# cwitkowitz/amt-tools

Measured on AMD Instinct MI355X. Metric: audio frames/sec (OnsetsFrames+Mel-229 inference), higher is better.
Workload: dtype bf16

## Files before the change

amt_tools_amd/_lib.py:

```python
import ctypes as C
import os
import re

_HERE = os.path.dirname(os.path.abspath(__file__))
LIB_PATH = os.environ.get('AMTX_LIB_PATH') or os.path.join(_HERE, 'csrc', 'libamtx.so')
HEADER_PATH = os.path.join(os.path.dirname(_HERE), 'include', 'amtx.h')
EXTRA_HEADERS = ('amtx_tracks.h',)

_lib = None


class AmtxError(RuntimeError):
    pass


ERR_UNSUPPORTED = -3


class _Pointer(C.c_void_p):
    @classmethod
    def from_param(cls, obj):
        if hasattr(obj, 'data_ptr'):
            obj = obj.data_ptr()
        elif hasattr(obj, 'ctypes'):
            obj = obj.ctypes.data
        elif isinstance(obj, (str, bytes)):
            raise TypeError('a pointer argument, not text')
        return C.c_void_p.from_param(obj)


_CTYPES = {'i': C.c_int, 'l': C.c_int64, 'z': C.c_size_t, 'f': C.c_float, 'd': C.c_double, 's': C.c_char_p, 'p': _Pointer}
_SCALARS = {'int': 'i', 'int64_t': 'l', 'size_t': 'z', 'float': 'f', 'double': 'd'}
_POINTEES = {'void', 'float', 'double', 'int', 'int32_t', 'int64_t', 'uint16_t', 'uint8_t'}
_PARAM = re.compile(r'(const )?(\w+) ?(\*{0,2}) ?(\w*)')


def parse_header(text):
    text = re.sub(r'/\*.*?\*/|//[^\n]*', ' ', text, flags=re.S)
    text = re.sub(r'^[ \t]*(#.*|extern "C" \{|\})[ \t]*$', '', text, flags=re.M)
    handles, table = set(), {}

    def letter(decl, param, is_return=False):
        m = _PARAM.fullmatch(param)
        if m:
            const, base, stars, name = m.groups()
            if not stars and not const and base in _SCALARS:
                return _SCALARS[base], name
            if stars == '*' and const and base == 'char':
                return 's', name
            if stars and not is_return and (base in _POINTEES or base in handles):
                return 'p', name
        raise AmtxError(f'cannot map "{param}" in the declaration "{decl}"')

    for decl in (' '.join(d.split()) for d in text.split(';')):
        m = re.fullmatch(r'typedef struct (\w+) \1', decl)
        if m:
            handles.add(m.group(1))
            continue
        m = re.fullmatch(r'(.*?) ?\b(amtx_\w+) ?\((.*)\)', decl)
        if not m:
            if decl:
                raise AmtxError(f'cannot read the declaration "{decl}"')
            continue
        ret, name, params = m.groups()
        if name in table:
            raise AmtxError(f'{name} is declared twice')
        params = [] if params.strip() == 'void' else [p.strip() for p in params.split(',')]
        letters, names = letter(decl, ret, is_return=True)[0], []
        for param in params:
            code, pname = letter(decl, param)
            letters += code
            names.append(pname)
        if 'stream' in names and (names.index('stream') != len(names) - 1 or params[-1].replace(' ', '') != 'void*stream'):
            raise AmtxError(f'`stream` must be the last parameter and a `void*` in the declaration "{decl}"')
        table[name] = (letters, 'stream' in names)
    return table


_signatures = None


def signatures():
    global _signatures
    if _signatures is None:
        with open(HEADER_PATH) as f:
            _signatures = parse_header(f.read())
    return _signatures


def declared_symbols():
    return sorted(signatures())


_extra_signatures = None


def extra_signatures():
    global _extra_signatures
    if _extra_signatures is None:
        tables, seen = {}, set(signatures())
        for header in EXTRA_HEADERS:
            with open(os.path.join(os.path.dirname(HEADER_PATH), header)) as f:
                tables[header] = parse_header(f.read())
            twice = seen & set(tables[header])
            if twice:
                raise AmtxError(f'{sorted(twice)[0]} is declared in {header} and in another header')
            seen |= set(tables[header])
        _extra_signatures = tables
    return _extra_signatures


_funcs = {}


def lib():
    global _lib
    if _lib is None:
        if not os.path.exists(LIB_PATH):
            raise AmtxError(f'{LIB_PATH} is missing: build the HIP extension first '
                            f'(python -m amt_tools_amd.build, or __graft_entry__.build()). '
                            f'There is no CPU fallback for the product path.')
        try:
            handle = C.CDLL(LIB_PATH)
        except OSError as e:
            raise AmtxError(f'cannot load {LIB_PATH}: {e}') from e
        bound = dict(signatures())
        for table in extra_signatures().values():
            bound.update(table)
        for name, (letters, stream) in bound.items():
            try:
                fn = getattr(handle, name)
            except AttributeError as e:
                raise AmtxError(f'{LIB_PATH} does not export {name}') from e
            fn.restype = _CTYPES[letters[0]]
            fn.argtypes = [_CTYPES[c] for c in letters[1:]]
            _funcs[name] = (fn, len(letters) - 1, letters[0] in 'il', stream)
        _lib = handle
    return _lib


def call(name, *args, device=None):
    lib()
    try:
        fn, nargs, checked, stream = _funcs[name]
    except KeyError:
        raise AmtxError(f'include/amtx.h and {", ".join(EXTRA_HEADERS)} declare no function {name}') from None
    fill_stream = stream and device is not None
    if len(args) + fill_stream != nargs:
        raise TypeError(f'{name} takes {nargs - fill_stream} arguments{" besides the stream" if fill_stream else ""} ({len(args)} given)')
    if device is None:
        rc = fn(*args)
    else:
        import torch
        with torch.cuda.device(device):
            rc = fn(*args, current_stream(device)) if stream else fn(*args)
    return check(rc, name) if checked else rc


def check(rc, what=''):
    if rc is None or rc < 0:
        msg = lib().amtx_last_error()
        raise AmtxError(f'{what} failed ({rc}): {msg.decode() if msg else "?"}')
    return rc


def ptr(t):
    if t is None:
        return None
    if hasattr(t, 'data_ptr'):
        return C.c_void_p(t.data_ptr())
    return C.c_void_p(t.ctypes.data)


def current_stream(device=None):
    import torch
    return C.c_void_p(torch.cuda.current_stream(device).cuda_stream)


GUARD_BYTES = 0
_GUARD_PATTERN = 0xA5
_GUARDED = {}


def alloc_workspace(nbytes, device):
    import torch
    nbytes = int(nbytes)
    g = int(GUARD_BYTES)
    if g <= 0:
        return torch.empty(nbytes, dtype=torch.uint8, device=device)
    assert g % 256 == 0
    full = torch.empty(nbytes + 2 * g, dtype=torch.uint8, device=device)
    full[:g] = _GUARD_PATTERN
    full[g + nbytes:] = _GUARD_PATTERN
    ws = full[g:g + nbytes]
    import weakref
    for k in [k for k, (r, _) in _GUARDED.items() if r() is None]:
        del _GUARDED[k]
    _GUARDED[ws.data_ptr()] = (weakref.ref(full), g)
    return ws


def guards_intact(ws):
    rec = _GUARDED.get(ws.data_ptr())
    base = getattr(ws, '_base', None)
    if rec is None or base is None or rec[0]() is not base:
        return True
    g = rec[1]
    return bool((base[:g] == _GUARD_PATTERN).all().item()) and bool((base[g + ws.numel():] == _GUARD_PATTERN).all().item())
```

amt_tools_amd/csrc/amtx_kernels.h:

```cpp
#pragma once
#include "amtx_common.h"

enum { AMTX_T_BF16 = 0, AMTX_T_F32 = 1, AMTX_T_SPLIT = 2 };

static inline size_t amtx_tsize(int t) { return t == AMTX_T_BF16 ? 2 : 4; }

struct GemmArgs {
    const void* A; int64_t lda; int a_type;
    const bf16_t* W; int n_pad, k_pad, planes;
    const float* bias;
    void* C; int64_t ldc; int c_type;
    int64_t M; int N, K;
    int groups; int64_t a_gs, w_gs, bias_gs, c_gs;
    const int2* pair_map = nullptr; float* pair_out = nullptr; int64_t pair_gs = 0, pair_pitch = 0;
    int pair_rows[16] = {0, 0, 0, 0, 0, 0, 0, 0, 0, 0, 0, 0, 0, 0, 0, 0};
    float* pair_max = nullptr; int pair_nh = 0;
    float* roll_out = nullptr; int roll_T = 0; float roll_thr = 0.5f; int roll_group = 0;
    bf16_t* copy16 = nullptr; int64_t copy16_ld = 0; int copy16_col0 = 0, copy16_gs = 0, copy16_pad = 0;
    int64_t a_plane = 0;
    int64_t a_valid_lo = 0, a_valid_hi = 0;
    int64_t a_split = 0, c_split = 0;
};
constexpr int AMTX_GEMM_MULTI_MAX = 10;
struct GemmMulti { GemmArgs p[AMTX_GEMM_MULTI_MAX]; int n; };

struct ConvArgs {
    const void* in; int in_type;
    const bf16_t* wfrag; int planes;
    const float* shift;
    void* out; int out_type;
    int B, T, F, c_out;
    int groups; int64_t in_gs, w_gs, shift_gs, out_gs;
    const float* feats = nullptr; int64_t f_stride_b = 0, f_stride_c = 0, f_stride_t = 0, f_stride_f = 0;
    int c_in = 0;
    const bf16_t* w1frag = nullptr; const float* shift1 = nullptr;
    int64_t w1_gs = 0;
    const float* f_clip_max = nullptr; const float* f_ref = nullptr;
    const void* feats16 = nullptr;
    int64_t out_ts = 0;
    int64_t in_split = 0, out_split = 0;
};
struct ConvTiling { int ft, ntf, ntt; int64_t ntiles; };
static inline ConvTiling amtx_conv_tiling(int B, int T, int F, int ft_max, int tt) {
    const int fe = (F + 1) & ~1;
    const int ntf = (fe + ft_max - 1) / ft_max, ntt = (T + tt - 1) / tt;
    return {2 * (((fe >> 1) + ntf - 1) / ntf), ntf, ntt, (int64_t)ntf * ntt * B};
}
static inline int amtx_conv_recip(int cols, int n) {
    const int inv = 65536 / cols + 1;
    for (int x = 0; x < n; ++x)
        if (((x * inv) >> 16) != x / cols) return 0;
    return inv;
}
struct ConvRefusal { int code = AMTX_OK; char text[192] = {0}; };
#define AMTX_ROUTE_REFUSE(r, code_, ...)                                  \
    do {                                                                   \
        (r).err.code = (code_);                                            \
        snprintf((r).err.text, sizeof((r).err.text), __VA_ARGS__);         \
        return (r);                                                        \
    } while (0)
#define AMTX_ROUTE_REQUIRE(r, cond, ...) do { if (!(cond)) AMTX_ROUTE_REFUSE(r, AMTX_ERR_ARG, __VA_ARGS__); } while (0)
#define AMTX_RETURN_REFUSAL(r)                                             \
    do {                                                                   \
        if ((r).err.code != AMTX_OK) {                                     \
            amtx_set_error("%s", (r).err.text);                            \
            return (r).err.code;                                           \
        }                                                                  \
    } while (0)

int amtx_launch_convx3(const ConvArgs& c, hipStream_t stream);
int amtx_launch_convx12(const ConvArgs& c, hipStream_t stream);

static inline __host__ __device__ bool amtx_conv1g_tapk(int c_in, int planes) { return (planes == 1 || planes == 2) && c_in >= 2 && c_in <= 8; }

struct Conv1Args {
    const float* in; int64_t stride_b, stride_c, stride_t, stride_f;
    const float* w;
    const float* shift;
    void* out; int out_type;
    int B, T, F, c_in, c_out;
    int groups; int64_t w_gs, shift_gs, out_gs;
    int relu = 1;
};

struct LstmArgs {
    const void* xproj; int x_type;
    const bf16_t* whh; int planes;
    void* out; int out_type;
    int B, T;
    int groups; int64_t x_gs, w_gs, out_gs;
    int hidden = 128;
    float* save = nullptr;
};

namespace amtx_bf16 {
#include "amtx_kernels_fmt.h"
}
#ifdef AMTX_WITH_F16
namespace amtx_f16 {
#include "amtx_kernels_fmt.h"
}
#endif
using namespace AMTX_FMT_NS;

size_t amtx_bce_loss_partials(int B, int T, int keys);
int amtx_launch_bce_loss(const float* logits, int64_t ld, const float* labels, const float* weight, int B, int T, int keys, float* loss,
                         float* grad, float* partial, hipStream_t stream);
int amtx_launch_loss_reduce(const float* partial, int64_t n, float inv_bt, float* loss, hipStream_t stream);
int amtx_launch_pianoroll(const float* logits, int64_t ld, int col0, int B, int T, int keys, float threshold, float* out,
                          hipStream_t stream);

int amtx_launch_cvt_pad_bf16(const float* src, int64_t ld_src, int n_src, bf16_t* dst, int ld_dst, int64_t rows, hipStream_t stream,
                             bool f16 = false );
int amtx_launch_cvt_split(const float* src, int64_t ld_src, int n_src, bf16_t* dst, int ld_dst, int64_t split, int64_t rows, hipStream_t stream);
int amtx_launch_zero_cols(void* base, int64_t pitch_bytes, int width_bytes, int64_t rows, hipStream_t stream);

constexpr int DEC_HALF = 150;
constexpr int DEC_TAPS = 2 * DEC_HALF + 1;
constexpr int DEC_KW = 352;
constexpr int DEC_NKS = DEC_KW / 32;
int amtx_launch_cqt_decimate(const float* in, int64_t n_in, int64_t in_stride, int in_pad, float* out, int64_t n_out, int64_t out_stride, int pad,
                             const void* tfrag, int zero_pads, float* maxbuf, int n_harm, int batch, hipStream_t stream);
```

amt_tools_amd/csrc/amtx_kernels_fmt.h:

```cpp

bool amtx_gemm_has_roll_epilogue(const GemmArgs& g);
int amtx_launch_gemm(const GemmArgs& g, hipStream_t stream);
int amtx_launch_gemm_multi(const GemmArgs* gs, int n, hipStream_t stream);
void amtx_gemm_pack_dims(int N, int K, int* n_pad, int* k_pad);
void amtx_gemm_pack_host(const float* W, int64_t ldw, int N, int K, int planes, bf16_t* out);

int amtx_launch_conv3x3(const ConvArgs& c, hipStream_t stream);
size_t amtx_conv1_wfrag_elems(int c_in, int planes);
void amtx_conv1_pack_host(const float* w, const float* scale, int c_in, int planes, bf16_t* out);
size_t amtx_conv3x3_wfrag_elems(int c_out, int planes);
void amtx_conv3x3_pack_host(const float* w, const float* scale, int c_out, int planes, bf16_t* out);
int amtx_launch_conv1(const Conv1Args& c, hipStream_t stream);

bool amtx_conv_stack_fused_ok(int B, int T, int F, int groups);
int amtx_launch_conv_stack(const ConvArgs& c2, const bf16_t* w3frag, int64_t w3_gs, const float* shift3, void* out, int64_t out_gs,
                           int64_t out_plane, hipStream_t stream);

int amtx_conv3x3_gen_ntc(int c_in, int c_out);
size_t amtx_conv3x3_gen_wfrag_elems(int c_in, int c_out, int planes);
void amtx_conv3x3_gen_pack_host(const float* w , const float* scale, int c_in, int c_out, int planes, bf16_t* out);
int amtx_launch_conv3x3_gen(const ConvArgs& c, int c_in, hipStream_t stream);
size_t amtx_conv1g_wfrag_elems(int c_in, int c_mid, int planes);
void amtx_conv1g_pack_host(const float* w , const float* scale, int c_in, int c_mid, int planes, bf16_t* out);
bool amtx_conv3x3_gen_can_fuse1(int c_in, int c_mid, int c_out, int planes);

int amtx_launch_bilstm(const LstmArgs& l, hipStream_t stream);
size_t amtx_bilstm_wfrag_elems(int hidden, int planes);
void amtx_bilstm_pack_host(const float* whh_fwd, const float* whh_bwd, int hidden, int planes, bf16_t* out);
int amtx_launch_bilstm_pack_dev(const float* whh_fwd, const float* whh_bwd, int hidden, int planes, bf16_t* frag_fwd, bf16_t* frag_bwd, hipStream_t stream);
int amtx_launch_bilstm_bwd(const float* dout, const float* save, const bf16_t* whh_t, int hidden, int planes, float* dxproj, int B, int T, int groups,
                           hipStream_t stream);

int amtx_pack_bn_fold_dev(const float* conv_bias, const float* gamma, const float* beta, const float* mean, const float* var, int c_out, float* scale,
                          float* shift, hipStream_t s);
int amtx_pack_conv3x3_dev(const float* w, const float* scale, int c_out, int planes, bf16_t* out, hipStream_t s);
int amtx_pack_conv1_dev(const float* w, const float* scale, int planes, bf16_t* out, hipStream_t s);
int amtx_pack_conv_gen_dev(const float* w, const float* scale, int c_in, int c_out, int ntc, int planes, bf16_t* out, hipStream_t s);
int amtx_pack_conv1g_dev(const float* w, const float* scale, int c_in, int c_mid, int planes, bf16_t* out, hipStream_t s);
int amtx_pack_scale_rows_dev(const float* w, const float* scale, int rows, int cols, float* out, hipStream_t s);
int amtx_pack_linear_dev(const float* W, int64_t ldw, int N, int K, int planes, int n_pad, int k_pad, int row0, int rows_owned, int perm_c, int perm_f,
                         bf16_t* out, hipStream_t s);
void amtx_pack_linear_host(const float* W, int64_t ldw, int N, int K, int planes, int n_pad, int k_pad, int row0, int rows_owned, int perm_c, int perm_f,
                           bf16_t* out);
int amtx_pack_head_fold_dev(const float* w_out, const float* w_fc1, const float* b_fc1, const float* b_out, int n_out, int dim_am, int kfc, int kfc_pad,
                            int nf3, int fq, float* wfold, float* bfold, hipStream_t s);
int amtx_pack_vec_add_dev(const float* a, const float* b, int n, float* out, hipStream_t s);
```

amt_tools_amd/csrc/amtx_pack_layouts.h:

```cpp
#pragma once
#include "amtx_common.h"

#include <cmath>

constexpr int AMTX_FRAG = 64 * 8;
constexpr int AMTX_CONV_CIN = 32;
constexpr int AMTX_LSTM_BWD_WAVES = 8;

static constexpr __host__ __device__ int g_wfrags_per_tile(int ci16) { return 9 * (ci16 / 2) + 5 * (ci16 % 2); }

static inline __host__ __device__ void amtx_split_store(bf16_t* out, size_t i, size_t plane_stride, int planes, float v) {
#if defined(__HIP_DEVICE_COMPILE__)
    asm volatile("" : "+v"(v));
#endif
    const bf16_t hi = f32_to_bf16_rn(v);
    out[i] = hi;
    if (planes == 2) out[i + plane_stride] = f32_to_bf16_rn(v - bf16_to_f32(hi));
}

namespace {
struct AmtxFragPut {
    bf16_t* out; int planes; int frag_elems = AMTX_FRAG;
    __host__ __device__ void operator()(size_t frag, int e, float v) const { amtx_split_store(out, frag * planes * frag_elems + e, frag_elems, planes, v); }
};
struct AmtxPlanePut {
    bf16_t* out; int planes; size_t plane_elems;
    __host__ __device__ void operator()(size_t i, float v) const { amtx_split_store(out, i, plane_elems, planes, v); }
};
}

static inline __host__ __device__ void amtx_bn_fold(const float* cb, const float* g, const float* be, const float* mu, const float* var, int c, float* scale,
                                                    float* shift) {
#pragma clang fp contract(off)
    const double s = (double)g[c] / sqrt((double)var[c] + 1e-5);
    scale[c] = (float)s;
    shift[c] = (float)((double)be[c] + ((double)cb[c] - (double)mu[c]) * s);
}

static inline __host__ __device__ void amtx_layout_scale_rows(int item, const float* w, const float* scale, int cols, float* out) {
    out[item] = w[item] * scale[item / cols];
}

static inline __host__ __device__ int amtx_layout_conv3x3_items(int c_out) { return 9 * (c_out / 16) * AMTX_FRAG; }
template <class Put>
static inline __host__ __device__ void amtx_layout_conv3x3(int item, const float* w, const float* scale, int c_out, const Put& put) {
    const int NT = c_out / 16;
    int r = item;
    const int j = r & 7; r >>= 3;
    const int l = r & 63; r >>= 6;
    const int nt = r % NT, tap = r / NT;
    const int row = l & 15;
    const int co = (row >> 2) * (4 * NT) + 4 * nt + (row & 3);
    const int ci = (l >> 4) * 8 + j;
    put(tap * NT + nt, l * 8 + j, w[((size_t)co * AMTX_CONV_CIN + ci) * 9 + tap] * (scale ? scale[co] : 1.0f));
}

constexpr int AMTX_LAYOUT_CONV1_ITEMS = 4 * 2 * AMTX_FRAG;
template <class Put>
static inline __host__ __device__ void amtx_layout_conv1(int item, const float* w, const float* scale, const Put& put) {
    int r = item;
    const int e = r & 7; r >>= 3;
    const int l = r & 63; r >>= 6;
    const int nt = r & 1, q = r >> 1;
    const int row = l & 15, g = l >> 4;
    const int co = (row >> 2) * 8 + 4 * nt + (row & 3);
    const int kw = e - q;
    put(q * 2 + nt, l * 8 + e, (g < 3 && kw >= 0 && kw <= 2) ? w[(size_t)co * 9 + g * 3 + kw] * (scale ? scale[co] : 1.0f) : 0.0f);
}

static inline void amtx_layout_conv1_multi(const float* w, const float* scale, int c_in, int planes, bf16_t* out) {
    const int kvalid = 9 * c_in, ksteps = (kvalid + 15) / 16;
    const AmtxFragPut put{out, planes, 64 * 4};
    for (int ks = 0; ks < ksteps; ++ks)
        for (int nt = 0; nt < 2; ++nt)
            for (int l = 0; l < 64; ++l) {
                const int row = l & 15;
                const int co = (row >> 2) * 8 + 4 * nt + (row & 3);
                for (int j = 0; j < 4; ++j) {
                    const int k = 16 * ks + 4 * (l >> 4) + j;
                    put(ks * 2 + nt, l * 4 + j, k < kvalid ? w[(size_t)co * kvalid + k] * (scale ? scale[co] : 1.0f) : 0.0f);
                }
            }
}

static inline __host__ __device__ int amtx_layout_conv_gen_items(int c_out) { return (c_out / 16) * AMTX_FRAG; }
template <class Put>
static inline __host__ __device__ void amtx_layout_conv_gen(int item, const float* w, const float* scale, int c_in, int ntc, const Put& put) {
    const int ci16 = c_in / 16, n32 = ci16 / 2, n16 = ci16 % 2;
    const int nmain = 9 * ntc * n32, nfrag = ntc * g_wfrags_per_tile(ci16);
    int r = item;
    const int j = r & 7; r >>= 3;
    const int l = r & 63; r >>= 6;
    const int nt = r % ntc, ch = r / ntc;
    const int row = l & 15, gq = l >> 4;
    const int co = ch * 16 * ntc + (row >> 2) * (4 * ntc) + 4 * nt + (row & 3);
    const float sc = scale ? scale[co] : 1.0f;
    auto wv = [&](int ci, int tap) { return w[((size_t)co * c_in + ci) * 9 + tap] * sc; };
    auto frag = [&](int f, float v) { put((size_t)ch * nfrag + f, l * 8 + j, v); };
    for (int tap = 0; tap < 9; ++tap)
        for (int ks = 0; ks < n32; ++ks) frag((tap * ntc + nt) * n32 + ks, wv(32 * ks + 8 * gq + j, tap));
    if (!n16) return;
    const int ct = 32 * n32 + 8 * (gq & 1) + j;
    for (int kw = 0; kw < 3; ++kw) frag(nmain + kw * ntc + nt, wv(ct, (gq < 2 ? 0 : 3) + kw));
    frag(nmain + 3 * ntc + nt, wv(ct, gq < 2 ? 6 : 7));
    frag(nmain + 4 * ntc + nt, gq < 2 ? wv(ct, 8) : 0.0f);
}

static inline __host__ __device__ int amtx_conv1g_ksteps(int c_in, bool tapk) { return tapk ? 3 : (9 * c_in + 31) / 32; }
static inline __host__ __device__ int amtx_layout_conv1g_items(int c_in, int c_mid, bool tapk) { return (c_mid / 16) * amtx_conv1g_ksteps(c_in, tapk) * AMTX_FRAG; }
template <class Put>
static inline __host__ __device__ void amtx_layout_conv1g(int item, const float* w, const float* scale, int c_in, bool tapk, const Put& put) {
    const int kvalid = 9 * c_in, nks = amtx_conv1g_ksteps(c_in, tapk);
    int r = item;
    const int j = r & 7; r >>= 3;
    const int l = r & 63; r >>= 6;
    const int ks = r % nks, nt = r / nks;
    const int co = 16 * nt + (l & 15);
    const int tap = 4 * ks + (l >> 4), k = 32 * ks + 8 * (l >> 4) + j;
    const bool valid = tapk ? tap < 9 && j < c_in : k < kvalid;
    const size_t src = tapk ? ((size_t)co * c_in + j) * 9 + tap : (size_t)co * kvalid + k;
    put(nt * nks + ks, l * 8 + j, valid ? w[src] * (scale ? scale[co] : 1.0f) : 0.0f);
}

static inline __host__ __device__ int amtx_fc1_col(int k, int nf3, int fq) { return (k % nf3) * fq + k / nf3; }

static inline __host__ __device__ int64_t amtx_layout_linear_items(int rows_owned, int k_pad) { return (int64_t)rows_owned * (k_pad / 8); }
template <class Put>
static inline __host__ __device__ void amtx_layout_linear(int64_t item, const float* W, int64_t ldw, int N, int K, int k_pad, int row0, int perm_c, int perm_f,
                                                          const Put& put) {
    const int n = (int)(item / (k_pad / 8)), k0 = 8 * (int)(item - (int64_t)n * (k_pad / 8));
    const float* src = W + (int64_t)n * ldw + (perm_c > 0 ? amtx_fc1_col(k0, perm_c, perm_f) : k0);
    const int step = perm_c > 0 ? perm_f : 1;
    for (int j = 0; j < 8; ++j) put((size_t)(row0 + n) * k_pad + k0 + j, n < N && k0 + j < K ? src[(int64_t)j * step] : 0.0f);
}

static inline __host__ __device__ int amtx_layout_bilstm_items(int hidden) { return hidden * hidden; }
template <class Put>
static inline __host__ __device__ void amtx_layout_bilstm(int item, const float* whh_fwd, const float* whh_bwd, int hidden, const Put& put) {
    const int nu = hidden / 16, ksn = hidden / 32;
    int r = item;
    const int l = r & 63; r >>= 6;
    const int ks = r % ksn; r /= ksn;
    const int q = r & 3; r >>= 2;
    const int u = r % nu, dir = r / nu;
    const float* src = (dir == 0 ? whh_fwd : whh_bwd) + (size_t)(q * hidden + 16 * u + (l & 15)) * hidden + 32 * ks + 8 * (l >> 4);
    for (int j = 0; j < 8; ++j) put(item >> 6, l * 8 + j, src[j]);
}

template <class Put>
static inline __host__ __device__ void amtx_layout_bilstm_transposed(int item, const float* whh_fwd, const float* whh_bwd, int hidden, const Put& put) {
    const int ut_n = hidden / (16 * AMTX_LSTM_BWD_WAVES), ksn = 4 * hidden / 32;
    int r = item;
    const int l = r & 63; r >>= 6;
    const int ks = r % ksn; r /= ksn;
    const int ut = r % ut_n; r /= ut_n;
    const int wv = r % AMTX_LSTM_BWD_WAVES, dir = r / AMTX_LSTM_BWD_WAVES;
    const float* src = (dir == 0 ? whh_fwd : whh_bwd) + (size_t)(32 * ks + 8 * (l >> 4)) * hidden + 16 * ut_n * wv + 16 * ut + (l & 15);
    for (int j = 0; j < 8; ++j) put(item >> 6, l * 8 + j, src[(size_t)j * hidden]);
}
```

amt_tools_amd/csrc/gemm.hip:

```cpp

#include "amtx_kernels.h"

#include <algorithm>
#include <cstdlib>

namespace {

constexpr int BM = 128, BN = 128, BK = 32;
constexpr int TILE_BYTES = BM * BK * 2;

__device__ __forceinline__ int lds_off(int row, int chunk) {
    return (row * 4 + (chunk ^ ((0x78 >> (((row >> 2) & 3) * 2)) & 3))) * 16;
}

template <int A_TYPE, int NS>
struct AStage {
    uint4 hi, lo;
    __device__ __forceinline__ void load(const char* base, int64_t row_off_elems, bool valid, int64_t vlo = 0, int64_t vhi = 0, int64_t split = 0) {
        if (A_TYPE == AMTX_T_SPLIT) {
            hi = valid ? *reinterpret_cast<const uint4*>(base + row_off_elems * 2) : make_uint4(0, 0, 0, 0);
            lo = valid ? *reinterpret_cast<const uint4*>(base + (split + row_off_elems) * 2) : make_uint4(0, 0, 0, 0);
        } else if (A_TYPE == AMTX_T_BF16) {
            hi = valid ? *reinterpret_cast<const uint4*>(base + row_off_elems * 2) : make_uint4(0, 0, 0, 0);
            lo = make_uint4(0, 0, 0, 0);
        } else {
            float4 x0 = make_float4(0, 0, 0, 0), x1 = make_float4(0, 0, 0, 0);
            if (valid && vhi > 0 && (row_off_elems < vlo || row_off_elems + 8 > vhi)) {
                float e[8];
#pragma unroll
                for (int i = 0; i < 8; ++i) {
                    const int64_t idx = row_off_elems + i;
                    e[i] = (idx >= vlo && idx < vhi) ? reinterpret_cast<const float*>(base)[idx] : 0.f;
                }
                x0 = make_float4(e[0], e[1], e[2], e[3]);
                x1 = make_float4(e[4], e[5], e[6], e[7]);
            } else if (valid) {
                struct __attribute__((packed, aligned(4))) f32x4_a4 { float x, y, z, w; };
                const f32x4_a4* p = reinterpret_cast<const f32x4_a4*>(base + row_off_elems * 4);
                const f32x4_a4 p0 = p[0], p1 = p[1];
                x0 = make_float4(p0.x, p0.y, p0.z, p0.w);
                x1 = make_float4(p1.x, p1.y, p1.z, p1.w);
            }
            hi = __builtin_bit_cast(uint4, x0);
            lo = __builtin_bit_cast(uint4, x1);
        }
    }
    __device__ __forceinline__ void finish() {
        if (A_TYPE == AMTX_T_F32) {
            const float4 x0 = __builtin_bit_cast(float4, hi), x1 = __builtin_bit_cast(float4, lo);
            const float f[8] = {x0.x, x0.y, x0.z, x0.w, x1.x, x1.y, x1.z, x1.w};
            uint32_t h[4], l[4];
#pragma unroll
            for (int i = 0; i < 4; ++i) {
                l[i] = 0;
                if (NS == 2) split_bf16x2(f[2 * i], f[2 * i + 1], h[i], l[i]);
                else h[i] = pack_bf16x2(f[2 * i], f[2 * i + 1]);
            }
            hi = make_uint4(h[0], h[1], h[2], h[3]);
            lo = make_uint4(l[0], l[1], l[2], l[3]);
        }
    }
};

template <int A_TYPE, int C_TYPE, int NS>
__device__ __forceinline__ void gemm_tile(const GemmArgs& g, int grp, int bx, int by, char* smem) {
    constexpr int BUF_BYTES = 2 * NS * TILE_BYTES;
    const int tid = threadIdx.x, lane = tid & 63, wave = tid >> 6;
    const int wm = wave >> 1, wn = wave & 1;
    const int64_t m0 = (int64_t)bx * BM;
    const int n0 = by * BN;

    const char* Abase = reinterpret_cast<const char*>(g.A) + (int64_t)grp * g.a_gs * (A_TYPE == AMTX_T_F32 ? 4 : 2);
    const bf16_t* Wbase = g.W + (int64_t)grp * g.w_gs;
    const int64_t plane_elems = (int64_t)g.n_pad * g.k_pad;

    const int srow0 = tid >> 2, srow1 = srow0 + 64, schunk = tid & 3;
    const bool arow_ok0 = (m0 + srow0) < g.M, arow_ok1 = (m0 + srow1) < g.M;
    const int64_t a_off0 = (m0 + srow0) * g.lda + schunk * 8, a_off1 = (m0 + srow1) * g.lda + schunk * 8;
    const int64_t w_off0 = (int64_t)(n0 + srow0) * g.k_pad + schunk * 8, w_off1 = (int64_t)(n0 + srow1) * g.k_pad + schunk * 8;
    const int soff0 = lds_off(srow0, schunk), soff1 = lds_off(srow1, schunk);

    AStage<A_TYPE, NS> sa0, sa1;
    uint4 sw0h, sw1h, sw0l = make_uint4(0, 0, 0, 0), sw1l = make_uint4(0, 0, 0, 0);
#define LOAD_TILE(k0)                                                                              \
    do {                                                                                           \
        const bool kok = ((k0) + schunk * 8) < g.K;                                                \
        sa0.load(Abase, a_off0 + (k0), arow_ok0 && kok, g.a_valid_lo, g.a_valid_hi, g.a_split);    \
        sa1.load(Abase, a_off1 + (k0), arow_ok1 && kok, g.a_valid_lo, g.a_valid_hi, g.a_split);    \
        sw0h = *reinterpret_cast<const uint4*>(Wbase + w_off0 + (k0));                             \
        sw1h = *reinterpret_cast<const uint4*>(Wbase + w_off1 + (k0));                             \
        if (NS == 2) {                                                                             \
            sw0l = *reinterpret_cast<const uint4*>(Wbase + plane_elems + w_off0 + (k0));           \
            sw1l = *reinterpret_cast<const uint4*>(Wbase + plane_elems + w_off1 + (k0));           \
        }                                                                                          \
    } while (0)
#define STORE_TILE(buf)                                                                            \
    do {                                                                                           \
        char* sb = smem + (buf) * BUF_BYTES;                                                       \
        sa0.finish();                                                                              \
        sa1.finish();                                                                              \
        *reinterpret_cast<uint4*>(sb + soff0) = sa0.hi;                                            \
        *reinterpret_cast<uint4*>(sb + soff1) = sa1.hi;                                            \
        if (NS == 2) {                                                                             \
            *reinterpret_cast<uint4*>(sb + TILE_BYTES + soff0) = sa0.lo;                           \
            *reinterpret_cast<uint4*>(sb + TILE_BYTES + soff1) = sa1.lo;                           \
        }                                                                                          \
        *reinterpret_cast<uint4*>(sb + NS * TILE_BYTES + soff0) = sw0h;                            \
        *reinterpret_cast<uint4*>(sb + NS * TILE_BYTES + soff1) = sw1h;                            \
        if (NS == 2) {                                                                             \
            *reinterpret_cast<uint4*>(sb + 3 * TILE_BYTES + soff0) = sw0l;                         \
            *reinterpret_cast<uint4*>(sb + 3 * TILE_BYTES + soff1) = sw1l;                         \
        }                                                                                          \
    } while (0)

    f32x4_t acc[4][4];
#pragma unroll
    for (int i = 0; i < 4; ++i)
#pragma unroll
        for (int j = 0; j < 4; ++j) acc[i][j] = (f32x4_t){0.f, 0.f, 0.f, 0.f};

    const int nk = g.k_pad / BK;
    LOAD_TILE(0);
    STORE_TILE(0);
    __syncthreads();

    const int frow = lane & 15, fchunk = lane >> 4;
    for (int kt = 0; kt < nk; ++kt) {
        const int cur = kt & 1;
        if (kt + 1 < nk) LOAD_TILE((kt + 1) * BK);
        const char* b = smem + cur * BUF_BYTES;
        uint4 af[4][NS], wf[4][NS];
#pragma unroll
        for (int t = 0; t < 4; ++t) {
            const int ar = wm * 64 + t * 16 + frow;
            const int wr = wn * 64 + t * 16 + frow;
#pragma unroll
            for (int p = 0; p < NS; ++p) {
                af[t][p] = *reinterpret_cast<const uint4*>(b + p * TILE_BYTES + lds_off(ar, fchunk));
                wf[t][p] = *reinterpret_cast<const uint4*>(b + (NS + p) * TILE_BYTES + lds_off(wr, fchunk));
            }
        }
#pragma unroll
        for (int nt = 0; nt < 4; ++nt)
#pragma unroll
            for (int mt = 0; mt < 4; ++mt) {
                acc[nt][mt] = mfma16(wf[nt][0], af[mt][0], acc[nt][mt]);
                if (NS == 2) {
                    acc[nt][mt] = mfma16(wf[nt][0], af[mt][1], acc[nt][mt]);
                    acc[nt][mt] = mfma16(wf[nt][1], af[mt][0], acc[nt][mt]);
                }
            }
        if (kt + 1 < nk) STORE_TILE(cur ^ 1);
        __syncthreads();
    }
// ... 107 lines not shown
    const bf16_t* a_src[4];
    const bf16_t* w_src[4];
#define GLDS_SET_TILE(TILE_ID)                                                                                \
    do {                                                                                                      \
        const unsigned lg = xcd_remap((unsigned)(TILE_ID), (unsigned)ntiles);                                 \
        const int tn0 = (lg % nbn) * TB;                                                                      \
        const int64_t tm0 = (int64_t)(lg / nbn) * TB;                                                         \
        _Pragma("unroll") for (int n = 0; n < 4; ++n) {                                                       \
            const int row = (wave * 4 + n) * 8 + (lane >> 3);                                                 \
            const int c = (lane & 7) ^ ((row >> 1) & 7);                                                      \
            const int cw = (lane & 7) ^ wswz(row);                                                            \
            int64_t mr = tm0 + row;                                                                           \
            if (mr >= g.M) mr = g.M - 1;           \
            a_src[n] = Abase + mr * a_pitch + c * 8;                                                          \
            w_src[n] = Wbase + (int64_t)(tn0 + row) * g.k_pad + cw * 8;                                       \
        }                                                                                                     \
    } while (0)
    const unsigned lds_base = __builtin_amdgcn_readfirstlane((unsigned)(uintptr_t)(lds_void_t*)smem) + wave * 4096;
#define GLDS_ISSUE(k0, buf)                                                                                   \
    do {                                                                                                      \
        const unsigned sb = lds_base + (buf) * 2 * TILE;                                                      \
        const int64_t a_off = (int64_t)((k0) / GBK) * a_kstep;                                                \
        glds16x4(a_src[0] + a_off, a_src[1] + a_off, a_src[2] + a_off, a_src[3] + a_off, sb);                 \
        glds16x4(w_src[0] + (k0), w_src[1] + (k0), w_src[2] + (k0), w_src[3] + (k0), sb + TILE);              \
    } while (0)
#define GLDS_COMPUTE(buf)                                                                                     \
    do {                                                                                                      \
        const char* b = smem + (buf) * 2 * TILE;                                                              \
        _Pragma("unroll") for (int kk = 0; kk < 2; ++kk) {                                                    \
            uint4 af[MT], wf[4];                                                                              \
            _Pragma("unroll") for (int t = 0; t < MT; ++t) {                                                  \
                const int ar = wm * (TB / 2) + t * 16 + frow;                                                 \
                af[t] = *reinterpret_cast<const uint4*>(b + ar * 128 + (((kk * 4 + fchunk) ^ ((ar >> 1) & 7)) << 4)); \
            }                                                                                                 \
            _Pragma("unroll") for (int t = 0; t < 4; ++t) {                                                   \
                const int wr = wn * 64 + 16 * (frow >> 2) + 4 * t + (frow & 3);         \
                wf[t] = *reinterpret_cast<const uint4*>(b + TILE + wr * 128 + (((kk * 4 + fchunk) ^ wswz(wr)) << 4)); \
            }                                                                                                 \
            _Pragma("unroll") for (int nt = 0; nt < 4; ++nt)                                                  \
                _Pragma("unroll") for (int mt = 0; mt < MT; ++mt) acc[nt][mt] = mfma16(wf[nt], af[mt], acc[nt][mt]); \
        }                                                                                                     \
    } while (0)
#define GLDS_SYNC()                                                                                           \
    do {                                                                                                      \
        asm volatile("s_waitcnt vmcnt(0)" ::: "memory");                                                      \
        __syncthreads();                                                                                      \
    } while (0)

    const int nk = g.k_pad / GBK;
    const int frow = lane & 15, fchunk = lane >> 4;

    int tile = blockIdx.x;
    GLDS_SET_TILE(tile);
    GLDS_ISSUE(0, 0);
    GLDS_SYNC();
    int cur = 0;
    for (;;) {
        const unsigned lg = xcd_remap((unsigned)tile, (unsigned)ntiles);
        const int n0 = (lg % nbn) * TB;
        const int64_t m0 = (int64_t)(lg / nbn) * TB;
        const int next = tile + (int)gridDim.x;
        const bool has_next = next < ntiles;

        f32x4_t acc[4][MT];
#pragma unroll
        for (int i = 0; i < 4; ++i)
#pragma unroll
            for (int j = 0; j < MT; ++j) acc[i][j] = (f32x4_t){0.f, 0.f, 0.f, 0.f};

        for (int kt = 0; kt + 1 < nk; ++kt) {
            GLDS_ISSUE((kt + 1) * GBK, cur ^ 1);
            GLDS_COMPUTE(cur);
            GLDS_SYNC();
            cur ^= 1;
        }
        if (has_next) {
            GLDS_SET_TILE(next);
            GLDS_ISSUE(0, cur ^ 1);
        }
        GLDS_COMPUTE(cur);

        {
            const int nb = n0 + wn * 64 + 16 * (lane >> 4);
            float bv[4][4];
#pragma unroll
            for (int nt = 0; nt < 4; ++nt)
#pragma unroll
                for (int r = 0; r < 4; ++r) bv[nt][r] = (bias && nb + 4 * nt < g.N) ? bias[nb + 4 * nt + r] : 0.f;
            constexpr int ES = (C_TYPE == AMTX_T_BF16 ? 2 : 4);
            const bool wide = nb + 16 <= g.N && ((g.ldc * ES) % 16) == 0;
#pragma unroll
            for (int mt = 0; mt < MT; ++mt) {
                const int64_t m = m0 + wm * (TB / 2) + mt * 16 + (lane & 15);
                if (m >= g.M) continue;
                char* dst = Cbase + (m * g.ldc + nb) * ES;
                float o[4][4];
#pragma unroll
                for (int nt = 0; nt < 4; ++nt)
#pragma unroll
                    for (int r = 0; r < 4; ++r) o[nt][r] = acc[nt][mt][r] + bv[nt][r];
                if (C_TYPE == AMTX_T_F32) {
                    if (g.C) {
#pragma unroll
                        for (int nt = 0; nt < 4; ++nt)
                            if (wide || nb + 4 * nt < g.N) reinterpret_cast<float4*>(dst)[nt] = make_float4(o[nt][0], o[nt][1], o[nt][2], o[nt][3]);
                    }
                    if (g.copy16) {
                        bf16_t* cp = g.copy16 + m * g.copy16_ld + g.copy16_col0 + (int64_t)grp * g.copy16_gs + nb;
#pragma unroll
                        for (int nt = 0; nt < 4; ++nt) {
                            const int n4 = nb + 4 * nt;
                            if (n4 < g.N) reinterpret_cast<uint2*>(cp)[nt] = make_uint2(pack_bf16x2(o[nt][0], o[nt][1]), pack_bf16x2(o[nt][2], o[nt][3]));
                            else if (n4 < g.N + g.copy16_pad) reinterpret_cast<uint2*>(cp)[nt] = make_uint2(0u, 0u);
                        }
                    }
                    if (g.roll_out && grp == g.roll_group) {
                        const unsigned bclip = (unsigned)m / (unsigned)g.roll_T, tfrm = (unsigned)m - bclip * (unsigned)g.roll_T;
                        float* ro = g.roll_out + ((int64_t)bclip * g.N + nb) * g.roll_T + tfrm;
#pragma unroll
                        for (int nt = 0; nt < 4; ++nt)
#pragma unroll
                            for (int r = 0; r < 4; ++r)
                                if (nb + 4 * nt + r < g.N) {
                                    const float sg = 1.0f / (1.0f + expf(-o[nt][r]));
                                    ro[(int64_t)(4 * nt + r) * g.roll_T] = g.roll_thr < 0.f ? sg : (sg < g.roll_thr ? 0.f : 1.f);
                                }
                    }
                } else if (wide) {
#pragma unroll
                    for (int h = 0; h < 2; ++h)
                        reinterpret_cast<uint4*>(dst)[h] = make_uint4(pack_bf16x2(o[2 * h][0], o[2 * h][1]), pack_bf16x2(o[2 * h][2], o[2 * h][3]),
                                                                     pack_bf16x2(o[2 * h + 1][0], o[2 * h + 1][1]), pack_bf16x2(o[2 * h + 1][2], o[2 * h + 1][3]));
                } else {
#pragma unroll
                    for (int nt = 0; nt < 4; ++nt)
                        if (nb + 4 * nt < g.N) reinterpret_cast<uint2*>(dst)[nt] = make_uint2(pack_bf16x2(o[nt][0], o[nt][1]), pack_bf16x2(o[nt][2], o[nt][3]));
                }
            }
        }
        if (!has_next) break;
        GLDS_SYNC();
        cur ^= 1;
        tile = next;
    }
#undef GLDS_SET_TILE
#undef GLDS_ISSUE
#undef GLDS_COMPUTE
#undef GLDS_SYNC
}
constexpr int RBK = 32, RST = 4, RTB = 256;
constexpr int RING_MAX_NPAD = 4096;
constexpr int ROP = RTB * RBK * 2;
constexpr int RSTAGE = 2 * ROP;
__device__ uint4 g_gemm_trash[4];

__device__ __forceinline__ int rswz(int q) { return (0x78 >> (q * 2)) & 3; }

#ifdef AMTX_GEMM_TIMING
__device__ unsigned long long g_gemm_prof[2][16];
#define PP_TICK(SLOT)                                                      \
    do {                                                                   \
        const unsigned long long now_ = __builtin_readcyclecounter();      \
        prof_acc[SLOT] += now_ - prof_t;                                   \
        prof_t = now_;                                                     \
    } while (0)
#else
#define PP_TICK(SLOT) do {} while (0)
#endif

template <int C_TYPE>
__global__ __launch_bounds__(512) void gemm_pp_kernel(GemmArgs g, int ntiles) {
    extern __shared__ __attribute__((aligned(16))) char smem[];
    constexpr int MT = 8;
    constexpr int ES = (C_TYPE == AMTX_T_BF16 ? 2 : 4);
    constexpr int NSTORE = MT * (C_TYPE == AMTX_T_BF16 ? 2 : 4);
    const int tid = threadIdx.x, lane = tid & 63, wave = __builtin_amdgcn_readfirstlane(tid >> 6);
    const int wm = wave >> 2, wn = wave & 3;
    const int grp = blockIdx.z;
    const unsigned nbn = g.n_pad / RTB;
    const int nk = g.k_pad / RBK;

    const bf16_t* Abase = reinterpret_cast<const bf16_t*>(g.A) + (int64_t)grp * g.a_gs;
    const bf16_t* Wbase = g.W + (int64_t)grp * g.w_gs;
    char* Cbase = reinterpret_cast<char*>(g.C) + (int64_t)grp * g.c_gs * ES;
    float* bias_l = reinterpret_cast<float*>(smem + RST * RSTAGE);
    for (int i = tid; i < g.n_pad; i += 512) bias_l[i] = (g.bias && i < g.N) ? g.bias[(int64_t)grp * g.bias_gs + i] : 0.f;

    const bf16_t* a_src[2];
    const bf16_t* w_src[2];
#define PP_SET_TILE(TILE_ID)                                                                                  \
    do {                                                                                                      \
        const unsigned lg = xcd_remap((unsigned)(TILE_ID), (unsigned)ntiles);                                 \
        const int tn0 = (lg % nbn) * RTB;                                                                     \
        const int64_t tm0 = (int64_t)(lg / nbn) * RTB;                                                        \
        _Pragma("unroll") for (int n = 0; n < 2; ++n) {                                                       \
            const int row = wave * 32 + n * 16 + (lane >> 2);                                                 \
            int64_t mr = tm0 + row;                                                                           \
            if (mr >= g.M) mr = g.M - 1;                                                                      \
            a_src[n] = Abase + mr * g.lda + ((lane & 3) ^ rswz((row >> 2) & 3)) * 8;                          \
            w_src[n] = Wbase + (int64_t)(tn0 + row) * g.k_pad + ((lane & 3) ^ rswz((row >> 4) & 3)) * 8;      \
        }                                                                                                     \
    } while (0)
    const unsigned lds_base = __builtin_amdgcn_readfirstlane((unsigned)(uintptr_t)(lds_void_t*)smem) + wave * 2048;

    const int my_tiles = (ntiles - (int)blockIdx.x + (int)gridDim.x - 1) / (int)gridDim.x;
    const int S = my_tiles * nk;
    int is = 0, ikt = 0, itile = blockIdx.x;
    bool pending_w = false;
#define PP_ISSUE_A()                                                                                          \
    do {                                                                                                      \
        if (is < S) {                                                                                         \
            const unsigned sb = lds_base + (is & (RST - 1)) * RSTAGE;                                         \
            _Pragma("unroll") for (int n = 0; n < 2; ++n) glds16(a_src[n] + ikt * RBK, sb + n * 1024);        \
            pending_w = true;                                                                                 \
        }                                                                                                     \
    } while (0)
#define PP_ISSUE_W()                                                                                          \
    do {                                                                                                      \
        if (pending_w) {                                                                                      \
            const unsigned sb = lds_base + (is & (RST - 1)) * RSTAGE;                                         \
            _Pragma("unroll") for (int n = 0; n < 2; ++n) glds16(w_src[n] + ikt * RBK, sb + ROP + n * 1024);  \
            pending_w = false;                                                                                \
            ++is;                                                                                             \
            if (++ikt == nk) {                                                                                \
                ikt = 0;                                                                                      \
                itile += (int)gridDim.x;                                                                      \
                if (is < S) PP_SET_TILE(itile);                                                               \
            }                                                                                                 \
        }                                                                                                     \
    } while (0)
#define PP_BARRIER()                                                                                          \
    do {                                                                                                      \
        __builtin_amdgcn_sched_barrier(0);                                                                    \
        asm volatile("s_barrier" ::: "memory");                                                               \
        __builtin_amdgcn_sched_barrier(0);                                                                    \
    } while (0)

    PP_SET_TILE(itile);
    PP_ISSUE_A(); PP_ISSUE_W();
    PP_ISSUE_A(); PP_ISSUE_W();
    PP_ISSUE_A();
    if (S >= 3) wait_vm<6>(); else if (S == 2) wait_vm<4>(); else wait_vm<0>();
    asm volatile("s_waitcnt lgkmcnt(0)\n\ts_barrier" ::: "memory");
    __builtin_amdgcn_sched_barrier(0);
    if (wm == 1) PP_BARRIER();

    const int frow = lane & 15, fchunk = lane >> 4;
    const int a_off = (wm * 128 + frow) * 64 + ((fchunk ^ rswz((frow >> 2) & 3)) << 4);
    const int w_off = ROP + (wn * 64 + 16 * (frow >> 2) + (frow & 3)) * 64 + ((fchunk ^ rswz(frow >> 2)) << 4);

    f32x4_t acc[4][MT];
#pragma unroll
    for (int i = 0; i < 4; ++i)
#pragma unroll
        for (int j = 0; j < MT; ++j) acc[i][j] = (f32x4_t){0.f, 0.f, 0.f, 0.f};

#ifdef AMTX_GEMM_TIMING
    unsigned long long prof_acc[14] = {0,0,0,0,0,0,0,0,0,0,0,0,0,0};
    unsigned long long prof_t = __builtin_readcyclecounter();
#endif
    int ckt = 0, ctile = blockIdx.x;
    bool stores_recent = false;
    for (int cs = 0; cs < S; ++cs) {
        const char* b = smem + (cs & (RST - 1)) * RSTAGE;
        uint4 af[4], wf[4];
#pragma unroll
        for (int t = 0; t < 4; ++t) wf[t] = *reinterpret_cast<const uint4*>(b + w_off + t * 256);
#pragma unroll
        for (int t = 0; t < 4; ++t) af[t] = *reinterpret_cast<const uint4*>(b + a_off + t * 1024);
        __builtin_amdgcn_sched_barrier(0);
        PP_ISSUE_W();
        PP_TICK(0);
        PP_BARRIER();
        PP_TICK(1);
        asm volatile("s_waitcnt lgkmcnt(0)" ::: "memory");
        PP_TICK(2);
        __builtin_amdgcn_s_setprio(1);
#pragma unroll
        for (int mt = 0; mt < 4; ++mt)
#pragma unroll
            for (int nt = 0; nt < 4; ++nt) acc[nt][mt] = mfma16(wf[nt], af[mt], acc[nt][mt]);
        __builtin_amdgcn_s_setprio(0);
        PP_TICK(3);
        PP_BARRIER();
        PP_TICK(4);
        {
            const int newer = min(S - 2 - cs, 1);
            if (newer >= 0) {
                if (!stores_recent) { if (newer == 1) wait_vm<4>(); else wait_vm<0>(); }
                else { if (newer == 1) wait_vm<4 + NSTORE>(); else wait_vm<NSTORE>(); }
            }
        }
        __builtin_amdgcn_sched_barrier(0);
        PP_TICK(5);
#pragma unroll
        for (int t = 0; t < 4; ++t) af[t] = *reinterpret_cast<const uint4*>(b + a_off + (4 + t) * 1024);
        __builtin_amdgcn_sched_barrier(0);
        PP_ISSUE_A();
        stores_recent = false;
        PP_TICK(6);
        PP_BARRIER();
        PP_TICK(7);
        asm volatile("s_waitcnt lgkmcnt(0)" ::: "memory");
        PP_TICK(8);
        __builtin_amdgcn_s_setprio(1);
#pragma unroll
        for (int mt = 0; mt < 4; ++mt)
#pragma unroll
            for (int nt = 0; nt < 4; ++nt) acc[nt][4 + mt] = mfma16(wf[nt], af[mt], acc[nt][4 + mt]);
        __builtin_amdgcn_s_setprio(0);
        PP_TICK(9);

        if (++ckt == nk) {
            const unsigned lg = xcd_remap((unsigned)ctile, (unsigned)ntiles);
            const int n0 = (lg % nbn) * RTB;
            const int64_t m0 = (int64_t)(lg / nbn) * RTB;
            const int nb = n0 + wn * 64 + 16 * (lane >> 4);
            f32x4_t bv[4];
#pragma unroll
            for (int nt = 0; nt < 4; ++nt) bv[nt] = *reinterpret_cast<const f32x4_t*>(bias_l + nb + 4 * nt);
#pragma unroll
            for (int mt = 0; mt < MT; ++mt) {
                const int64_t m = m0 + wm * 128 + mt * 16 + (lane & 15);
#ifdef AMTX_PP_NOSTORE
                char* dst = reinterpret_cast<char*>(g_gemm_trash);
#else
                char* dst = m < g.M ? Cbase + (m * g.ldc + nb) * ES : reinterpret_cast<char*>(g_gemm_trash);
#endif
                float o[4][4];
#pragma unroll
                for (int nt = 0; nt < 4; ++nt)
#pragma unroll
                    for (int r = 0; r < 4; ++r) o[nt][r] = acc[nt][mt][r] + bv[nt][r];
                if (C_TYPE == AMTX_T_F32) {
#pragma unroll
                    for (int nt = 0; nt < 4; ++nt) reinterpret_cast<float4*>(dst)[nt] = make_float4(o[nt][0], o[nt][1], o[nt][2], o[nt][3]);
                } else {
#pragma unroll
                    for (int h = 0; h < 2; ++h)
                        reinterpret_cast<uint4*>(dst)[h] = make_uint4(pack_bf16x2(o[2 * h][0], o[2 * h][1]), pack_bf16x2(o[2 * h][2], o[2 * h][3]),
                                                                     pack_bf16x2(o[2 * h + 1][0], o[2 * h + 1][1]), pack_bf16x2(o[2 * h + 1][2], o[2 * h + 1][3]));
                }
#pragma unroll
                for (int nt = 0; nt < 4; ++nt) acc[nt][mt] = (f32x4_t){0.f, 0.f, 0.f, 0.f};
            }
            ckt = 0;
            ctile += (int)gridDim.x;
            stores_recent = true;
            PP_TICK(13);
        }
        PP_TICK(10);
        PP_BARRIER();
        PP_TICK(11);
    }
#ifdef AMTX_GEMM_TIMING
    if (lane == 0 && (wave & 3) == 0) {
        for (int i = 0; i < 12; ++i) atomicAdd(&g_gemm_prof[wm][i], prof_acc[i]);
        atomicAdd(&g_gemm_prof[wm][13], prof_acc[13]);
        atomicAdd(&g_gemm_prof[wm][12], (unsigned long long)S);
    }
#endif
    if (wm == 0) PP_BARRIER();
#undef PP_SET_TILE
#undef PP_ISSUE_A
#undef PP_ISSUE_W
#undef PP_BARRIER
}

constexpr int SPL = 256 * RBK * 2;
constexpr int SSTAGE = 4 * SPL;

template <int C_TYPE>
__global__ __launch_bounds__(512) void gemm_split_kernel(GemmArgs g, int ntiles) {
    extern __shared__ __attribute__((aligned(16))) char smem[];
    constexpr int MT = 8;
    const int tid = threadIdx.x, lane = tid & 63, wave = __builtin_amdgcn_readfirstlane(tid >> 6);
    const int wm = wave >> 2, wn = wave & 3;
    const int grp = blockIdx.z;
    const unsigned nbn = g.n_pad / RTB;
    const int nk = g.k_pad / RBK;

    const bf16_t* Abase = reinterpret_cast<const bf16_t*>(g.A) + (int64_t)grp * g.a_gs;
    const bf16_t* Wbase = g.W + (int64_t)grp * g.w_gs;
    const int64_t w_plane = (int64_t)g.n_pad * g.k_pad;
    const float* bias = g.bias ? g.bias + (int64_t)grp * g.bias_gs : nullptr;

    const bf16_t* a_src[2];
    const bf16_t* w_src[2];
#define SP_SET_TILE(TILE_ID)                                                                                  \
    do {                                                                                                      \
        const unsigned lg = xcd_remap((unsigned)(TILE_ID), (unsigned)ntiles);                                 \
        const int tn0 = (lg % nbn) * RTB;                                                                     \
        const int64_t tm0 = (int64_t)(lg / nbn) * RTB;                                                        \
        _Pragma("unroll") for (int n = 0; n < 2; ++n) {                                                       \
            const int row = wave * 32 + n * 16 + (lane >> 2);                                                 \
            int64_t mr = tm0 + row;                                                                           \
            if (mr >= g.M) mr = g.M - 1;                                                                      \
            a_src[n] = Abase + mr * g.lda + ((lane & 3) ^ rswz((row >> 2) & 3)) * 8;                          \
            w_src[n] = Wbase + (int64_t)(tn0 + row) * g.k_pad + ((lane & 3) ^ rswz((row >> 4) & 3)) * 8;      \
        }                                                                                                     \
    } while (0)
    const unsigned lds_base = __builtin_amdgcn_readfirstlane((unsigned)(uintptr_t)(lds_void_t*)smem) + wave * 2048;
#define SP_ISSUE(k0, buf)                                                                                     \
    do {                                                                                                      \
        const unsigned sb = lds_base + (buf) * SSTAGE;                                                        \
        glds16x2(a_src[0] + (k0), a_src[1] + (k0), sb);                                                       \
        glds16x2(a_src[0] + g.a_split + (k0), a_src[1] + g.a_split + (k0), sb + SPL);                         \
        glds16x2(w_src[0] + (k0), w_src[1] + (k0), sb + 2 * SPL);                                             \
        glds16x2(w_src[0] + w_plane + (k0), w_src[1] + w_plane + (k0), sb + 3 * SPL);                         \
    } while (0)
    const int frow = lane & 15, fchunk = lane >> 4;
    const int a_off = (wm * 128 + frow) * 64 + ((fchunk ^ rswz((frow >> 2) & 3)) << 4);
    const int w_off = 2 * SPL + (wn * 64 + 16 * (frow >> 2) + (frow & 3)) * 64 + ((fchunk ^ rswz(frow >> 2)) << 4);
#define SP_COMPUTE(buf)                                                                                       \
    do {                                                                                                      \
        const char* b = smem + (buf) * SSTAGE;                                                                \
        uint4 wh[4], wl[4];                                                                                   \
        _Pragma("unroll") for (int t = 0; t < 4; ++t) {                                                       \
            wh[t] = *reinterpret_cast<const uint4*>(b + w_off + t * 256);                                     \
            wl[t] = *reinterpret_cast<const uint4*>(b + w_off + SPL + t * 256);                               \
        }                                                                                                     \
        _Pragma("unroll") for (int h = 0; h < 2; ++h) {                                                       \
            uint4 ah[4], al[4];                                                                               \
            _Pragma("unroll") for (int t = 0; t < 4; ++t) {                                                   \
                ah[t] = *reinterpret_cast<const uint4*>(b + a_off + (4 * h + t) * 1024);                      \
                al[t] = *reinterpret_cast<const uint4*>(b + a_off + SPL + (4 * h + t) * 1024);                \
            }                                                                                                 \
            _Pragma("unroll") for (int mt = 0; mt < 4; ++mt)                                                  \
                _Pragma("unroll") for (int nt = 0; nt < 4; ++nt) acc[nt][4 * h + mt] = mfma16(wh[nt], ah[mt], acc[nt][4 * h + mt]); \
            _Pragma("unroll") for (int mt = 0; mt < 4; ++mt)                                                  \
                _Pragma("unroll") for (int nt = 0; nt < 4; ++nt) acc[nt][4 * h + mt] = mfma16(wh[nt], al[mt], acc[nt][4 * h + mt]); \
            _Pragma("unroll") for (int mt = 0; mt < 4; ++mt)                                                  \
                _Pragma("unroll") for (int nt = 0; nt < 4; ++nt) acc[nt][4 * h + mt] = mfma16(wl[nt], ah[mt], acc[nt][4 * h + mt]); \
        }                                                                                                     \
    } while (0)
#define SP_SYNC()                                                                                             \
    do {                                                                                                      \
        asm volatile("s_waitcnt vmcnt(0)" ::: "memory");                                                      \
        __syncthreads();                                                                                      \
    } while (0)

    int tile = blockIdx.x;
    SP_SET_TILE(tile);
    SP_ISSUE(0, 0);
    SP_SYNC();
    int cur = 0;
    for (;;) {
        const unsigned lg = xcd_remap((unsigned)tile, (unsigned)ntiles);
        const int n0 = (lg % nbn) * RTB;
        const int64_t m0 = (int64_t)(lg / nbn) * RTB;
        const int next = tile + (int)gridDim.x;
        const bool has_next = next < ntiles;

        f32x4_t acc[4][MT];
#pragma unroll
        for (int i = 0; i < 4; ++i)
#pragma unroll
            for (int j = 0; j < MT; ++j) acc[i][j] = (f32x4_t){0.f, 0.f, 0.f, 0.f};

        for (int kt = 0; kt + 1 < nk; ++kt) {
            SP_ISSUE((kt + 1) * RBK, cur ^ 1);
            SP_COMPUTE(cur);
            SP_SYNC();
            cur ^= 1;
        }
        if (has_next) {
            SP_SET_TILE(next);
            SP_ISSUE(0, cur ^ 1);
        }
        SP_COMPUTE(cur);

        {
            const int nb = n0 + wn * 64 + 16 * (lane >> 4);
            float bv[4][4];
#pragma unroll
            for (int nt = 0; nt < 4; ++nt)
#pragma unroll
                for (int r = 0; r < 4; ++r) bv[nt][r] = (bias && nb + 4 * nt < g.N) ? bias[nb + 4 * nt + r] : 0.f;
#pragma unroll
            for (int mt = 0; mt < MT; ++mt) {
                const int64_t m = m0 + wm * 128 + mt * 16 + (lane & 15);
                if (m >= g.M || nb + 16 > g.N) continue;
                float o[16];
#pragma unroll
                for (int nt = 0; nt < 4; ++nt)
#pragma unroll
                    for (int r = 0; r < 4; ++r) o[4 * nt + r] = acc[nt][mt][r] + bv[nt][r];
                if (C_TYPE == AMTX_T_F32) {
                    float4* dst = reinterpret_cast<float4*>(reinterpret_cast<float*>(g.C) + (int64_t)grp * g.c_gs + m * g.ldc + nb);
#pragma unroll
                    for (int nt = 0; nt < 4; ++nt) dst[nt] = make_float4(o[4 * nt], o[4 * nt + 1], o[4 * nt + 2], o[4 * nt + 3]);
                } else {
                    bf16_t* dh = reinterpret_cast<bf16_t*>(g.C) + (int64_t)grp * g.c_gs + m * g.ldc + nb;
                    uint32_t hh[8], ll[8];
// ... 343 lines not shown
                                if (nb + 4 * nt + r < g.N) {
                                    const float sg = 1.0f / (1.0f + expf(-o[nt][r]));
                                    ro[(int64_t)(4 * nt + r) * g.roll_T] = g.roll_thr < 0.f ? sg : (sg < g.roll_thr ? 0.f : 1.f);
                                }
                    }
                }
            }
            zero_acc();
            ckt = 0;
            ++cj;
        }
    }
    asm volatile("s_waitcnt vmcnt(0)" ::: "memory");
}

int launch_skinny(const GemmArgs& g, hipStream_t stream, bool split) {
    const int64_t ntiles = (g.M + 255) / 256;
    AMTX_REQUIRE(ntiles < (1ll << 31), "gemm: too many output tiles");
    int64_t gx = std::max<int64_t>(1, 256 / std::max(1, g.groups));
    if (gx > ntiles) gx = ntiles;
    if (split) {
        AMTX_GRANT_LDS(gemm_skinny_split_kernel, SK_LDS);
        hipLaunchKernelGGL(gemm_skinny_split_kernel, dim3((unsigned)gx, 1, (unsigned)g.groups), dim3(512), SK_LDS, stream, g, (int)ntiles);
    } else {
        AMTX_GRANT_LDS(gemm_skinny_kernel, SK_LDS);
        hipLaunchKernelGGL(gemm_skinny_kernel, dim3((unsigned)gx, 1, (unsigned)g.groups), dim3(512), SK_LDS, stream, g, (int)ntiles);
    }
    AMTX_CHECK_LAUNCH();
    return AMTX_OK;
}

template <int C_TYPE, int TB>
int launch_glds(const GemmArgs& g, hipStream_t stream) {
    const int64_t ntiles = ((g.M + TB - 1) / TB) * (g.n_pad / TB);
    AMTX_REQUIRE(ntiles < (1ll << 31), "gemm: too many output tiles");
    const size_t lds = 4 * (size_t)TB * GBK * 2;
    auto kern = gemm_glds_kernel<C_TYPE, TB>;
    AMTX_GRANT_LDS(kern, lds);
    hipLaunchKernelGGL(kern, dim3(persistent_gx(TB == 128 ? 512 : 256, g.groups, ntiles), 1, (unsigned)g.groups), dim3(TB * 2), lds, stream, g, (int)ntiles);
    AMTX_CHECK_LAUNCH();
    return AMTX_OK;
}

template <int A_TYPE, int C_TYPE, int NS>
int launch(const GemmArgs& g, hipStream_t stream) {
    dim3 grid((unsigned)((g.M + BM - 1) / BM), (unsigned)(g.n_pad / BN), (unsigned)g.groups);
    const size_t lds = 2 * 2 * NS * TILE_BYTES;
    hipLaunchKernelGGL((gemm_kernel<A_TYPE, C_TYPE, NS>), grid, dim3(256), lds, stream, g);
    AMTX_CHECK_LAUNCH();
    return AMTX_OK;
}

}

#if defined(AMTX_GEMM_TIMING) && !defined(AMTX_F16)
extern "C" void amtxdbg_gemm_prof(unsigned long long* out, int reset) {
    unsigned long long h[2][16];
    (void)hipMemcpyFromSymbol(h, HIP_SYMBOL(g_gemm_prof), sizeof(h));
    memcpy(out, h, sizeof(h));
    if (reset) { memset(h, 0, sizeof(h)); (void)hipMemcpyToSymbol(HIP_SYMBOL(g_gemm_prof), h, sizeof(h)); }
}
#endif

namespace AMTX_FMT_NS {

void amtx_gemm_pack_dims(int N, int K, int* n_pad, int* k_pad) {
    *n_pad = ((N + BN - 1) / BN) * BN;
    *k_pad = ((K + GBK - 1) / GBK) * GBK;
}

void amtx_gemm_pack_host(const float* W, int64_t ldw, int N, int K, int planes, bf16_t* out) {
    int n_pad, k_pad;
    amtx_gemm_pack_dims(N, K, &n_pad, &k_pad);
    amtx_pack_linear_host(W, ldw, N, K, planes, n_pad, k_pad, 0, n_pad, 0, 0, out);
}


struct GemmSwitches { bool no_skinny, force_pp, no_pp, no_split_dma; };
static const GemmSwitches& gemm_switches() {
    auto on = [](const char* name) { return getenv(name) != nullptr; };
    static const GemmSwitches sw = {on("AMTX_GEMM_NO_SKINNY"), on("AMTX_GEMM_PP"), on("AMTX_GEMM_NO_PP"), on("AMTX_GEMM_NO_SPLIT_DMA")};
    return sw;
}

static int gemm_validate(const GemmArgs& g) {
    AMTX_REQUIRE(g.A && g.W, "gemm: null pointer");
    AMTX_REQUIRE(!g.pair_map || (g.a_type == AMTX_T_F32 && g.c_type == AMTX_T_F32 && g.pair_out && g.N % 2 == 0), "gemm: the magnitude epilogue needs fp32 A / C, an output and an even N");
    AMTX_REQUIRE(g.M > 0 && g.N > 0 && g.K > 0 && g.groups > 0, "gemm: bad sizes");
    AMTX_REQUIRE(g.K % 8 == 0 && g.N % 4 == 0, "gemm: K must be a multiple of 8 and N of 4 (K=%d N=%d)", g.K, g.N);
    AMTX_REQUIRE(g.n_pad % BN == 0 && g.k_pad % BK == 0 && g.n_pad >= g.N && g.k_pad >= g.K, "gemm: bad packed dims");
    AMTX_REQUIRE(g.a_type == AMTX_T_F32 ? (g.a_valid_hi > 0 ? ((uintptr_t)g.A % 4) == 0 : (g.lda % 4 == 0 && ((uintptr_t)g.A % 16) == 0))
                                        : ((g.lda * 2) % 16 == 0 && ((uintptr_t)g.A % 16) == 0),
                 "gemm: A rows must be 16-byte aligned (4-byte aligned for a bounded fp32 A)");
    AMTX_REQUIRE(g.a_valid_hi == 0 || (g.a_type == AMTX_T_F32 && g.a_valid_lo >= 0 && g.a_valid_hi > g.a_valid_lo), "gemm: bad valid range of A");
    AMTX_REQUIRE(g.ldc % 4 == 0 && ((uintptr_t)g.C % 16) == 0, "gemm: C rows must be 16-byte aligned");
    AMTX_REQUIRE(g.planes == 1 || g.planes == 2, "gemm: planes must be 1 or 2");
    return AMTX_OK;
}

int amtx_launch_gemm_multi(const GemmArgs* gs, int n, hipStream_t stream) {
    AMTX_REQUIRE(gs && n >= 1 && n <= AMTX_GEMM_MULTI_MAX, "gemm_multi: 1 .. %d problems", AMTX_GEMM_MULTI_MAX);
    GemmMulti mm;
    unsigned gx = 0, gy = 0;
    for (int i = 0; i < n; ++i) {
        const GemmArgs& g = gs[i];
        AMTX_REQUIRE(g.C || g.pair_map, "gemm: null pointer");
        if (const int rc = gemm_validate(g); rc != AMTX_OK) return rc;
        AMTX_REQUIRE(g.a_type == AMTX_T_F32 && g.c_type == AMTX_T_F32 && g.planes == 2 && g.groups == gs[0].groups,
                     "gemm_multi: fp32 A / C, two weight planes and one group count for all problems");
        mm.p[i] = g;
        gx = std::max(gx, (unsigned)((g.M + BM - 1) / BM));
        gy = std::max(gy, (unsigned)(g.n_pad / BN));
    }
    mm.n = n;
    const size_t lds = 2 * 2 * 2 * TILE_BYTES;
    hipLaunchKernelGGL((gemm_multi_kernel<AMTX_T_F32, AMTX_T_F32, 2>), dim3(gx, gy, (unsigned)(n * gs[0].groups)), dim3(256), lds, stream, mm);
    AMTX_CHECK_LAUNCH();
    return AMTX_OK;
}

enum GemmRoute { ROUTE_SKINNY, ROUTE_SKINNY_SPLIT, ROUTE_GLDS256, ROUTE_GLDS128, ROUTE_PP, ROUTE_SPLIT, ROUTE_GENERIC, ROUTE_ERROR };
struct GemmRouted { GemmRoute route; const char* error; };

static GemmRouted gemm_route(const GemmArgs& g, const GemmSwitches& sw) {
#define ROUTE_REQUIRE(cond, msg) if (!(cond)) return {ROUTE_ERROR, msg}
    const bool tiles256 = g.n_pad % 256 == 0 && g.N % 256 == 0 && g.M >= 256;
    if (g.a_type == AMTX_T_BF16 && g.planes == 1 && g.K % GBK == 0 && g.k_pad == g.K && (g.lda % 8) == 0) {
        if (!sw.no_skinny && g.n_pad == 128 && g.c_type == AMTX_T_F32 && g.M >= 1024 && g.K >= 2 * GBK && g.M < (1ll << 31) * 256) return {ROUTE_SKINNY, nullptr};
        if (!tiles256) return {ROUTE_GLDS128, nullptr};
        if (!g.a_plane && !sw.no_pp && (sw.force_pp || g.K <= 1024) && g.n_pad <= RING_MAX_NPAD && g.K >= 4 * RBK && (g.ldc * amtx_tsize(g.c_type)) % 16 == 0)
            return {ROUTE_PP, nullptr};
        return {ROUTE_GLDS256, nullptr};
    }
    ROUTE_REQUIRE(!g.a_plane, "gemm: planar A exists on the bf16 direct-to-LDS path only");
    if (g.a_type == AMTX_T_SPLIT) {
        ROUTE_REQUIRE(g.planes == 2 && g.a_split > 0 && (g.a_split % 8) == 0, "gemm: two-plane A needs two-plane weights and a plane stride that keeps 16-byte alignment");
        ROUTE_REQUIRE(g.c_type != AMTX_T_SPLIT || (g.c_split > 0 && (g.c_split % 8) == 0), "gemm: two-plane C needs a plane stride");
        ROUTE_REQUIRE(!g.pair_map && !g.roll_out && !g.copy16 && g.C, "gemm: two-plane A has the plain epilogues only");
        const bool c_aligned = g.c_type == AMTX_T_SPLIT ? ((g.ldc * 2) % 16 == 0 && (g.c_split % 8) == 0) : ((g.ldc * 4) % 16 == 0);
        if (!sw.no_split_dma && tiles256 && g.K == g.k_pad && (g.lda % 8) == 0 && g.c_type != AMTX_T_BF16 && c_aligned) return {ROUTE_SPLIT, nullptr};
        ROUTE_REQUIRE(g.c_type != AMTX_T_BF16, "gemm: two-plane A writes fp32 or two-plane C");
        if (!sw.no_skinny && !sw.no_split_dma && g.n_pad == 128 && g.c_type == AMTX_T_F32 && g.M >= 1024 && g.K == g.k_pad && g.K >= 2 * RBK && (g.lda % 8) == 0 &&
            g.M < (1ll << 31) * 256)
            return {ROUTE_SKINNY_SPLIT, nullptr};
        return {ROUTE_GENERIC, nullptr};
    }
    ROUTE_REQUIRE(g.c_type != AMTX_T_SPLIT, "gemm: two-plane C needs two-plane A");
    return {ROUTE_GENERIC, nullptr};
#undef ROUTE_REQUIRE
}

static bool route_has_roll_epilogue(GemmRoute r, const GemmArgs& g) { return (r == ROUTE_SKINNY || r == ROUTE_GLDS128) && g.c_type == AMTX_T_F32; }
bool amtx_gemm_has_roll_epilogue(const GemmArgs& g) { return route_has_roll_epilogue(gemm_route(g, gemm_switches()).route, g); }

int amtx_launch_gemm(const GemmArgs& g, hipStream_t stream) {
    if (const int rc = gemm_validate(g); rc != AMTX_OK) return rc;
    const GemmRouted r = gemm_route(g, gemm_switches());
    const bool roll_epilogue = route_has_roll_epilogue(r.route, g);
    AMTX_REQUIRE(g.a_type == AMTX_T_BF16 || g.a_type == AMTX_T_F32 || g.a_type == AMTX_T_SPLIT, "gemm: bad A type");
    AMTX_REQUIRE(!g.copy16 || (roll_epilogue && g.copy16_pad % 4 == 0 && g.N + g.copy16_pad <= g.n_pad &&
                               (g.copy16_ld % 4) == 0 && ((g.copy16_col0 | g.copy16_gs) % 4) == 0 && ((uintptr_t)g.copy16 % 8) == 0),
                 "gemm: bad bf16-copy epilogue arguments");
    AMTX_REQUIRE(g.C || g.pair_map || g.roll_out || g.copy16, "gemm: no output");
    AMTX_REQUIRE(!g.roll_out || roll_epilogue, "gemm: the piano-roll epilogue exists on the bf16 direct-to-LDS path with fp32 C only");
    AMTX_REQUIRE(!g.roll_out || (g.roll_T > 0 && g.M % g.roll_T == 0 && g.M < (1ll << 31)), "gemm: piano-roll epilogue: M must be clips x frames");
    const bool c16 = g.c_type == AMTX_T_BF16;
    switch (r.route) {
        case ROUTE_ERROR: amtx_set_error("%s", r.error); return AMTX_ERR_ARG;
        case ROUTE_SKINNY: case ROUTE_SKINNY_SPLIT: return launch_skinny(g, stream, r.route == ROUTE_SKINNY_SPLIT);
        case ROUTE_GLDS256: return c16 ? launch_glds<AMTX_T_BF16, 256>(g, stream) : launch_glds<AMTX_T_F32, 256>(g, stream);
        case ROUTE_GLDS128: return c16 ? launch_glds<AMTX_T_BF16, 128>(g, stream) : launch_glds<AMTX_T_F32, 128>(g, stream);
        case ROUTE_PP: return c16 ? launch_pp<AMTX_T_BF16>(g, stream) : launch_pp<AMTX_T_F32>(g, stream);
        case ROUTE_SPLIT: return g.c_type == AMTX_T_SPLIT ? launch_split<AMTX_T_SPLIT>(g, stream) : launch_split<AMTX_T_F32>(g, stream);
        case ROUTE_GENERIC: break;
    }
    if (g.a_type == AMTX_T_SPLIT) return g.c_type == AMTX_T_SPLIT ? launch<AMTX_T_SPLIT, AMTX_T_SPLIT, 2>(g, stream) : launch<AMTX_T_SPLIT, AMTX_T_F32, 2>(g, stream);
    const int key = (g.a_type << 2) | (g.c_type << 1) | (g.planes - 1);
    switch (key) {
        case 0: return launch<AMTX_T_BF16, AMTX_T_BF16, 1>(g, stream);
        case 1: return launch<AMTX_T_BF16, AMTX_T_BF16, 2>(g, stream);
        case 2: return launch<AMTX_T_BF16, AMTX_T_F32, 1>(g, stream);
        case 3: return launch<AMTX_T_BF16, AMTX_T_F32, 2>(g, stream);
        case 4: return launch<AMTX_T_F32, AMTX_T_BF16, 1>(g, stream);
        case 5: return launch<AMTX_T_F32, AMTX_T_BF16, 2>(g, stream);
        case 6: return launch<AMTX_T_F32, AMTX_T_F32, 1>(g, stream);
        case 7: return launch<AMTX_T_F32, AMTX_T_F32, 2>(g, stream);
    }
    amtx_set_error("gemm: unsupported type combination");
    return AMTX_ERR_UNSUPPORTED;
}

}
```

amt_tools_amd/csrc/lstm.hip:

```cpp

#include "amtx_kernels.h"
#include "amtx_pack_layouts.h"

#include <type_traits>

namespace {

constexpr int H = 128;
constexpr int UB = 1;
constexpr int LWAVES = H / (16 * UB);
constexpr int LTHREADS = 64 * LWAVES;
constexpr int HP = H + 8;
constexpr int HBUF_BYTES = 16 * HP * 2;

template <bool FAST>
__device__ __forceinline__ float sigmoid_f(float x) {
    if (FAST) return __builtin_amdgcn_rcpf(1.0f + __builtin_amdgcn_exp2f(-1.4426950408889634f * x));
    return 1.0f / (1.0f + expf(-x));
}
template <bool FAST>
__device__ __forceinline__ float tanh_f(float x) {
    if (FAST) return fmaf(2.0f, __builtin_amdgcn_rcpf(1.0f + __builtin_amdgcn_exp2f(-2.8853900817779268f * x)), -1.0f);
    return tanhf(x);
}
// ... 47 lines not shown
    __device__ __forceinline__ uint4 load(int gi, int k, int p) const {
        return __builtin_bit_cast(uint4, *reinterpret_cast<const gu4_t*>(wb + ((gi * SGK + k) * NS + p) * 1024 + wlane));
    }
    __device__ __forceinline__ void load_group(int gi, uint4 (&dst)[SGK][NS]) const {
        static_for<0, SGK>([&](auto kc) {
            static_for<0, NS>([&](auto pc) { dst[decltype(kc)::value][decltype(pc)::value] = load(gi, decltype(kc)::value, decltype(pc)::value); });
        });
    }
};

template <int X_TYPE> struct XRaw { typedef float4 type; };
template <> struct XRaw<AMTX_T_BF16> { typedef uint2 type; };

template <int X_TYPE>
__device__ __forceinline__ void load_x(const char* xbase, int64_t row_off, typename XRaw<X_TYPE>::type (&dst)[UB][4]) {
#pragma unroll
    for (int ub = 0; ub < UB; ++ub)
#pragma unroll
        for (int q = 0; q < 4; ++q) {
            const int64_t e = row_off + q * 128 + 16 * ub;
            dst[ub][q] = *reinterpret_cast<const typename XRaw<X_TYPE>::type*>(xbase + e * (X_TYPE == AMTX_T_F32 ? 4 : 2));
        }
}
__device__ __forceinline__ f32x4_t unpack_x(float4 v) { return (f32x4_t){v.x, v.y, v.z, v.w}; }
__device__ __forceinline__ f32x4_t unpack_x(uint2 v) {
    return (f32x4_t){unpack16_lo(v.x), unpack16_hi(v.x), unpack16_lo(v.y), unpack16_hi(v.y)};
}

__device__ __forceinline__ void lds_barrier() {
    asm volatile("s_waitcnt lgkmcnt(0)\n\ts_barrier" ::: "memory");
    __builtin_amdgcn_sched_barrier(0);
}

template <int NS, int X_TYPE, int OUT_TYPE, bool FAST>
__device__ __forceinline__ void lstm_step(char* smem, int cur, const uint4 (&wf)[UB][4][4][NS], const typename XRaw<X_TYPE>::type (&xcur)[UB][4],
                                          typename XRaw<X_TYPE>::type (&xnext)[UB][4], float (&c)[UB][4], const char* xbase, char* obase, int t, int tnext,
                                          int clip, int g, int wave, bool clip_ok) {
    const char* hb = smem + cur * NS * HBUF_BYTES;
    uint4 hf[4][NS];
#pragma unroll
    for (int ks = 0; ks < 4; ++ks)
#pragma unroll
        for (int p = 0; p < NS; ++p)
            hf[ks][p] = *reinterpret_cast<const uint4*>(hb + p * HBUF_BYTES + (clip * HP + 32 * ks + 8 * g) * 2);

    load_x<X_TYPE>(xbase, (int64_t)tnext * 1024, xnext);

    f32x4_t acc[UB][4];
#pragma unroll
    for (int ub = 0; ub < UB; ++ub)
#pragma unroll
        for (int q = 0; q < 4; ++q) acc[ub][q] = unpack_x(xcur[ub][q]);
#pragma unroll
    for (int ks = 0; ks < 4; ++ks)
#pragma unroll
        for (int ub = 0; ub < UB; ++ub)
#pragma unroll
            for (int q = 0; q < 4; ++q) {
                acc[ub][q] = mfma16(wf[ub][q][ks][0], hf[ks][0], acc[ub][q]);
                if (NS == 2) {
                    acc[ub][q] = mfma16(wf[ub][q][ks][0], hf[ks][1], acc[ub][q]);
                    acc[ub][q] = mfma16(wf[ub][q][ks][1], hf[ks][0], acc[ub][q]);
                }
            }

    char* hn = smem + (cur ^ 1) * NS * HBUF_BYTES;
#pragma unroll
    for (int ub = 0; ub < UB; ++ub) {
        float h[4];
#pragma unroll
        for (int r = 0; r < 4; ++r) {
            h[r] = lstm_cell<FAST>(lstm_gates<FAST>(acc[ub][0][r], acc[ub][1][r], acc[ub][2][r], acc[ub][3][r]), c[ub][r]);
        }
        uint2 hiw, low;
        split16<NS>(h, hiw, low);
        store16<NS>(hn, HBUF_BYTES, (clip * HP + 16 * UB * wave + 16 * ub + 4 * g) * 2, hiw, low);
        if (clip_ok) {
            const int64_t e = (int64_t)t * 256 + 16 * ub;
            if (OUT_TYPE == AMTX_T_BF16) *reinterpret_cast<uint2*>(obase + e * 2) = hiw;
            else *reinterpret_cast<float4*>(obase + e * 4) = make_float4(h[0], h[1], h[2], h[3]);
        }
    }
    lds_barrier();
}

template <int NS, int X_TYPE, int OUT_TYPE>
__global__ __launch_bounds__(LTHREADS) void bilstm_kernel(LstmArgs a) {
    extern __shared__ __attribute__((aligned(16))) char smem[];
    constexpr bool FAST = true;
    const int tid = threadIdx.x, lane = tid & 63, wave = tid >> 6;
    const int clip = lane & 15, g = lane >> 4;
    const int b0 = blockIdx.x * 16, dir = blockIdx.y, grp = blockIdx.z;
    const int b = b0 + clip;
    const bool clip_ok = b < a.B;
    const int T = a.T;

    uint4 wf[UB][4][4][NS];
    {
        const uint4* w = reinterpret_cast<const uint4*>(a.whh + (int64_t)grp * a.w_gs) + lane;
#pragma unroll
        for (int ub = 0; ub < UB; ++ub)
#pragma unroll
            for (int q = 0; q < 4; ++q)
#pragma unroll
                for (int ks = 0; ks < 4; ++ks)
#pragma unroll
                    for (int p = 0; p < NS; ++p)
                        wf[ub][q][ks][p] = w[((((((dir * LWAVES + wave) * UB + ub) * 4 + q) * 4 + ks) * NS) + p) * 64];
    }

    for (int i = tid; i < 2 * NS * HBUF_BYTES / 16; i += LTHREADS) reinterpret_cast<uint4*>(smem)[i] = make_uint4(0, 0, 0, 0);

    float c[UB][4];
#pragma unroll
    for (int ub = 0; ub < UB; ++ub)
#pragma unroll
        for (int r = 0; r < 4; ++r) c[ub][r] = 0.f;

    const char* xbase = reinterpret_cast<const char*>(a.xproj) +
                        ((int64_t)grp * a.x_gs + (int64_t)(clip_ok ? b : 0) * T * 1024 + dir * 512 + 16 * UB * wave + 4 * g) * (X_TYPE == AMTX_T_BF16 ? 2 : 4);
    char* obase = reinterpret_cast<char*>(a.out) +
                  ((int64_t)grp * a.out_gs + (int64_t)(clip_ok ? b : 0) * T * 256 + dir * 128 + 16 * UB * wave + 4 * g) * (OUT_TYPE == AMTX_T_BF16 ? 2 : 4);

    typename XRaw<X_TYPE>::type x0[UB][4], x1[UB][4], x2[UB][4], x3[UB][4];
    auto tidx = [&](int s) { return (int64_t)step_frame(s, T, dir); };
    load_x<X_TYPE>(xbase, tidx(0) * 1024, x0);
    load_x<X_TYPE>(xbase, tidx(1) * 1024, x1);
    load_x<X_TYPE>(xbase, tidx(2) * 1024, x2);
    __syncthreads();

    for (int s = 0; s < T; s += 4) {
        lstm_step<NS, X_TYPE, OUT_TYPE, FAST>(smem, 0, wf, x0, x3, c, xbase, obase, (int)tidx(s), (int)tidx(s + 3), clip, g, wave, clip_ok);
        lstm_step<NS, X_TYPE, OUT_TYPE, FAST>(smem, 1, wf, x1, x0, c, xbase, obase, (int)tidx(s + 1), (int)tidx(s + 4), clip, g, wave, clip_ok && s + 1 < T);
        lstm_step<NS, X_TYPE, OUT_TYPE, FAST>(smem, 0, wf, x2, x1, c, xbase, obase, (int)tidx(s + 2), (int)tidx(s + 5), clip, g, wave, clip_ok && s + 2 < T);
        lstm_step<NS, X_TYPE, OUT_TYPE, FAST>(smem, 1, wf, x3, x2, c, xbase, obase, (int)tidx(s + 3), (int)tidx(s + 6), clip, g, wave, clip_ok && s + 3 < T);
    }
}

template <int X_TYPE> struct XScalar { typedef float type; };
template <> struct XScalar<AMTX_T_BF16> { typedef unsigned int type; };
__device__ __forceinline__ float unpack_xs(float v, bool) { return v; }
__device__ __forceinline__ float unpack_xs(unsigned int v, bool odd) { return odd ? unpack16_hi(v) : unpack16_lo(v); }

template <int X_TYPE>
__device__ __forceinline__ void load_x4(const char* xbase, int64_t row_off, typename XScalar<X_TYPE>::type (&dst)[4]) {
#pragma unroll
    for (int q = 0; q < 4; ++q)
    {
        if (X_TYPE == AMTX_T_F32) dst[q] = *reinterpret_cast<const typename XScalar<X_TYPE>::type*>(xbase + (row_off + q * 128) * 4);
        else dst[q] = *reinterpret_cast<const unsigned int*>(xbase + (row_off + q * 128) * 2);
    }
}

template <int NS, int X_TYPE, int OUT_TYPE, bool FAST, int NC>
__device__ __forceinline__ void lstm4_step(char* smem, int cur, const uint4 (&wf)[4][4][NS], const typename XScalar<X_TYPE>::type (&xcur)[NC][4],
                                           typename XScalar<X_TYPE>::type (&xnext)[NC][4], float (&c)[NC], const char* const (&xbase)[NC],
                                           char* const (&obase)[NC], int t, int tnext, int lane, const int (&hwoff)[NC], const bool (&clip_ok)[NC],
                                           float* save) {
    constexpr int RSTEP = 4 / NC;
    const char* hb = smem + cur * NS * HBUF_BYTES;
    uint4 hf[4][NS];
#pragma unroll
    for (int ks = 0; ks < 4; ++ks)
#pragma unroll
        for (int p = 0; p < NS; ++p)
            hf[ks][p] = *reinterpret_cast<const uint4*>(hb + p * HBUF_BYTES + ((lane & 15) * HP + 32 * ks + 8 * (lane >> 4)) * 2);

#pragma unroll
    for (int j = 0; j < NC; ++j) load_x4<X_TYPE>(xbase[j], (int64_t)tnext * 1024, xnext[j]);

    f32x4_t acc[4];
#pragma unroll
    for (int q = 0; q < 4; ++q) {
        acc[q] = (f32x4_t){0.f, 0.f, 0.f, 0.f};
#pragma unroll
        for (int j = 0; j < NC; ++j) acc[q][RSTEP * j] = unpack_xs(xcur[j][q], lane & 1);
    }
#pragma unroll
    for (int ks = 0; ks < 4; ++ks) {
#pragma unroll
        for (int q = 0; q < 4; ++q) acc[q] = mfma16(hf[ks][0], wf[q][ks][0], acc[q]);
        if (NS == 2) {
#pragma unroll
            for (int q = 0; q < 4; ++q) acc[q] = mfma16(hf[ks][NS - 1], wf[q][ks][0], acc[q]);
#pragma unroll
            for (int q = 0; q < 4; ++q) acc[q] = mfma16(hf[ks][0], wf[q][ks][NS - 1], acc[q]);
        }
    }

    char* hn = smem + (cur ^ 1) * NS * HBUF_BYTES;
    Gates z[NC];
    float h[NC];
    uint32_t hiw[NC], low[NC];
#pragma unroll
    for (int j = 0; j < NC; ++j) z[j] = lstm_gates<FAST>(acc[0][RSTEP * j], acc[1][RSTEP * j], acc[2][RSTEP * j], acc[3][RSTEP * j]);
#pragma unroll
    for (int j = 0; j < NC; ++j) {
        h[j] = lstm_cell<FAST>(z[j], c[j]);
        low[j] = 0;
        if (NS == 2) split_bf16x2(h[j], 0.f, hiw[j], low[j]);
        else hiw[j] = pack_bf16x2(h[j], 0.f);
    }
#pragma unroll
    for (int j = 0; j < NC; ++j) {
        *reinterpret_cast<unsigned short*>(hn + hwoff[j]) = (unsigned short)hiw[j];
        if (NS == 2) *reinterpret_cast<unsigned short*>(hn + HBUF_BYTES + hwoff[j]) = (unsigned short)low[j];
    }
#pragma unroll
    for (int j = 0; j < NC; ++j) {
        if (NC == 1 && save && clip_ok[j]) {
            float* sv = save + (int64_t)t * (2 * 5 * H);
            sv[0] = z[j].i; sv[H] = z[j].f; sv[2 * H] = z[j].g; sv[3 * H] = z[j].o; sv[4 * H] = c[j];
        }
        if (clip_ok[j]) {
            if (OUT_TYPE == AMTX_T_BF16) *reinterpret_cast<unsigned short*>(obase[j] + (int64_t)t * 256 * 2) = (unsigned short)hiw[j];
            else *reinterpret_cast<float*>(obase[j] + (int64_t)t * 256 * 4) = h[j];
        }
    }
    lds_barrier();
}

template <int NS, int X_TYPE, int OUT_TYPE, int NC = 1>
__global__ __launch_bounds__(LTHREADS) void bilstm4_kernel(LstmArgs a) {
    extern __shared__ __attribute__((aligned(16))) char smem[];
    constexpr bool FAST = true;
    const int tid = threadIdx.x, lane = tid & 63, wave = tid >> 6;
    const int unit = 16 * wave + (lane & 15), cg = lane >> 4;
    const int dir = blockIdx.y, grp = blockIdx.z;
    const int T = a.T;

    uint4 wf[4][4][NS];
    {
        const uint4* w = reinterpret_cast<const uint4*>(a.whh + (int64_t)grp * a.w_gs) + lane;
#pragma unroll
        for (int q = 0; q < 4; ++q)
#pragma unroll
            for (int ks = 0; ks < 4; ++ks)
#pragma unroll
                for (int p = 0; p < NS; ++p) wf[q][ks][p] = w[(((((dir * LWAVES + wave) * 4 + q) * 4 + ks) * NS) + p) * 64];
    }
    for (int i = tid; i < 2 * NS * HBUF_BYTES / 16; i += LTHREADS) reinterpret_cast<uint4*>(smem)[i] = make_uint4(0, 0, 0, 0);

    float c[NC];
    bool clip_ok[NC];
    const char* xbase[NC];
    char* obase[NC];
    int hwoff[NC];
    float* save = nullptr;
#pragma unroll
    for (int j = 0; j < NC; ++j) {
        const int b = (blockIdx.x * 4 + cg) * NC + j;
        clip_ok[j] = b < a.B;
        c[j] = 0.f;
        xbase[j] = reinterpret_cast<const char*>(a.xproj) +
                   ((int64_t)grp * a.x_gs + (int64_t)(clip_ok[j] ? b : 0) * T * 1024 + dir * 512 + (X_TYPE == AMTX_T_BF16 ? (unit & ~1) : unit)) *
                       (X_TYPE == AMTX_T_BF16 ? 2 : 4);
        obase[j] = reinterpret_cast<char*>(a.out) +
                   ((int64_t)grp * a.out_gs + (int64_t)(clip_ok[j] ? b : 0) * T * 256 + dir * 128 + unit) * (OUT_TYPE == AMTX_T_BF16 ? 2 : 4);
        hwoff[j] = ((4 * cg + (4 / NC) * j) * HP + unit) * 2;
        if (NC == 1) save = a.save ? a.save + (((int64_t)grp * a.B + (clip_ok[j] ? b : 0)) * T * 2 + dir) * (5 * H) + unit : nullptr;
    }

    typename XScalar<X_TYPE>::type x0[NC][4], x1[NC][4], x2[NC][4], x3[NC][4];
    auto tidx = [&](int s) { return (int64_t)step_frame(s, T, dir); };
#pragma unroll
    for (int j = 0; j < NC; ++j) {
        load_x4<X_TYPE>(xbase[j], tidx(0) * 1024, x0[j]);
        load_x4<X_TYPE>(xbase[j], tidx(1) * 1024, x1[j]);
        load_x4<X_TYPE>(xbase[j], tidx(2) * 1024, x2[j]);
    }
    __syncthreads();

    for (int s = 0; s < T; s += 4) {
        bool ok1[NC], ok2[NC], ok3[NC];
#pragma unroll
        for (int j = 0; j < NC; ++j) { ok1[j] = clip_ok[j] && s + 1 < T; ok2[j] = clip_ok[j] && s + 2 < T; ok3[j] = clip_ok[j] && s + 3 < T; }
        lstm4_step<NS, X_TYPE, OUT_TYPE, FAST, NC>(smem, 0, wf, x0, x3, c, xbase, obase, (int)tidx(s), (int)tidx(s + 3), lane, hwoff, clip_ok, save);
        lstm4_step<NS, X_TYPE, OUT_TYPE, FAST, NC>(smem, 1, wf, x1, x0, c, xbase, obase, (int)tidx(s + 1), (int)tidx(s + 4), lane, hwoff, ok1, save);
        lstm4_step<NS, X_TYPE, OUT_TYPE, FAST, NC>(smem, 0, wf, x2, x1, c, xbase, obase, (int)tidx(s + 2), (int)tidx(s + 5), lane, hwoff, ok2, save);
        lstm4_step<NS, X_TYPE, OUT_TYPE, FAST, NC>(smem, 1, wf, x3, x2, c, xbase, obase, (int)tidx(s + 3), (int)tidx(s + 6), lane, hwoff, ok3, save);
    }
}

constexpr int GP = 4 * H + 8;
constexpr int GBUF_BYTES = 16 * GP * 2;

struct LstmBwdArgs {
    const float* dout;
    const float* save;
    const bf16_t* whh_t;
    int planes;
    float* dxproj;
    int B, T;
};

#ifdef AMTX_LSTM_TIMING
__device__ unsigned long long g_lstm_prof[4];
#define LT_TICK(SLOT) do { const unsigned long long n_ = __builtin_readcyclecounter(); lt_acc[SLOT] += n_ - lt_t; lt_t = n_; } while (0)
#else
#define LT_TICK(SLOT) do {} while (0)
#endif
template <int NS>
__global__ __launch_bounds__(LTHREADS) void bilstm4_bwd_kernel(LstmBwdArgs a) {
    extern __shared__ __attribute__((aligned(16))) char smem[];
    const int tid = threadIdx.x, lane = tid & 63, wave = tid >> 6;
    const int unit = 16 * wave + (lane & 15), cg = lane >> 4;
    const int dir = blockIdx.y;
    const int b = blockIdx.x * 4 + cg;
    const bool clip_ok = b < a.B;
    const int T = a.T;

    uint4 wt[16][NS];
    {
        const uint4* w = reinterpret_cast<const uint4*>(a.whh_t) + lane;
#pragma unroll
        for (int ks = 0; ks < 16; ++ks)
#pragma unroll
            for (int p = 0; p < NS; ++p) wt[ks][p] = w[((((dir * LWAVES + wave) * 16 + ks) * NS) + p) * 64];
    }
    for (int i = tid; i < 2 * NS * GBUF_BYTES / 16; i += LTHREADS) reinterpret_cast<uint4*>(smem)[i] = make_uint4(0, 0, 0, 0);
    __syncthreads();

    const int64_t bb = clip_ok ? b : 0;
    const float* sv0 = a.save + ((bb * T) * 2 + dir) * (5 * H) + unit;
    const float* do0 = a.dout + (bb * T) * 256 + dir * H + unit;
    float* dx0 = a.dxproj + (bb * T) * 1024 + dir * 512 + unit;
    const int gwoff = (4 * cg * GP + unit) * 2;

    float dh_rec = 0.f, dc_rec = 0.f;
    auto frame = [&](int s) { return step_frame(s, T, dir == 0); };
    float n_i, n_f, n_g, n_o, n_c, n_do;
    {
        const float* sv = sv0 + (int64_t)frame(0) * (2 * 5 * H);
        n_i = sv[0]; n_f = sv[H]; n_g = sv[2 * H]; n_o = sv[3 * H]; n_c = sv[4 * H];
        n_do = do0[(int64_t)frame(0) * 256];
    }
#ifdef AMTX_LSTM_TIMING
    unsigned long long lt_acc[4] = {0, 0, 0, 0}, lt_t = __builtin_readcyclecounter();
#endif
    for (int s = 0; s < T; ++s) {
        const int t = frame(s);
        const float ig = n_i, fg = n_f, gg = n_g, og = n_o, ct = n_c, dout_t = n_do;
        {
            const int tn = frame(s + 1);
            const float* sv = sv0 + (int64_t)tn * (2 * 5 * H);
            n_i = sv[0]; n_f = sv[H]; n_g = sv[2 * H]; n_o = sv[3 * H]; n_c = sv[4 * H];
            n_do = do0[(int64_t)tn * 256];
        }
        asm volatile("" : "+v"(n_c));
        const float cp = s + 1 < T ? n_c : 0.f;
        const float dh = dout_t + dh_rec;
        const float tc = tanh_f<true>(ct);
        const float d_o = dh * tc * og * (1.f - og);
        const float dc = dc_rec + dh * og * (1.f - tc * tc);
        const float d_i = dc * gg * ig * (1.f - ig);
        const float d_g = dc * ig * (1.f - gg * gg);
        const float d_f = dc * cp * fg * (1.f - fg);
        dc_rec = dc * fg;
        const float dgv[4] = {d_i, d_f, d_g, d_o};
        char* gt = smem + (s & 1) * NS * GBUF_BYTES;
#pragma unroll
        for (int q = 0; q < 4; ++q) {
            if (clip_ok) dx0[(int64_t)t * 1024 + q * H] = dgv[q];
            uint32_t hiw, low = 0;
            if (NS == 2) split_bf16x2(dgv[q], 0.f, hiw, low);
            else hiw = pack_bf16x2(dgv[q], 0.f);
            *reinterpret_cast<unsigned short*>(gt + gwoff + q * H * 2) = (unsigned short)hiw;
            if (NS == 2) *reinterpret_cast<unsigned short*>(gt + GBUF_BYTES + gwoff + q * H * 2) = (unsigned short)low;
        }
        LT_TICK(0);
        lds_barrier();
        LT_TICK(1);
        f32x4_t acc4[4];
#pragma unroll
        for (int i = 0; i < 4; ++i) acc4[i] = (f32x4_t){0.f, 0.f, 0.f, 0.f};
#pragma unroll
        for (int k4 = 0; k4 < 16; k4 += 4) {
            uint4 gf[4][NS];
#pragma unroll
            for (int i = 0; i < 4; ++i)
#pragma unroll
                for (int p = 0; p < NS; ++p)
                    gf[i][p] = *reinterpret_cast<const uint4*>(gt + p * GBUF_BYTES + ((lane & 15) * GP + 32 * (k4 + i) + 8 * (lane >> 4)) * 2);
#pragma unroll
            for (int i = 0; i < 4; ++i) acc4[i] = mfma16(gf[i][0], wt[k4 + i][0], acc4[i]);
            if (NS == 2) {
#pragma unroll
                for (int i = 0; i < 4; ++i) acc4[i] = mfma16(gf[i][NS - 1], wt[k4 + i][0], acc4[i]);
#pragma unroll
                for (int i = 0; i < 4; ++i) acc4[i] = mfma16(gf[i][0], wt[k4 + i][NS - 1], acc4[i]);
            }
        }
        dh_rec = (acc4[0][0] + acc4[1][0]) + (acc4[2][0] + acc4[3][0]);
#ifdef AMTX_LSTM_TIMING
        asm volatile("" ::"v"(dh_rec));
        LT_TICK(2);
        lt_acc[3] += 1;
#endif
    }
#ifdef AMTX_LSTM_TIMING
    if (tid == 0 && blockIdx.x == 0 && blockIdx.y == 0)
        for (int i = 0; i < 4; ++i) atomicAdd(&g_lstm_prof[i], lt_acc[i]);
#endif
}
#if defined(AMTX_LSTM_TIMING) && !defined(AMTX_F16)
extern "C" int amtxdbg_lstm_prof(unsigned long long* out4, int reset) {
    if (hipMemcpyFromSymbol(out4, HIP_SYMBOL(g_lstm_prof), 4 * sizeof(unsigned long long)) != hipSuccess) return -1;
    if (reset) {
        unsigned long long z[4] = {0, 0, 0, 0};
        if (hipMemcpyToSymbol(HIP_SYMBOL(g_lstm_prof), z, sizeof(z)) != hipSuccess) return -1;
    }
    return 0;
}
#endif

template <int HC>
__global__ void bilstm_pack_dev_kernel(const float* __restrict__ whh_fwd, const float* __restrict__ whh_bwd, int hidden, AmtxFragPut fwd, AmtxFragPut bwd) {
    if (HC) hidden = HC;
    for (int item = blockIdx.x * blockDim.x + threadIdx.x, n = amtx_layout_bilstm_items(hidden); item < n; item += gridDim.x * blockDim.x) {
        amtx_layout_bilstm(item, whh_fwd, whh_bwd, hidden, fwd);
        amtx_layout_bilstm_transposed(item, whh_fwd, whh_bwd, hidden, bwd);
    }
}

template <int HH, int NS, int X_TYPE, int OUT_TYPE>
__global__ __launch_bounds__(512) void bilstm_stream_kernel(LstmArgs a) {
    constexpr int NU = HH / 16, UPW = NU / 8, KSN = HH / 32;
    constexpr int SGK = NS == 2 ? 2 : 4;
    constexpr int NSUB = KSN / SGK;
    constexpr int NG = UPW * 4 * NSUB;
    constexpr int HPG = HH + 8;
    constexpr int HBG = 16 * HPG * 2;
    constexpr bool FAST = true;
    constexpr int RS = 4;
// ... 228 lines not shown

    for (int s = 0; s < T; ++s) {
        ws.rewind();
        const int t = frame(s);
        float cur[UT][6];
#pragma unroll
        for (int ut = 0; ut < UT; ++ut)
#pragma unroll
            for (int q = 0; q < 6; ++q) cur[ut][q] = nv[ut][q];
        load_next(frame(s + 1));
        char* gt = smem + (s & 1) * NS * GBH;
#pragma unroll
        for (int ut = 0; ut < UT; ++ut) {
            asm volatile("" : "+v"(nv[ut][4]));
            const float cp = s + 1 < T ? nv[ut][4] : 0.f;
            const float ig = cur[ut][0], fg = cur[ut][1], gg = cur[ut][2], og = cur[ut][3], ct = cur[ut][4];
            const float dh = cur[ut][5] + dh_rec[ut];
            const float tc = tanh_f<true>(ct);
            const float d_o = dh * tc * og * (1.f - og);
            const float dc = dc_rec[ut] + dh * og * (1.f - tc * tc);
            const float d_i = dc * gg * ig * (1.f - ig);
            const float d_g = dc * ig * (1.f - gg * gg);
            const float d_f = dc * cp * fg * (1.f - fg);
            dc_rec[ut] = dc * fg;
            const float dgv[4] = {d_i, d_f, d_g, d_o};
#pragma unroll
            for (int q = 0; q < 4; ++q) {
                if (clip_ok) dx0[(int64_t)t * (8 * HH) + q * HH + 16 * ut] = dgv[q];
                uint32_t hiw, low = 0;
                if (NS == 2) split_bf16x2(dgv[q], 0.f, hiw, low);
                else hiw = pack_bf16x2(dgv[q], 0.f);
                *reinterpret_cast<unsigned short*>(gt + gwoff + (q * HH + 16 * ut) * 2) = (unsigned short)hiw;
                if (NS == 2) *reinterpret_cast<unsigned short*>(gt + GBH + gwoff + (q * HH + 16 * ut) * 2) = (unsigned short)low;
            }
        }
        lds_barrier();
        f32x4_t acc[UT];
#pragma unroll
        for (int ut = 0; ut < UT; ++ut) acc[ut] = (f32x4_t){0.f, 0.f, 0.f, 0.f};
        static_for<0, NG>([&](auto ic) {
            constexpr int gi = decltype(ic)::value;
            constexpr int ut = gi / (KSN / SGK), sub = gi % (KSN / SGK);
            constexpr bool pinned = PINB && (gi & 3) == 0;
            constexpr int si = PINB ? (gi >> 2) * 3 + (gi & 3) - 1 : gi;
            if constexpr (!pinned) {
                constexpr int sn = (si + RS - 1) % NSGB;
                constexpr int gn = PINB ? (sn / 3) * 4 + 1 + sn % 3 : sn;
                ws.load_group(gn, w[sn % RS]);
            }
            static_for<0, SGK>([&](auto kc) {
                constexpr int k = decltype(kc)::value;
                constexpr int ks = sub * SGK + k;
                uint4 gf[NS];
#pragma unroll
                for (int p = 0; p < NS; ++p)
                    gf[p] = *reinterpret_cast<const uint4*>(gt + p * GBH + groff + 32 * ks * 2);
                uint4 w0, w1;
                if constexpr (pinned) { w0 = wpin[gi >> 2][k][0]; w1 = wpin[gi >> 2][k][NS - 1]; }
                else { w0 = w[si % RS][k][0]; w1 = w[si % RS][k][NS - 1]; }
                acc[ut] = mfma16(gf[0], w0, acc[ut]);
                if constexpr (NS == 2) {
                    acc[ut] = mfma16(gf[NS - 1], w0, acc[ut]);
                    acc[ut] = mfma16(gf[0], w1, acc[ut]);
                }
            });
            __builtin_amdgcn_sched_barrier(0);
        });
#pragma unroll
        for (int ut = 0; ut < UT; ++ut) dh_rec[ut] = acc[ut][0];
    }
}


struct LstmSwitches { bool no8; };
const LstmSwitches& lstm_switches() {
    static const LstmSwitches sw = {getenv("AMTX_LSTM_NO8") != nullptr};
    return sw;
}

enum LstmFamily { LSTM_CLIPS4, LSTM_CLIPS8, LSTM_CLIPS16, LSTM_STREAM, LSTM_ERROR };
enum LstmInst { LSTM_BF16, LSTM_BF16_F32IO, LSTM_X3, LSTM_NO_INST };
struct LstmRouted { LstmFamily family; LstmInst inst; dim3 grid; size_t lds; int code; const char* error; };

LstmRouted lstm_route(const LstmArgs& a, const LstmSwitches& sw) {
    const bool io16 = a.x_type == AMTX_T_BF16 && a.out_type == AMTX_T_BF16, io32 = a.x_type == AMTX_T_F32 && a.out_type == AMTX_T_F32;
    const LstmInst inst = a.planes == 1 && io16 ? LSTM_BF16 : (a.planes == 1 && io32 ? LSTM_BF16_F32IO : (a.planes == 2 && io32 ? LSTM_X3 : LSTM_NO_INST));
    auto error = [](int code, const char* msg) { return LstmRouted{LSTM_ERROR, LSTM_NO_INST, dim3(), 0, code, msg}; };
    auto on = [&](LstmFamily family, int clips, size_t lds) {
        return LstmRouted{family, inst, dim3((unsigned)((a.B + clips - 1) / clips), 2, (unsigned)a.groups), lds, AMTX_OK, nullptr};
    };
    if (a.hidden != H) {
        if (a.save && a.planes != 2) return error(AMTX_ERR_ARG, "bilstm: the training forward (save) is built for the two-plane precision");
        if (a.hidden != 256 && a.hidden != 384 && a.hidden != 512) return error(AMTX_ERR_UNSUPPORTED, "bilstm: unsupported hidden size (128, 256, 384 and 512 are built)");
        if (inst != LSTM_BF16 && inst != LSTM_X3) return error(AMTX_ERR_UNSUPPORTED, "bilstm: unsupported precision/type combination");
        return on(LSTM_STREAM, 16, 2 * (size_t)a.planes * 16 * (a.hidden + 8) * 2 + (a.planes == 1 && a.hidden <= 384 ? (size_t)8 * 4 * 4096 : 0));
    }
    if (inst == LSTM_NO_INST) return error(AMTX_ERR_UNSUPPORTED, "bilstm: unsupported precision/type combination");
    const size_t lds = 2 * (size_t)a.planes * HBUF_BYTES;
    const int64_t blocks4 = (int64_t)((a.B + 3) / 4) * 2 * a.groups;
    if (a.save) return on(LSTM_CLIPS4, 4, lds);
    if (blocks4 > 1024) return on(LSTM_CLIPS16, 16, lds);
    if (!sw.no8 && a.planes == 1 && blocks4 > 256) return on(LSTM_CLIPS8, 8, lds);
    return on(LSTM_CLIPS4, 4, lds);
}

template <typename F>
int with_hidden(int hidden, F&& f) {
    switch (hidden) {
        case 256: return f(std::integral_constant<int, 256>{});
        case 384: return f(std::integral_constant<int, 384>{});
        case 512: return f(std::integral_constant<int, 512>{});
    }
    amtx_set_error("bilstm: unsupported hidden size %d (128, 256, 384 and 512 are built)", hidden);
    return AMTX_ERR_UNSUPPORTED;
}

template <typename K, typename A>
int launch_kernel(K kern, dim3 grid, size_t lds, hipStream_t stream, const A& a) {
    AMTX_GRANT_LDS(kern, lds);
    hipLaunchKernelGGL(kern, grid, dim3(LTHREADS), lds, stream, a);
    AMTX_CHECK_LAUNCH();
    return AMTX_OK;
}

template <int NS, int XT>
int launch_routed(const LstmRouted& r, const LstmArgs& a, hipStream_t stream) {
    switch (r.family) {
        case LSTM_CLIPS4: return launch_kernel(bilstm4_kernel<NS, XT, XT>, r.grid, r.lds, stream, a);
        case LSTM_CLIPS8: return launch_kernel(bilstm4_kernel<NS, XT, XT, 2>, r.grid, r.lds, stream, a);
        case LSTM_CLIPS16: return launch_kernel(bilstm_kernel<NS, XT, XT>, r.grid, r.lds, stream, a);
        case LSTM_STREAM:
            if constexpr (NS == 2 || XT == AMTX_T_BF16)
                return with_hidden(a.hidden, [&](auto hh) { return launch_kernel(bilstm_stream_kernel<decltype(hh)::value, NS, XT, XT>, r.grid, r.lds, stream, a); });
            break;
        case LSTM_ERROR: break;
    }
    amtx_set_error("bilstm: route without a kernel");
    return AMTX_ERR_UNSUPPORTED;
}

}

namespace AMTX_FMT_NS {

size_t amtx_bilstm_wfrag_elems(int hidden, int planes) { return (size_t)2 * 4 * hidden * hidden * planes; }

static_assert(16 * UB * LWAVES == H && LWAVES == AMTX_LSTM_BWD_WAVES, "W_hh fragment layouts");

void amtx_bilstm_pack_host(const float* whh_fwd, const float* whh_bwd, int hidden, int planes, bf16_t* out) {
    const AmtxFragPut put{out, planes};
    for (int item = 0, n = amtx_layout_bilstm_items(hidden); item < n; ++item) amtx_layout_bilstm(item, whh_fwd, whh_bwd, hidden, put);
}

int amtx_launch_bilstm(const LstmArgs& a, hipStream_t stream) {
    AMTX_REQUIRE(a.xproj && a.whh && a.out, "bilstm: null pointer");
    AMTX_REQUIRE(a.B > 0 && a.T > 0 && a.groups > 0, "bilstm: bad sizes");
    AMTX_REQUIRE(a.planes == 1 || a.planes == 2, "bilstm: planes must be 1 or 2");
    const LstmRouted r = lstm_route(a, lstm_switches());
    switch (r.inst) {
        case LSTM_BF16: return launch_routed<1, AMTX_T_BF16>(r, a, stream);
        case LSTM_BF16_F32IO: return launch_routed<1, AMTX_T_F32>(r, a, stream);
        case LSTM_X3: return launch_routed<2, AMTX_T_F32>(r, a, stream);
        case LSTM_NO_INST: break;
    }
    amtx_set_error("%s (hidden %d)", r.error, a.hidden);
    return r.code;
}

int amtx_launch_bilstm_pack_dev(const float* whh_fwd, const float* whh_bwd, int hidden, int planes, bf16_t* frag_fwd, bf16_t* frag_bwd, hipStream_t stream) {
    AMTX_REQUIRE(whh_fwd && whh_bwd && frag_fwd && frag_bwd && (planes == 1 || planes == 2), "bilstm pack: bad argument");
    AMTX_REQUIRE(hidden == H || hidden == 256 || hidden == 384 || hidden == 512, "bilstm pack: hidden size %d is not built (128, 256, 384, 512)", hidden);
    const AmtxFragPut fwd{frag_fwd, planes}, bwd{frag_bwd, planes};
    if (hidden == H) hipLaunchKernelGGL(bilstm_pack_dev_kernel<H>, dim3(64), dim3(256), 0, stream, whh_fwd, whh_bwd, H, fwd, bwd);
    else hipLaunchKernelGGL(bilstm_pack_dev_kernel<0>, dim3(256), dim3(256), 0, stream, whh_fwd, whh_bwd, hidden, fwd, bwd);
    AMTX_CHECK_LAUNCH();
    return AMTX_OK;
}

int amtx_launch_bilstm_bwd(const float* dout, const float* save, const bf16_t* whh_t, int hidden, int planes, float* dxproj, int B, int T, int groups,
                           hipStream_t stream) {
    AMTX_REQUIRE(groups >= 1, "bilstm backward: bad group count");
    AMTX_REQUIRE(dout && save && whh_t && dxproj, "bilstm backward: null pointer");
    AMTX_REQUIRE(B > 0 && T > 0 && (planes == 1 || planes == 2), "bilstm backward: bad sizes");
    const int64_t w_gs = (int64_t)amtx_bilstm_wfrag_elems(hidden, planes), bt = (int64_t)B * T;
    const dim3 grid((unsigned)((B + 3) / 4), 2);
    if (hidden == H) {
        for (int g = 0; g < groups; ++g) {
            const LstmBwdArgs a{dout + g * bt * 2 * H, save + g * bt * 2 * 5 * H, whh_t + g * w_gs, planes, dxproj + g * bt * 8 * H, B, T};
            const size_t lds = 2 * (size_t)planes * GBUF_BYTES;
            const int rc = planes == 2 ? launch_kernel(bilstm4_bwd_kernel<2>, grid, lds, stream, a) : launch_kernel(bilstm4_bwd_kernel<1>, grid, lds, stream, a);
            if (rc != AMTX_OK) return rc;
        }
        return AMTX_OK;
    }
    AMTX_REQUIRE(planes == 2 && (hidden == 256 || hidden == 384 || hidden == 512),
                 "bilstm backward: hidden 256 / 384 / 512 are built for the two-plane precision only (got hidden %d, planes %d)", hidden, planes);
    const LstmBwdHArgs a{dout, save, whh_t, dxproj, B, T, w_gs};
    return with_hidden(hidden, [&](auto hh) {
        return launch_kernel(bilstm_stream_bwd_kernel<decltype(hh)::value, 2>, dim3(grid.x, 2, (unsigned)groups), 2 * (size_t)planes * 5 * (4 * hidden + 8) * 2, stream, a);
    });
}

}
```

amt_tools_amd/csrc/ofmodel.hip:

```cpp

#include "amtx_kernels.h"
#include "amtx_model_common.h"
#include "amtx_pack_layouts.h"

#include <cmath>
#include <cstdlib>
#include <thread>

namespace {

struct LinearPack { DevBuf w, b; int N = 0, K = 0, n_pad = 0, k_pad = 0, groups = 0; };

#define AMTX_FMT_KERNELS(X, ns)                                                                                                    \
    X(ns, pack_linear_host) X(ns, bilstm_pack_host) X(ns, conv1_pack_host) X(ns, conv1g_pack_host) X(ns, conv3x3_pack_host)     \
    X(ns, conv3x3_gen_pack_host) X(ns, pack_conv1_dev) X(ns, pack_conv1g_dev) X(ns, pack_conv3x3_dev) X(ns, pack_conv_gen_dev)    \
    X(ns, pack_linear_dev) X(ns, launch_bilstm_pack_dev) X(ns, launch_conv1) X(ns, launch_conv3x3) X(ns, launch_conv3x3_gen)    \
    X(ns, launch_conv_stack) X(ns, launch_gemm) X(ns, launch_bilstm)
#define AMTX_KERNEL_FIELD(ns, name) decltype(&ns::amtx_##name) name;
#define AMTX_KERNEL_ENTRY(ns, name) &ns::amtx_##name,
struct KernelSet { AMTX_FMT_KERNELS(AMTX_KERNEL_FIELD, amtx_bf16) };
const KernelSet kKernelsBf16 = {AMTX_FMT_KERNELS(AMTX_KERNEL_ENTRY, amtx_bf16)};
#ifdef AMTX_WITH_F16
const KernelSet kKernelsF16 = {AMTX_FMT_KERNELS(AMTX_KERNEL_ENTRY, amtx_f16)};
#endif

enum ConvFamily { K_CONV1,
                  K_CONV,
                  K_CONVG };
struct ConvLayer { const char* name; int c_in, c_out; ConvFamily fam; size_t frag_per; };

struct ConvSwitches { bool no_convg_mc2, no_conv_fuse, x3_no_split, no_convx12m, rowmajor_a3, no_roll_epilogue; };
ConvSwitches switches_from_env() {
    auto on = [](const char* name) { return getenv(name) != nullptr; };
    return {on("AMTX_NO_CONVG_MC2"), on("AMTX_NO_CONV_FUSE"), on("AMTX_X3_NO_SPLIT"), on("AMTX_NO_CONVX12M"), on("AMTX_OF_ROWMAJOR_A3"), on("AMTX_OF_NO_ROLL_EPILOGUE")};
}

struct ConvPlan {
    ConvLayer layer[3];
    bool conv1_fused;
    bool stack;
    bool two_plane_acts;
    bool convx12; size_t c2x_per;
    bool rowmajor_a3, no_roll_epilogue;
    bool device_resync;
    int fuses_db_scale, takes_feats16;
};

ConvPlan make_conv_plan(int in_channels, int model_complexity, int precision, const ConvSwitches& sw) {
    const int ic = in_channels, nf1 = 16 * model_complexity, nf3 = 2 * nf1, pl = precision == AMTX_PREC_X3 ? 2 : 1;
    ConvPlan p{};
    const ConvFamily f3 = nf1 != 32 ? K_CONVG : K_CONV;
    const bool g_fuse1 = amtx_conv3x3_gen_can_fuse1(ic, nf1, nf1, pl);
    const ConvFamily f2 = f3 == K_CONVG || (ic > 1 && !sw.no_convg_mc2 && g_fuse1) ? K_CONVG : K_CONV;
    p.conv1_fused = f2 == K_CONVG ? g_fuse1 : 9 * ic <= 64;
    auto frag3x3 = [pl](ConvFamily f, int c_in, int c_out) { return f == K_CONVG ? amtx_conv3x3_gen_wfrag_elems(c_in, c_out, pl) : amtx_conv3x3_wfrag_elems(c_out, pl); };
    p.layer[0] = {"layer1", ic, nf1, p.conv1_fused ? f2 : K_CONV1,
                  !p.conv1_fused ? 0 : f2 == K_CONVG ? amtx_conv1g_wfrag_elems(ic, nf1, pl) : amtx_conv1_wfrag_elems(ic, pl)};
    p.layer[1] = {"layer2", nf1, nf1, f2, frag3x3(f2, nf1, nf1)};
    p.layer[2] = {"layer3", nf1, nf3, f3, frag3x3(f3, nf1, nf3)};
    p.stack = f2 == K_CONV && p.conv1_fused && ic == 1 && pl == 1 && !sw.no_conv_fuse;
    p.two_plane_acts = pl == 2 && f3 == K_CONV && p.conv1_fused && !sw.x3_no_split && (f2 == K_CONV ? ic == 1 : ic > 1 && (9 * ic + 31) / 32 <= 2);
    p.convx12 = p.two_plane_acts && f2 == K_CONVG && ic >= 2 && ic <= 8 && amtx_conv1g_tapk(ic, 2) && !sw.no_convx12m;
    p.c2x_per = frag3x3(K_CONV, nf1, nf1);
    p.rowmajor_a3 = sw.rowmajor_a3; p.no_roll_epilogue = sw.no_roll_epilogue;
    p.device_resync = f2 == K_CONVG || ic == 1;
    p.fuses_db_scale = p.conv1_fused && f2 == K_CONV && ic == 1;
    p.takes_feats16 = !(p.conv1_fused && f2 == K_CONVG && precision != AMTX_PREC_F16) ? 0 : p.convx12 ? 2 : pl == 1 && nf1 == 32 && amtx_conv1g_tapk(ic, pl);
    return p;
}

}

struct amtx_of_model {
    int dim_in, in_channels, mc, n_out, has_offsets, precision;
    int planes, act_type;
    bool f16 = false;
    const KernelSet* k = &kKernelsBf16;
    int nf1, nf2, nf3, dim_am, dim_lm, fq, kfc;
    int kfc_pad;
    int hid, xw;
    size_t hh_elems;
    ConvPlan plan;
    int n_heads;
    int n_rec;
    std::vector<std::string> head_names;
    TensorStore store{"of_model", "was not provided"};
    DevBuf pack_scratch;
    bool finalized = false;
    bool packed_once = false;
    DevBuf conv_w[3], conv_s[3];
    DevBuf conv1_w;
    DevBuf conv2_wx;
    LinearPack fc1;
    LinearPack rec_ih;
    DevBuf rec_hh;
    LinearPack rec_out;
    LinearPack pitch_out;
    LinearPack adj_ih;
    DevBuf adj_hh;
    LinearPack adj_out;
    int dim_aj;
    mutable bool prof = false;
    mutable std::vector<std::vector<hipEvent_t>> prof_events;
};

enum { ST_CONV1 = 0, ST_CONV2, ST_CONV3, ST_FC1, ST_REC_XPROJ, ST_REC_LSTM, ST_REC_HEAD, ST_PITCH_HEAD, ST_ADJ_XPROJ, ST_ADJ_LSTM,
       ST_ADJ_HEAD, ST_PIANOROLL, ST_COUNT };
static const char* kStageNames[ST_COUNT] = {"conv1", "conv2_pool", "conv3_pool", "fc1_gemm", "rec_xproj_gemm", "rec_bilstm", "rec_head_gemm",
                                            "pitch_head_gemm", "adj_xproj_gemm", "adj_bilstm", "adj_head_gemm", "pianoroll"};

namespace {

struct Workspace {
    char *a1, *a2, *a3, *e, *xp, *l1, *joint, *joint16, *xp2, *l2, *mp;
    size_t total;
};

enum ConvPath { PATH_STACK,
                PATH_CONVX12,
                PATH_CONV12, PATH_CONVG12,
                PATH_CONV1 };
struct ConvCall { ConvPath path; bool a2_in_hbm; int64_t a3_plane; };

ConvCall resolve_conv(const amtx_of_model* m, int B, int T, bool feats16) {
    const ConvPlan& p = m->plan;
    if (p.stack && amtx_conv_stack_fused_ok(B, T, m->dim_in, m->n_heads))
        return {PATH_STACK, false, p.rowmajor_a3 ? 0 : (int64_t)B * T * 64};
    return {feats16 && p.convx12 ? PATH_CONVX12 : !p.conv1_fused ? PATH_CONV1 : p.layer[1].fam == K_CONVG ? PATH_CONVG12 : PATH_CONV12, true, 0};
}

Workspace carve(const amtx_of_model* m, int B, int T, char* base) {
    Workspace w;
    const size_t es = amtx_tsize(m->act_type);
    const size_t BT = (size_t)B * T;
    const int F = m->dim_in, F2 = F / 2;
    WorkspaceCarver ws{base};
    w.a1 = ws.take(m->plan.conv1_fused ? 256 : BT * F * m->nf1 * es * m->n_heads);
    w.a2 = ws.take(resolve_conv(m, B, T, false).a2_in_hbm ? BT * F2 * m->nf2 * es * m->n_heads : 256);
    w.a3 = ws.take(BT * m->kfc_pad * es * m->n_heads);
    w.e = ws.take(BT * m->dim_am * es * m->n_heads);
    w.xp = ws.take(BT * m->xw * es * m->n_rec);
    w.l1 = ws.take(BT * m->dim_lm * es * m->n_rec);
    w.joint = ws.take(BT * m->dim_aj * sizeof(float));
    w.joint16 = ws.take(BT * (size_t)((m->dim_aj + 63) / 64 * 64) * 2 * (m->plan.two_plane_acts ? 2 : 1));
    w.xp2 = ws.take(BT * m->xw * es);
    w.l2 = ws.take(BT * m->dim_lm * es);
    w.mp = ws.take(BT * m->n_out * sizeof(float));
    w.total = ws.off;
    return w;
}

}

extern "C" int amtx_has_f16(void) {
#ifdef AMTX_WITH_F16
    return 1;
#else
    return 0;
#endif
}

extern "C" int amtx_of_model_create(amtx_of_model** out, int dim_in, int in_channels, int model_complexity, int n_out,
                                    int has_offsets, int precision) {
    AMTX_REQUIRE(out, "amtx_of_model_create: null model pointer");
    *out = nullptr;
    AMTX_REQUIRE(precision == AMTX_PREC_BF16 || precision == AMTX_PREC_X3 || precision == AMTX_PREC_F16, "amtx_of_model_create: bad precision");
    AMTX_REQUIRE(dim_in >= 4 && in_channels >= 1 && n_out > 0 && n_out % 4 == 0, "amtx_of_model_create: bad dims");
    if (precision == AMTX_PREC_F16 && !amtx_has_f16()) {
        amtx_set_error("amtx_of_model_create: precision f16 needs a library built with the half-operand kernel twins (AMTX_BUILD_F16=1 python -m amt_tools_amd.build)");
        return AMTX_ERR_UNSUPPORTED;
    }
    if (model_complexity < 2 || model_complexity > 5) {
        amtx_set_error("amtx_of_model_create: model_complexity 2 (32/32/64-channel convolutions, LSTM hidden 128), 3 (48/48/96, hidden 256) and "
                       "4 (64/64/128, hidden 384), 5 (80/80/160, hidden 512) are implemented, with or without the OnsetsFrames2 offset head (got model_complexity=%d)", model_complexity);
        return AMTX_ERR_UNSUPPORTED;
    }
    amtx_of_model* m = new amtx_of_model();
    m->dim_in = dim_in; m->in_channels = in_channels; m->mc = model_complexity; m->n_out = n_out;
    m->has_offsets = has_offsets; m->precision = precision;
    m->planes = precision == AMTX_PREC_X3 ? 2 : 1;
    m->act_type = precision == AMTX_PREC_X3 ? AMTX_T_F32 : AMTX_T_BF16;
    m->f16 = precision == AMTX_PREC_F16;
#ifdef AMTX_WITH_F16
    if (m->f16) m->k = &kKernelsF16;
#endif
    m->nf1 = 16 * model_complexity; m->nf2 = m->nf1; m->nf3 = 32 * model_complexity;
    m->dim_am = 256 * model_complexity; m->dim_lm = 256 * (model_complexity - 1);
    m->fq = dim_in / 4;
    m->kfc = m->nf3 * m->fq;
    m->kfc_pad = (m->kfc + 63) / 64 * 64;
    m->hid = m->dim_lm / 2; m->xw = 8 * m->hid;
    m->hh_elems = amtx_bilstm_wfrag_elems(m->hid, m->planes);
    m->plan = make_conv_plan(in_channels, model_complexity, precision, switches_from_env());
    m->head_names = {"onset_head"};
    if (has_offsets) m->head_names.push_back("offset_head");
    m->n_rec = (int)m->head_names.size();
    m->head_names.push_back("pitch_head");
    m->n_heads = (int)m->head_names.size();
    m->dim_aj = (m->n_rec + 1) * n_out;
    *out = m;
    return AMTX_OK;
}

extern "C" int amtx_of_model_destroy(amtx_of_model* m) {
    if (!m) return AMTX_OK;
    DevBuf* bufs[] = {&m->conv1_w, &m->conv_w[0], &m->conv_w[1], &m->conv_w[2], &m->conv_s[0], &m->conv_s[1], &m->conv_s[2], &m->conv2_wx, &m->fc1.w, &m->fc1.b,
                      &m->rec_ih.w, &m->rec_ih.b, &m->rec_hh, &m->rec_out.w, &m->rec_out.b, &m->pitch_out.w, &m->pitch_out.b,
                      &m->adj_ih.w, &m->adj_ih.b, &m->adj_hh, &m->adj_out.w, &m->adj_out.b, &m->pack_scratch};
    for (DevBuf* b : bufs) b->release();
    delete m;
    return AMTX_OK;
}

extern "C" int amtx_of_model_set_tensor(amtx_of_model* m, const char* name, const float* host_data, int64_t numel) {
    AMTX_REQUIRE(m && name && host_data && numel > 0, "amtx_of_model_set_tensor: bad argument");
    m->store.set(name, host_data, numel);
    m->finalized = false;
// ... 128 lines not shown
        lp.N = N; lp.K = K; lp.groups = groups;
        amtx_gemm_pack_dims(N, K, &lp.n_pad, &lp.k_pad);
    };
    size_linear(m->fc1, m->dim_am, m->kfc_pad, m->n_rec);
    size_linear(m->rec_ih, m->xw, m->dim_am, m->n_rec);
    size_linear(m->rec_out, m->n_out, m->dim_lm, m->n_rec);
    size_linear(m->pitch_out, m->n_out, m->kfc_pad, 1);
    size_linear(m->adj_ih, m->xw, m->dim_aj, 1);
    size_linear(m->adj_out, m->n_out, m->dim_lm, 1);
    auto linear = [&](LinearPack& lp, int grp, const float* W, int N, int K, int row0, int rows, int perm_c, int perm_f) {
        const size_t per = (size_t)lp.n_pad * lp.k_pad * pl;
        return x.linear(W, K, N, K, lp, row0, rows, perm_c, perm_f, x.template dst<bf16_t>(lp.w, per * lp.groups) + per * grp);
    };
    auto bias = [&](LinearPack& lp, int grp) { return x.template dst<float>(lp.b, (size_t)lp.N * lp.groups) + (size_t)lp.N * grp; };
    auto need_fc1 = [&](int h, const float*& w, const float*& b) {
        NEED(m->head_names[h] + ".0.fc1.0.weight", (size_t)m->dim_am * m->kfc, w);
        NEED(m->head_names[h] + ".0.fc1.0.bias", (size_t)m->dim_am, b);
        return (int)AMTX_OK;
    };
    auto need_bank = [&](const std::string& bank, int K, const float*& w, const float*& b) {
        NEED(bank + ".output_layer.weight", (size_t)m->n_out * K, w);
        NEED(bank + ".output_layer.bias", (size_t)m->n_out, b);
        return (int)AMTX_OK;
    };
    AMTX_REQUIRE(m->nf3 <= 256, "of_model: internal: scale scratch");
    float* scale;
    STEP(x.scratch(256 + (size_t)m->n_out * m->kfc_pad + m->n_out, &scale));
    float* wfold = scale + 256;
    float* bfold = wfold + (size_t)m->n_out * m->kfc_pad;

    for (int h = 0; h < nh; ++h) {
        const std::string am = m->head_names[h] + ".0";
        const float *w, *cb, *g, *be, *mu, *var;
        for (int l = 0; l < 3; ++l) {
            const ConvLayer& y = p.layer[l];
            const std::string conv = am + "." + y.name + ".0", bn = am + "." + y.name + ".1";
            NEED(conv + ".weight", (size_t)y.c_out * y.c_in * 9, w);
            NEED(conv + ".bias", (size_t)y.c_out, cb); NEED(bn + ".weight", (size_t)y.c_out, g); NEED(bn + ".bias", (size_t)y.c_out, be);
            NEED(bn + ".running_mean", (size_t)y.c_out, mu); NEED(bn + ".running_var", (size_t)y.c_out, var);
            STEP(x.bn_fold(cb, g, be, mu, var, y.c_out, scale, x.template dst<float>(m->conv_s[l], (size_t)nh * y.c_out) + (size_t)h * y.c_out));
            bf16_t* frag = x.template dst<bf16_t>(m->conv_w[l], y.frag_per * nh) + y.frag_per * h;
            if (l == 0) {
                const size_t per = (size_t)y.c_out * ic * 9;
                STEP(x.scale_rows(w, scale, y.c_out, ic * 9, x.template dst<float>(m->conv1_w, per * nh) + per * h));
                if (y.fam == K_CONVG) STEP(x.conv1g(w, scale, ic, y.c_out, frag));
                else if (y.fam == K_CONV) STEP(x.conv1(w, scale, ic, frag));
            } else if (y.fam == K_CONVG) STEP(x.conv_gen(w, scale, y.c_in, y.c_out, frag));
            else STEP(x.conv3x3(w, scale, y.c_out, frag));
            if (l == 1 && p.convx12) STEP(x.conv3x3(w, scale, y.c_out, x.template dst<bf16_t>(m->conv2_wx, p.c2x_per * nh) + p.c2x_per * h));
        }
        if (h < m->n_rec) {
            const float* fb;
            STEP(need_fc1(h, w, fb));
            STEP(linear(m->fc1, h, w, m->dim_am, m->kfc, 0, m->fc1.n_pad, m->nf3, m->fq));
            STEP(x.copy(bias(m->fc1, h), fb, m->dim_am));
        }
    }
    auto pack_rec = [&](const std::string& lstm, const std::string& bank, int dim_in, LinearPack& ih, DevBuf& hh, LinearPack& outp, int grp) {
        const float *wif, *wib, *whf, *whb, *bif, *bib, *bhf, *bhb, *wo, *bo;
        const std::string q = lstm + ".mlm.";
        NEED(q + "weight_ih_l0", (size_t)G * dim_in, wif); NEED(q + "weight_ih_l0_reverse", (size_t)G * dim_in, wib);
        NEED(q + "weight_hh_l0", (size_t)G * m->hid, whf); NEED(q + "weight_hh_l0_reverse", (size_t)G * m->hid, whb);
        NEED(q + "bias_ih_l0", (size_t)G, bif); NEED(q + "bias_ih_l0_reverse", (size_t)G, bib);
        NEED(q + "bias_hh_l0", (size_t)G, bhf); NEED(q + "bias_hh_l0_reverse", (size_t)G, bhb);
        STEP(linear(ih, grp, wif, G, dim_in, 0, G, 0, 0));
        STEP(linear(ih, grp, wib, G, dim_in, G, ih.n_pad - G, 0, 0));
        STEP(x.vec_add(bif, bhf, G, bias(ih, grp)));
        STEP(x.vec_add(bib, bhb, G, bias(ih, grp) + G));
        STEP(x.bilstm(whf, whb, x.template dst<bf16_t>(hh, m->hh_elems * ih.groups) + m->hh_elems * grp));
        STEP(need_bank(bank, m->dim_lm, wo, bo));
        STEP(linear(outp, grp, wo, m->n_out, m->dim_lm, 0, outp.n_pad, 0, 0));
        STEP(x.copy(bias(outp, grp), bo, m->n_out));
        return (int)AMTX_OK;
    };
    for (int r = 0; r < m->n_rec; ++r) STEP(pack_rec(m->head_names[r] + ".1", m->head_names[r] + ".2", m->dim_am, m->rec_ih, m->rec_hh, m->rec_out, r));
    {
        const float *wo, *bo, *w1, *b1;
        STEP(need_bank("pitch_head.1", m->dim_am, wo, bo));
        STEP(need_fc1(nh - 1, w1, b1));
        STEP(x.head_fold(wo, w1, b1, bo, wfold, bfold));
        STEP(linear(m->pitch_out, 0, wfold, m->n_out, m->kfc_pad, 0, m->pitch_out.n_pad, 0, 0));
        STEP(x.copy(bias(m->pitch_out, 0), bfold, m->n_out));
    }
    return pack_rec("adjoin.0", "adjoin.1", m->dim_aj, m->adj_ih, m->adj_hh, m->adj_out, 0);
}

}

extern "C" int amtx_of_model_finalize(amtx_of_model* m) {
    AMTX_REQUIRE(m, "amtx_of_model_finalize: null model");
    STEP(amtx_quiesce_before_resync(m->packed_once));
    if (m->plan.layer[2].fam == K_CONVG && (!amtx_conv3x3_gen_ntc(m->nf1, m->nf2) || !amtx_conv3x3_gen_ntc(m->nf2, m->nf3))) {
        amtx_set_error("of_model: no convolution kernel for %d -> %d -> %d channels", m->nf1, m->nf2, m->nf3);
        return AMTX_ERR_UNSUPPORTED;
    }
    HostPack x{m};
    STEP(pack_model(m, x));
    DevBuf* order[] = {&m->conv1_w, &m->conv_s[0], &m->conv_w[0], &m->conv_w[1], &m->conv2_wx, &m->conv_s[1], &m->conv_w[2], &m->conv_s[2],
                       &m->fc1.w, &m->fc1.b, &m->rec_ih.w, &m->rec_ih.b, &m->rec_hh, &m->rec_out.w, &m->rec_out.b, &m->pitch_out.w, &m->pitch_out.b,
                       &m->adj_ih.w, &m->adj_ih.b, &m->adj_hh, &m->adj_out.w, &m->adj_out.b};
    for (DevBuf* b : order) {
        const std::vector<char>& v = x.image[b];
        if (!v.empty()) STEP(b->upload(v.data(), v.size()));
    }
    m->store.host.clear();
    m->finalized = true;
    m->packed_once = true;
    return AMTX_OK;
}

extern "C" int amtx_of_model_set_tensor_device(amtx_of_model* m, const char* name, const float* device_data, int64_t numel) {
    AMTX_REQUIRE(m && name && device_data && numel > 0, "amtx_of_model_set_tensor_device: bad argument");
    m->store.set_device(name, device_data, numel);
    return AMTX_OK;
}

extern "C" int amtx_of_model_finalize_device(amtx_of_model* m, void* stream_) {
    AMTX_REQUIRE(m, "amtx_of_model_finalize_device: null model");
    struct Clear {
        amtx_of_model* m;
        ~Clear() { m->store.device.clear(); }
    } clear{m};
    AMTX_REQUIRE(m->finalized, "amtx_of_model_finalize_device: the first sync goes through amtx_of_model_finalize (it allocates the packed buffers)");
    if (!m->plan.device_resync) {
        amtx_set_error("amtx_of_model_finalize_device: no device packer for conv.hip's multi-channel first conv; use amtx_of_model_finalize");
        return AMTX_ERR_UNSUPPORTED;
    }
    DevicePack x{m, (hipStream_t)stream_, true};
    STEP(pack_model(m, x));
    STEP(amtx_quiesce_before_resync(m->packed_once));
    x.dry = false;
    const int rc = pack_model(m, x);
    if (rc != AMTX_OK) m->finalized = false;
    return rc;
}

extern "C" size_t amtx_of_workspace_bytes(const amtx_of_model* m, int batch, int num_frames) {
    if (!m || batch <= 0 || num_frames <= 0) return 0;
    return carve(m, batch, num_frames, nullptr).total;
}

static GemmArgs gemm_args(const void* A, int64_t lda, int a_type, const LinearPack& lp, int planes, void* C, int64_t ldc, int c_type,
                          int64_t M, int groups, int64_t a_gs, int64_t c_gs) {
    GemmArgs g;
    g.A = A; g.lda = lda; g.a_type = a_type;
    g.W = (const bf16_t*)lp.w.p; g.n_pad = lp.n_pad; g.k_pad = lp.k_pad; g.planes = planes;
    g.bias = (const float*)lp.b.p;
    g.C = C; g.ldc = ldc; g.c_type = c_type;
    g.M = M; g.N = lp.N; g.K = lp.K;
    g.groups = groups; g.a_gs = a_gs; g.w_gs = (int64_t)lp.n_pad * lp.k_pad * planes; g.bias_gs = lp.N; g.c_gs = c_gs;
    return g;
}

struct FeatsIn { const float* feats; const void* feats16; int64_t stride_b, stride_c, stride_t, stride_f; const float *clip_max, *ref; };

template <class Mark>
static int run_convs(const amtx_of_model* m, const ConvCall& call, const FeatsIn& in, const Workspace& w, int B, int T, hipStream_t s, Mark&& mark) {
    const ConvPlan& p = m->plan;
    const KernelSet* k = m->k;
    const int64_t BT = (int64_t)B * T;
    const int F = m->dim_in, F2 = F / 2, at = m->act_type, pl = m->planes, nh = m->n_heads;
    int rc;
    if (call.path == PATH_CONV1) {
        Conv1Args c1;
        c1.in = in.feats; c1.stride_b = in.stride_b; c1.stride_c = in.stride_c; c1.stride_t = in.stride_t; c1.stride_f = in.stride_f;
        c1.w = (const float*)m->conv1_w.p; c1.shift = (const float*)m->conv_s[0].p; c1.out = w.a1; c1.out_type = at;
        c1.B = B; c1.T = T; c1.F = F; c1.c_in = m->in_channels; c1.c_out = m->nf1;
        c1.groups = nh; c1.w_gs = (int64_t)m->nf1 * m->in_channels * 9; c1.shift_gs = m->nf1; c1.out_gs = BT * F * m->nf1;
        if ((rc = k->launch_conv1(c1, s)) != AMTX_OK) return rc;
    }
    mark();
    ConvArgs c2;
    c2.in = w.a1; c2.in_type = at; c2.wfrag = (const bf16_t*)m->conv_w[1].p; c2.planes = pl; c2.shift = (const float*)m->conv_s[1].p;
    c2.out = w.a2; c2.out_type = at; c2.B = B; c2.T = T; c2.F = F; c2.c_out = m->nf2;
    c2.groups = nh; c2.in_gs = BT * F * m->nf1; c2.shift_gs = m->nf2; c2.w_gs = (int64_t)p.layer[1].frag_per; c2.out_gs = BT * F2 * m->nf2;
    const int64_t a2_split = BT * F2 * m->nf2 * nh, a3_split = BT * m->kfc_pad * nh;
    if (p.two_plane_acts) { c2.out_type = AMTX_T_SPLIT; c2.out_split = a2_split; }
    if (p.conv1_fused) {
        c2.in = nullptr;
        c2.feats = in.feats; c2.f_stride_b = in.stride_b; c2.f_stride_c = in.stride_c; c2.f_stride_t = in.stride_t; c2.f_stride_f = in.stride_f;
        c2.c_in = m->in_channels; c2.w1frag = (const bf16_t*)m->conv_w[0].p; c2.shift1 = (const float*)m->conv_s[0].p; c2.w1_gs = (int64_t)p.layer[0].frag_per;
        c2.f_clip_max = in.clip_max; c2.f_ref = in.ref;
        if (in.feats16) { c2.feats = nullptr; c2.feats16 = in.feats16; }
    }
    if (call.path == PATH_CONVX12) { c2.in_split = BT * F * 8; c2.wfrag = (const bf16_t*)m->conv2_wx.p; c2.w_gs = (int64_t)p.c2x_per; }
    if (call.path == PATH_STACK)
        rc = k->launch_conv_stack(c2, (const bf16_t*)m->conv_w[2].p, (int64_t)p.layer[2].frag_per, (const float*)m->conv_s[2].p, w.a3, BT * m->kfc_pad, call.a3_plane, s);
    else if (call.path == PATH_CONVX12) rc = amtx_launch_convx12(c2, s);
    else rc = p.layer[1].fam == K_CONVG ? k->launch_conv3x3_gen(c2, m->nf1, s) : k->launch_conv3x3(c2, s);
    if (rc != AMTX_OK) return rc;
    mark();
    ConvArgs c3 = c2;
    c3.feats = nullptr; c3.feats16 = nullptr; c3.w1frag = nullptr; c3.shift1 = nullptr; c3.c_in = 0;
    c3.in = w.a2; c3.wfrag = (const bf16_t*)m->conv_w[2].p; c3.shift = (const float*)m->conv_s[2].p; c3.out = w.a3;
    c3.F = F2; c3.c_out = m->nf3; c3.in_gs = BT * F2 * m->nf2; c3.w_gs = (int64_t)p.layer[2].frag_per; c3.shift_gs = m->nf3; c3.out_gs = BT * m->kfc_pad;
    if (p.two_plane_acts) { c3.in_type = AMTX_T_SPLIT; c3.in_split = a2_split; c3.out_type = AMTX_T_SPLIT; c3.out_split = a3_split; }
    if (m->kfc_pad != m->kfc) {
        AMTX_REQUIRE(p.layer[2].fam == K_CONVG, "amtx_of_forward: internal: padded fc1 rows need the general conv kernel");
        c3.out_ts = m->kfc_pad;
        const size_t es = amtx_tsize(at);
        if ((rc = amtx_launch_zero_cols(w.a3 + (size_t)m->kfc * es, (int64_t)m->kfc_pad * es, (int)((m->kfc_pad - m->kfc) * es), BT * nh, s)) != AMTX_OK) return rc;
    }
    if (call.path != PATH_STACK && (rc = p.layer[2].fam == K_CONVG ? k->launch_conv3x3_gen(c3, m->nf2, s) : k->launch_conv3x3(c3, s)) != AMTX_OK) return rc;
    mark();
    return AMTX_OK;
}

static int of_forward_impl(const amtx_of_model* m, const FeatsIn& in, int B, int T, void* workspace, size_t workspace_bytes, float* out_onsets,
                           float* out_multi_pitch, float* logits_onsets, float* logits_multi_pitch, float* logits_pitch_head, void* stream_) {
    AMTX_REQUIRE(m && m->finalized, "amtx_of_forward: model not finalized");
    AMTX_REQUIRE(!in.clip_max || m->plan.fuses_db_scale, "amtx_of_forward_power: this model does not stage its features in the conv kernel");
    AMTX_REQUIRE(!in.feats16 || m->plan.takes_feats16, "amtx_of_forward_feats16: this model does not stage 16-bit channels-last features");
    AMTX_REQUIRE((in.feats || in.feats16) && workspace, "amtx_of_forward: null pointer");
    AMTX_REQUIRE(B > 0 && T > 0, "amtx_of_forward: bad batch/num_frames");
    Workspace w = carve(m, B, T, (char*)workspace);
    AMTX_REQUIRE(workspace_bytes >= w.total, "amtx_of_forward: workspace too small (%zu < %zu)", workspace_bytes, w.total);
    AMTX_REQUIRE(((uintptr_t)workspace % 256) == 0, "amtx_of_forward: workspace must be 256-byte aligned");
    hipStream_t s = (hipStream_t)stream_;
    const int64_t BT = (int64_t)B * T;
    const int at = m->act_type, pl = m->planes;
    const KernelSet* k = m->k;
    int rc;
    std::vector<hipEvent_t>* evs = nullptr;
    if (m->prof) {
        m->prof_events.emplace_back();
        evs = &m->prof_events.back();
    }
    auto mark = [&]() {
        if (!evs) return;
        hipEvent_t e;
        if (hipEventCreate(&e) == hipSuccess) { (void)hipEventRecord(e, s); evs->push_back(e); }
    };
    mark();

    const ConvCall call = resolve_conv(m, B, T, in.feats16 != nullptr);
    if ((rc = run_convs(m, call, in, w, B, T, s, mark)) != AMTX_OK) return rc;
    const bool sp = m->plan.two_plane_acts, no_roll_epi = m->plan.no_roll_epilogue;
    const int64_t a3_plane = call.a3_plane, a3_split = BT * m->kfc_pad * m->n_heads, e_split = BT * m->dim_am * m->n_heads;

    const int at_d = sp ? AMTX_T_SPLIT : at;
    GemmArgs g = gemm_args(w.a3, m->kfc_pad, at_d, m->fc1, pl, w.e, m->dim_am, at_d, BT, m->n_rec, BT * m->kfc_pad, BT * m->dim_am);
    g.a_plane = a3_plane; g.a_split = a3_split; g.c_split = e_split;
    if ((rc = k->launch_gemm(g, s)) != AMTX_OK) return rc;
    mark();

    g = gemm_args(w.e, m->dim_am, at_d, m->rec_ih, pl, w.xp, m->xw, at, BT, m->n_rec, BT * m->dim_am, BT * m->xw);
    g.a_split = e_split;
    if ((rc = k->launch_gemm(g, s)) != AMTX_OK) return rc;
    mark();
    LstmArgs l;
    l.xproj = w.xp; l.x_type = at; l.whh = (const bf16_t*)m->rec_hh.p; l.planes = pl; l.out = w.l1; l.out_type = at;
    l.B = B; l.T = T; l.groups = m->n_rec; l.x_gs = BT * m->xw; l.w_gs = (int64_t)m->hh_elems; l.out_gs = BT * m->dim_lm;
    l.hidden = m->hid;
    if ((rc = k->launch_bilstm(l, s)) != AMTX_OK) return rc;
    mark();
    g = gemm_args(w.l1, m->dim_lm, at, m->rec_out, pl, w.joint, m->dim_aj, AMTX_T_F32, BT, m->n_rec, BT * m->dim_lm, m->n_out);
    const bool roll_on = out_onsets && !no_roll_epi && amtx_gemm_has_roll_epilogue(g);
    if (roll_on) { g.roll_out = out_onsets; g.roll_T = T; g.roll_thr = 0.5f; g.roll_group = 0; }
    const int kp = (m->dim_aj + 63) / 64 * 64;
    GemmArgs gp = gemm_args(w.a3 + (size_t)(m->n_heads - 1) * BT * m->kfc_pad * (sp ? 2 : amtx_tsize(at)), m->kfc_pad, at_d, m->pitch_out, pl,
                            w.joint + (size_t)m->n_rec * m->n_out * sizeof(float), m->dim_aj, AMTX_T_F32, BT, 1, 0, 0);
    gp.a_plane = a3_plane; gp.a_split = a3_split;
    const bool copy_on = pl == 1 && !no_roll_epi && amtx_gemm_has_roll_epilogue(g) && amtx_gemm_has_roll_epilogue(gp) && m->n_out % 4 == 0 &&
                         (kp - m->dim_aj) % 4 == 0 && gp.N + (kp - m->dim_aj) <= gp.n_pad;
    if (copy_on) {
        g.copy16 = (bf16_t*)w.joint16; g.copy16_ld = kp; g.copy16_col0 = 0; g.copy16_gs = m->n_out; g.copy16_pad = 0;
        gp.copy16 = (bf16_t*)w.joint16; gp.copy16_ld = kp; gp.copy16_col0 = m->n_rec * m->n_out; gp.copy16_gs = 0; gp.copy16_pad = kp - m->dim_aj;
        if (roll_on && !logits_onsets && !logits_pitch_head && !m->has_offsets) { g.C = nullptr; gp.C = nullptr; }
    }
    if ((rc = k->launch_gemm(g, s)) != AMTX_OK) return rc;
    mark();
    if ((rc = k->launch_gemm(gp, s)) != AMTX_OK) return rc;
    mark();

    if (pl == 1) {
        if (!copy_on && (rc = amtx_launch_cvt_pad_bf16((const float*)w.joint, m->dim_aj, m->dim_aj, (bf16_t*)w.joint16, kp, BT, s, m->f16)) != AMTX_OK) return rc;
        g = gemm_args(w.joint16, kp, AMTX_T_BF16, m->adj_ih, pl, w.xp2, m->xw, at, BT, 1, 0, 0);
        g.K = kp;
    } else if (sp) {
        if ((rc = amtx_launch_cvt_split((const float*)w.joint, m->dim_aj, m->dim_aj, (bf16_t*)w.joint16, kp, BT * kp, BT, s)) != AMTX_OK) return rc;
        g = gemm_args(w.joint16, kp, AMTX_T_SPLIT, m->adj_ih, pl, w.xp2, m->xw, at, BT, 1, 0, 0);
        g.K = kp; g.a_split = BT * kp;
    } else {
        g = gemm_args(w.joint, m->dim_aj, AMTX_T_F32, m->adj_ih, pl, w.xp2, m->xw, at, BT, 1, 0, 0);
    }
    if ((rc = k->launch_gemm(g, s)) != AMTX_OK) return rc;
    mark();
    l.xproj = w.xp2; l.whh = (const bf16_t*)m->adj_hh.p; l.out = w.l2; l.groups = 1;
    if ((rc = k->launch_bilstm(l, s)) != AMTX_OK) return rc;
    mark();
    g = gemm_args(w.l2, m->dim_lm, at, m->adj_out, pl, w.mp, m->n_out, AMTX_T_F32, BT, 1, 0, 0);
    const bool roll_mp = out_multi_pitch && !no_roll_epi && amtx_gemm_has_roll_epilogue(g);
    if (roll_mp) {
        g.roll_out = out_multi_pitch; g.roll_T = T; g.roll_thr = 0.5f; g.roll_group = 0;
        if (!logits_multi_pitch) g.C = nullptr;
    }
    if ((rc = k->launch_gemm(g, s)) != AMTX_OK) return rc;
    mark();

    if (out_onsets && !roll_on && (rc = amtx_launch_pianoroll((const float*)w.joint, m->dim_aj, 0, B, T, m->n_out, 0.5f, out_onsets, s)) != AMTX_OK) return rc;
    if (out_multi_pitch && !roll_mp && (rc = amtx_launch_pianoroll((const float*)w.mp, m->n_out, 0, B, T, m->n_out, 0.5f, out_multi_pitch, s)) != AMTX_OK) return rc;

    mark();
    const size_t row = (size_t)m->n_out * sizeof(float);
    if (logits_onsets)
        AMTX_CHECK_HIP(hipMemcpy2DAsync(logits_onsets, row, w.joint, (size_t)m->dim_aj * 4, row, BT, hipMemcpyDeviceToDevice, s));
    if (logits_pitch_head)
        AMTX_CHECK_HIP(hipMemcpy2DAsync(logits_pitch_head, row, w.joint + (size_t)m->n_rec * row, (size_t)m->dim_aj * 4, row, BT,
                                        hipMemcpyDeviceToDevice, s));
    if (logits_multi_pitch)
        AMTX_CHECK_HIP(hipMemcpyAsync(logits_multi_pitch, w.mp, row * BT, hipMemcpyDeviceToDevice, s));
    return AMTX_OK;
}

extern "C" int amtx_of_fuses_db_scale(const amtx_of_model* m) { return m && m->finalized && m->plan.fuses_db_scale; }
extern "C" int amtx_of_conv_stack_fused(const amtx_of_model* m, int batch, int num_frames) { return m && resolve_conv(m, batch, num_frames, false).path == PATH_STACK; }

extern "C" int amtx_of_forward(const amtx_of_model* m, const float* feats, int64_t stride_b, int64_t stride_c, int64_t stride_t,
                               int64_t stride_f, int batch, int num_frames, void* workspace, size_t workspace_bytes,
                               float* out_onsets, float* out_multi_pitch, float* logits_onsets, float* logits_multi_pitch,
                               float* logits_pitch_head, void* stream_) {
    return of_forward_impl(m, {feats, nullptr, stride_b, stride_c, stride_t, stride_f, nullptr, nullptr}, batch, num_frames, workspace, workspace_bytes,
                           out_onsets, out_multi_pitch, logits_onsets, logits_multi_pitch, logits_pitch_head, stream_);
}

extern "C" int amtx_of_forward_power(const amtx_of_model* m, const float* power, int64_t stride_b, int64_t stride_t, int64_t stride_f,
                                     const float* clip_max, const float* ref, int batch, int num_frames, void* workspace,
                                     size_t workspace_bytes, float* out_onsets, float* out_multi_pitch, float* logits_onsets,
                                     float* logits_multi_pitch, float* logits_pitch_head, void* stream_) {
    AMTX_REQUIRE(clip_max, "amtx_of_forward_power: clip_max is null");
    return of_forward_impl(m, {power, nullptr, stride_b, 0, stride_t, stride_f, clip_max, ref}, batch, num_frames, workspace, workspace_bytes,
                           out_onsets, out_multi_pitch, logits_onsets, logits_multi_pitch, logits_pitch_head, stream_);
}

extern "C" int amtx_of_takes_feats16(const amtx_of_model* m) { return m && m->finalized ? m->plan.takes_feats16 : 0; }

extern "C" int amtx_of_forward_feats16(const amtx_of_model* m, const void* feats16, int batch, int num_frames, void* workspace, size_t workspace_bytes,
                                       float* out_onsets, float* out_multi_pitch, float* logits_onsets, float* logits_multi_pitch,
                                       float* logits_pitch_head, void* stream_) {
    AMTX_REQUIRE(feats16, "amtx_of_forward_feats16: feats16 is null");
    return of_forward_impl(m, {nullptr, feats16, 0, 0, 0, 0, nullptr, nullptr}, batch, num_frames, workspace, workspace_bytes, out_onsets, out_multi_pitch,
                           logits_onsets, logits_multi_pitch, logits_pitch_head, stream_);
}

extern "C" int amtx_of_offsets(const amtx_of_model* m, void* workspace, size_t workspace_bytes, int batch, int num_frames, float* out_offsets,
                               float* logits_offsets, void* stream_) {
    AMTX_REQUIRE(m && m->finalized, "amtx_of_offsets: model not finalized");
    AMTX_REQUIRE(m->has_offsets, "amtx_of_offsets: the model has no offset head");
    AMTX_REQUIRE(workspace && batch > 0 && num_frames > 0, "amtx_of_offsets: bad argument");
    Workspace w = carve(m, batch, num_frames, (char*)workspace);
    AMTX_REQUIRE(workspace_bytes >= w.total, "amtx_of_offsets: workspace too small");
    hipStream_t s = (hipStream_t)stream_;
    const int64_t BT = (int64_t)batch * num_frames;
    int rc;
    if (out_offsets && (rc = amtx_launch_pianoroll((const float*)w.joint, m->dim_aj, m->n_out, batch, num_frames, m->n_out, -1.0f, out_offsets, s)) != AMTX_OK)
        return rc;
    const size_t row = (size_t)m->n_out * sizeof(float);
    if (logits_offsets)
        AMTX_CHECK_HIP(hipMemcpy2DAsync(logits_offsets, row, w.joint + row, (size_t)m->dim_aj * 4, row, BT, hipMemcpyDeviceToDevice, s));
    return AMTX_OK;
}

extern "C" int amtx_of_num_stages(void) { return ST_COUNT; }
extern "C" const char* amtx_of_stage_name(int i) { return (i >= 0 && i < ST_COUNT) ? kStageNames[i] : ""; }

extern "C" int amtx_of_profile_enable(amtx_of_model* m, int enable) {
    AMTX_REQUIRE(m, "amtx_of_profile_enable: null model");
    for (auto& v : m->prof_events)
        for (hipEvent_t e : v) (void)hipEventDestroy(e);
    m->prof_events.clear();
    m->prof = enable != 0;
    return AMTX_OK;
}

extern "C" int amtx_of_profile_read(amtx_of_model* m, double* stage_ms, int* num_forwards) {
    AMTX_REQUIRE(m && stage_ms && num_forwards, "amtx_of_profile_read: null argument");
    for (int i = 0; i < ST_COUNT; ++i) stage_ms[i] = 0.0;
    *num_forwards = 0;
    for (auto& v : m->prof_events) {
        if ((int)v.size() != ST_COUNT + 1) continue;
        AMTX_CHECK_HIP(hipEventSynchronize(v.back()));
        for (int i = 0; i < ST_COUNT; ++i) {
            float ms = 0.f;
            AMTX_CHECK_HIP(hipEventElapsedTime(&ms, v[i], v[i + 1]));
            stage_ms[i] += ms;
        }
        ++*num_forwards;
    }
    return AMTX_OK;
}
```

amt_tools_amd/models.py:

```python

import ctypes as C

import numpy as np
import os

import torch
import torch.nn.functional as F
from torch import nn

from . import _lib, tools

__all__ = ['TranscriptionModel', 'OutputLayer', 'LogisticBank', 'AcousticModel', 'LanguageModel', 'OnsetsFrames',
           'SpectralFrontend']


class TranscriptionModel(nn.Module):

    def __init__(self, dim_in, profile, in_channels=1, model_complexity=1, frame_width=1, device='cpu'):
        nn.Module.__init__(self)
        self.dim_in = dim_in
        self.profile = profile
        self.in_channels = in_channels
        self.model_complexity = model_complexity
        self.frame_width = frame_width
# ... 215 lines not shown

    def __init__(self, module):
        super().__init__()
        self.module = module

    def forward(self, audio):
        assert audio.dim() == 3 and audio.shape[1] == 1
        from .features import _SpecPlanOwner
        if isinstance(self.module, _SpecPlanOwner):
            feats = self.module.process_batch(audio[:, 0].float(), model_layout=True)
            return feats.transpose(-1, -2)
        return self.module.process_batch(audio[:, 0].float())


def _pick_side_stream(device, candidates=6, spins=20, spin_cycles=20000):
    import time
    sleep = getattr(torch.cuda, '_sleep', None)
    main = torch.cuda.current_stream(device)
    first = None
    try:
        with torch.cuda.device(device):
            def chains(streams):
                torch.cuda.synchronize(device)
                t0 = time.perf_counter()
                for st in streams:
                    with torch.cuda.stream(st):
                        for _ in range(spins):
                            sleep(spin_cycles)
                for st in streams:
                    st.synchronize()
                return time.perf_counter() - t0
            for _ in range(candidates):
                s = torch.cuda.Stream(device=device)
                first = first or s
                if sleep is None:
                    return s
                chains((main, s))
                one = min(chains((main,)) for _ in range(2))
                if min(chains((main, s)) for _ in range(2)) < 1.7 * one:
                    return s
    except Exception:
        pass
    return first or torch.cuda.Stream(device=device)


class PendingFeatures(object):

    def __init__(self, module, power, clip_max, ref=None):
        self.module, self.power, self.clip_max, self.ref = module, power, clip_max, ref

    @property
    def device(self):
        return self.power.device

    def materialize(self):
        return self.module.scale_batch(self.power, self.clip_max, self.ref, model_layout=True)


class PendingFeatures16(PendingFeatures):

    def __init__(self, module, feats16, audio):
        self.module, self.feats16, self.audio = module, feats16, audio

    @property
    def device(self):
        return self.feats16.device

    def materialize(self):
        return self.module.process_batch(self.audio).transpose(-1, -2)


class _EngineBase(object):

    ABI = None

    def __init__(self, device, *create_args):
        self.device = device
        self.handle = C.c_void_p()
        _lib.call(self.ABI + '_create', C.byref(self.handle), *create_args, device=device)
        self.version = None
        self.workspace = None

    def sync_weights(self, model):
        items = [(k, v) for k, v in model.state_dict().items() if v.dtype.is_floating_point and not k.startswith('frontend.') and v.numel() > 0]
        version = tuple((k, v._version, v.data_ptr()) for k, v in items)
        if version == self.version:
            return
        if self.version is None or not self._resync_on_device(items):
            flat = torch.cat([v.detach().reshape(-1).to(torch.float32) for _, v in items]).cpu().numpy()
            off = 0
            for k, v in items:
                n = v.numel()
                _lib.call(self.ABI + '_set_tensor', self.handle, k.encode(), flat[off:off + n], n)
                off += n
            _lib.call(self.ABI + '_finalize', self.handle, device=self.device)
        self.version = version

    def _resync_on_device(self, items):
        return False

    def _grow_workspace(self, need, device):
        if self.workspace is None or self.workspace.numel() < need:
            self.workspace = None
            self.workspace = _lib.alloc_workspace(need, device)

    def __del__(self):
        try:
            _lib.call(self.ABI + '_destroy', self.handle)
        except Exception:
            pass


class _OFEngine(_EngineBase):

    ABI = 'amtx_of_model'

    def __init__(self, model, device):
        self.n_out = model.profile.get_range_len()
        super().__init__(device, int(model.dim_in), int(model.in_channels), int(model.model_complexity), int(self.n_out),
                         int(model.has_offsets), {'bf16': 0, 'x3': 1, 'f16': 2}[model.precision])
        self.device_sync = os.environ.get('AMTX_HOST_WEIGHT_SYNC') is None
        self.device_syncs = 0

    def _resync_on_device(self, items):
        if not (self.device_sync and all(v.is_cuda and v.device == torch.device(self.device) and v.dtype == torch.float32 for _, v in items)):
            return False
        keep = []
        for k, v in items:
            t = v.detach()
            t = t if t.is_contiguous() else t.contiguous()
            keep.append(t)
            _lib.call('amtx_of_model_set_tensor_device', self.handle, k.encode(), t, t.numel())
        with torch.cuda.device(self.device):
            rc = _lib.lib().amtx_of_model_finalize_device(self.handle, _lib.current_stream(self.device))
            if keep and rc == 0:
                torch.cuda.current_stream(self.device).synchronize()
        del keep
        if rc == 0:
            self.device_syncs += 1
            return True
        if rc != _lib.ERR_UNSUPPORTED:
            _lib.check(rc, 'amtx_of_model_finalize_device')
        self.device_sync = False
        return False

    def fuses_db_scale(self):
        return bool(_lib.call('amtx_of_fuses_db_scale', self.handle))

    def takes_feats16(self):
        return int(_lib.call('amtx_of_takes_feats16', self.handle))

    def conv_stack_fused(self, batch, num_frames):
        return bool(_lib.call('amtx_of_conv_stack_fused', self.handle, int(batch), int(num_frames)))

    def forward(self, feats, want_logits=True):
        pending = feats if isinstance(feats, PendingFeatures) else None
        pending16 = isinstance(pending, PendingFeatures16)
        if pending16:
            feats = pending.feats16
            B, T = feats.shape[-4], feats.shape[-3]
        elif pending is not None:
            feats = pending.power.unsqueeze(1)
        if not pending16:
            B, Cc, T, Fd = feats.shape
        self._grow_workspace(_lib.call('amtx_of_workspace_bytes', self.handle, B, T), feats.device)
        n_out = self.n_out
        opts = dict(dtype=torch.float32, device=feats.device)
        onsets = torch.empty((B, n_out, T), **opts)
        multi_pitch = torch.empty((B, n_out, T), **opts)
        lo = torch.empty((B, T, n_out), **opts) if want_logits else None
        lm = torch.empty((B, T, n_out), **opts) if want_logits else None
        lp = torch.empty((B, T, n_out), **opts) if want_logits else None
        sb, sc, st, sf = (0, 0, 0, 0) if pending16 else feats.stride()
        ws, outs = self.workspace, (onsets, multi_pitch, lo, lm, lp)
        if pending16:
            _lib.call('amtx_of_forward_feats16', self.handle, feats, B, T, ws, ws.numel(), *outs, device=feats.device)
        elif pending is not None:
            _lib.call('amtx_of_forward_power', self.handle, feats, sb, st, sf, pending.clip_max, pending.ref, B, T, ws, ws.numel(), *outs,
                      device=feats.device)
        else:
            _lib.call('amtx_of_forward', self.handle, feats, sb, sc, st, sf, B, T, ws, ws.numel(), *outs, device=feats.device)
        self._last = (B, T)
        return onsets, multi_pitch, lo, lm, lp

    def offsets(self, device, want_logits=True):
        B, T = self._last
        opts = dict(dtype=torch.float32, device=device)
        prob = torch.empty((B, self.n_out, T), **opts)
        logits = torch.empty((B, T, self.n_out), **opts) if want_logits else None
        _lib.call('amtx_of_offsets', self.handle, self.workspace, self.workspace.numel(), B, T, prob, logits, device=device)
        return prob, logits


class OnsetsFrames(TranscriptionModel):

    has_offsets = False

    def __init__(self, dim_in, profile, in_channels=1, model_complexity=2, detach_heads=False, device='cpu',
                 precision='x3'):
        super().__init__(dim_in, profile, in_channels, model_complexity, 1, device)
        assert precision in ('bf16', 'x3', 'f16')
        self.detach_heads = detach_heads
        self.precision = precision
        self.dim_am = 256 * self.model_complexity
        self.dim_lm = 256 * (self.model_complexity - 1)
        dim_out = self.profile.get_range_len()
        self.onset_head = nn.Sequential(AcousticModel(self.dim_in, self.dim_am, self.in_channels, self.model_complexity),
                                        LanguageModel(self.dim_am, self.dim_lm), LogisticBank(self.dim_lm, dim_out))
        self.pitch_head = nn.Sequential(AcousticModel(self.dim_in, self.dim_am, self.in_channels, self.model_complexity),
                                        LogisticBank(self.dim_am, dim_out))
        self.dim_aj = 2 * dim_out
        self.adjoin = nn.Sequential(LanguageModel(self.dim_aj, self.dim_lm), LogisticBank(self.dim_lm, dim_out))

    _engine_class = _OFEngine
    _transient = TranscriptionModel._transient + ('_engine_out', '_engine_offsets', '_side_stream', '_overlap_armed', '_fb_last_forward',
                                                  '_overlap_latched_off')

    def pre_proc(self, batch):
        pending = self._deferred_scale(batch) if self.__dict__.get('_in_run_on_batch') else None
        if pending is not None:
            return pending
        batch = super().pre_proc(batch)
        batch[tools.KEY_FEATS] = batch[tools.KEY_FEATS].transpose(-1, -2)
        return batch

    def _deferred_scale(self, batch):
        if self.training or len(self.frontend) != 1 or not isinstance(self.frontend[0], SpectralFrontend):
            return None
        if os.environ.get('AMTX_DEFER_DB_SCALE', '1') == '0':
            return None
        from .features import _SpecPlanOwner, _CqtPlanOwner
        module = self.frontend[0].module
        cqt = isinstance(module, _CqtPlanOwner)
        if cqt:
            if os.environ.get('AMTX_CQT_FEATS16', '1') == '0':
                return None
        elif not isinstance(module, _SpecPlanOwner) or not getattr(module, 'decibels', False):
            return None
        if tools.query_dict(batch, tools.KEY_FEATS) or not tools.query_dict(batch, tools.KEY_AUDIO):
            return None
        if torch.device(self.device).type != 'cuda':
            return None
        batch = tools.dict_to_device(batch, self.device)
        audio = batch[tools.KEY_AUDIO]
        from .tracks import TrackClips
        if isinstance(audio, TrackClips):
            if cqt or not self._get_engine(audio.device).fuses_db_scale():
                return None
            power, track_max = self._clips_module(audio).power_clips(audio)
            batch[tools.KEY_FEATS] = PendingFeatures(module, power, clip_max=track_max)
            return batch
        if not (torch.is_tensor(audio) and audio.is_cuda and audio.dim() == 2):
            return None
        if cqt:
            form = self._get_engine(audio.device).takes_feats16()
            if not form:
                return None
            if int(getattr(module, 'n_bins', -1)) != int(self.dim_in) or int(module.get_num_channels()) != int(self.in_channels):
                return None
            audio = audio.float()
            batch[tools.KEY_FEATS] = PendingFeatures16(module, module.process_batch16(audio, split=(form == 2)), audio)
            return batch
        if not self._get_engine(audio.device).fuses_db_scale():
            return None
        power, clip_max = module.power_batch(audio.float())
        batch[tools.KEY_FEATS] = PendingFeatures(module, power, clip_max)
        return batch

    def run_on_batch(self, batch):
        labelled = any(tools.query_dict(batch, k) for k in (tools.KEY_MULTIPITCH, tools.KEY_ONSETS, tools.KEY_OFFSETS))
        self.__dict__['_logits_wanted'] = labelled
        self.__dict__['_in_run_on_batch'] = True
        try:
            return super().run_on_batch(batch)
        finally:
            self.__dict__.pop('_logits_wanted', None)
            self.__dict__.pop('_in_run_on_batch', None)

    def forward(self, feats):
        pending = isinstance(feats, PendingFeatures)
        if pending and self.training:
            feats, pending = feats.materialize(), False
        if pending or (feats.is_cuda and not self.training):
            eng = self._get_engine(feats.device)
            if not pending and feats.dtype != torch.float32:
                feats = feats.float()
            want = self.__dict__.get('_logits_wanted', True)
            onsets_bin, mp_bin, lo, lm, lp = eng.forward(feats if pending else feats.detach(), want_logits=want)
            if not want:
                lo, lm = onsets_bin, mp_bin
            output = {tools.KEY_ONSETS: lo, tools.KEY_MULTIPITCH: lm}
            self.__dict__['_engine_out'] = (lo, lm, onsets_bin, mp_bin, lp)
            if self.has_offsets:
                prob, logits = eng.offsets(feats.device, want_logits=want)
                output[tools.KEY_OFFSETS] = logits if want else prob
                self.__dict__['_engine_offsets'] = (output[tools.KEY_OFFSETS], prob)
            return output
        self.__dict__.pop('_engine_out', None)
        self.__dict__.pop('_engine_offsets', None)
        output = dict()
        fb0 = None
        if feats.is_cuda and self.training and torch.is_grad_enabled():
            from . import autograd as _ag
            fb0 = _ag.fallback_total()
        if self._overlap_heads(feats):
            main = torch.cuda.current_stream(feats.device)
# ... 381 lines not shown
```

Baseline: 40.59 million.

## Write LSTM input projections in gate-interleaved tiled layout for BiLSTM reads

The input-projection GEMMs feeding both BiLSTM stages now permute weight rows so the four gates of each hidden unit sit next to each other, and they write bf16 output in a 16-row tiled chunk layout. The BiLSTM kernel gains a tiled reader that fetches all four gate values for a cell in one 8-byte load, replacing four scattered row-major loads per timestep. This targets the memory latency on the recurrent critical path. The price is extra layout plumbing, constraints on M, N and the GEMM route, and an env switch to fall back to row-major.

```diff
diff --git a/amt_tools_amd/_lib.py b/amt_tools_amd/_lib.py
--- a/amt_tools_amd/_lib.py
+++ b/amt_tools_amd/_lib.py
@@ -6,6 +6,8 @@
 LIB_PATH = os.environ.get('AMTX_LIB_PATH') or os.path.join(_HERE, 'csrc', 'libamtx.so')
 HEADER_PATH = os.path.join(os.path.dirname(_HERE), 'include', 'amtx.h')
 EXTRA_HEADERS = ('amtx_tracks.h',)
+
+QUERY_HEADERS = ('amtx_xp.h',)
 
 _lib = None
 
@@ -110,6 +112,17 @@
     return _extra_signatures
 
 
+def query_signatures():
+    table = {}
+    with open(HEADER_PATH) as f:
+        base = f.read()
+    for header in QUERY_HEADERS:
+        with open(os.path.join(os.path.dirname(HEADER_PATH), header)) as f:
+            both = parse_header(base + '\n' + f.read())
+        table.update({name: row for name, row in both.items() if name not in signatures()})
+    return table
+
+
 _funcs = {}
 
 
@@ -127,6 +140,7 @@
         bound = dict(signatures())
         for table in extra_signatures().values():
             bound.update(table)
+        bound.update(query_signatures())
         for name, (letters, stream) in bound.items():
             try:
                 fn = getattr(handle, name)
diff --git a/amt_tools_amd/csrc/amtx_kernels.h b/amt_tools_amd/csrc/amtx_kernels.h
--- a/amt_tools_amd/csrc/amtx_kernels.h
+++ b/amt_tools_amd/csrc/amtx_kernels.h
@@ -20,6 +20,8 @@
     int64_t a_plane = 0;
     int64_t a_valid_lo = 0, a_valid_hi = 0;
     int64_t a_split = 0, c_split = 0;
+    int c_tiled = 0;
+    int n_gate_shift = 0;
 };
 constexpr int AMTX_GEMM_MULTI_MAX = 10;
 struct GemmMulti { GemmArgs p[AMTX_GEMM_MULTI_MAX]; int n; };
@@ -91,6 +93,7 @@
     int groups; int64_t x_gs, w_gs, out_gs;
     int hidden = 128;
     float* save = nullptr;
+    int x_tiled = 0;
 };
 
 namespace amtx_bf16 {
diff --git a/amt_tools_amd/csrc/amtx_kernels_fmt.h b/amt_tools_amd/csrc/amtx_kernels_fmt.h
--- a/amt_tools_amd/csrc/amtx_kernels_fmt.h
+++ b/amt_tools_amd/csrc/amtx_kernels_fmt.h
@@ -1,5 +1,6 @@
 
 bool amtx_gemm_has_roll_epilogue(const GemmArgs& g);
+bool amtx_gemm_writes_tiled_c(const GemmArgs& g);
 int amtx_launch_gemm(const GemmArgs& g, hipStream_t stream);
 int amtx_launch_gemm_multi(const GemmArgs* gs, int n, hipStream_t stream);
 void amtx_gemm_pack_dims(int N, int K, int* n_pad, int* k_pad);
@@ -25,6 +26,7 @@
 bool amtx_conv3x3_gen_can_fuse1(int c_in, int c_mid, int c_out, int planes);
 
 int amtx_launch_bilstm(const LstmArgs& l, hipStream_t stream);
+bool amtx_lstm_reads_tiled_x(const LstmArgs& l);
 size_t amtx_bilstm_wfrag_elems(int hidden, int planes);
 void amtx_bilstm_pack_host(const float* whh_fwd, const float* whh_bwd, int hidden, int planes, bf16_t* out);
 int amtx_launch_bilstm_pack_dev(const float* whh_fwd, const float* whh_bwd, int hidden, int planes, bf16_t* frag_fwd, bf16_t* frag_bwd, hipStream_t stream);
diff --git a/amt_tools_amd/csrc/amtx_pack_layouts.h b/amt_tools_amd/csrc/amtx_pack_layouts.h
--- a/amt_tools_amd/csrc/amtx_pack_layouts.h
+++ b/amt_tools_amd/csrc/amtx_pack_layouts.h
@@ -134,6 +134,17 @@
     for (int j = 0; j < 8; ++j) put((size_t)(row0 + n) * k_pad + k0 + j, n < N && k0 + j < K ? src[(int64_t)j * step] : 0.0f);
 }
 
+static inline __host__ __device__ int amtx_xp_gate_row(int n, int shift) {
+    const int h = 1 << shift, r = n & (4 * h - 1);
+    return (n - r) + (r & 3) * h + (r >> 2);
+}
+constexpr int AMTX_XP_CHUNK = 2048;
+static inline __host__ __device__ int amtx_xp_piece(int h, int g, int m) { return h * (AMTX_XP_CHUNK / 2) + (m * 4 + g) * 16; }
+static inline __host__ __device__ int64_t amtx_xp_tile_byte(int64_t R, int n, int N) {
+    const int64_t chunk = (R >> 4) * (N / 64) + n / 64;
+    return chunk * AMTX_XP_CHUNK + amtx_xp_piece((n % 16) / 8, (n % 64) / 16, (int)(R & 15)) + (n % 8) * 2;
+}
+
 static inline __host__ __device__ int amtx_layout_bilstm_items(int hidden) { return hidden * hidden; }
 template <class Put>
 static inline __host__ __device__ void amtx_layout_bilstm(int item, const float* whh_fwd, const float* whh_bwd, int hidden, const Put& put) {
diff --git a/amt_tools_amd/csrc/gemm.hip b/amt_tools_amd/csrc/gemm.hip
--- a/amt_tools_amd/csrc/gemm.hip
+++ b/amt_tools_amd/csrc/gemm.hip
@@ -1,5 +1,6 @@
 
 #include "amtx_kernels.h"
+#include "amtx_pack_layouts.h"
 
 #include <algorithm>
 #include <cstdlib>
@@ -413,7 +414,7 @@
 constexpr int RING_MAX_NPAD = 4096;
 constexpr int ROP = RTB * RBK * 2;
 constexpr int RSTAGE = 2 * ROP;
-__device__ uint4 g_gemm_trash[4];
+__device__ uint4 g_gemm_trash[128];
 
 __device__ __forceinline__ int rswz(int q) { return (0x78 >> (q * 2)) & 3; }
 
@@ -445,7 +446,7 @@
     const bf16_t* Wbase = g.W + (int64_t)grp * g.w_gs;
     char* Cbase = reinterpret_cast<char*>(g.C) + (int64_t)grp * g.c_gs * ES;
     float* bias_l = reinterpret_cast<float*>(smem + RST * RSTAGE);
-    for (int i = tid; i < g.n_pad; i += 512) bias_l[i] = (g.bias && i < g.N) ? g.bias[(int64_t)grp * g.bias_gs + i] : 0.f;
+    for (int i = tid; i < g.n_pad; i += 512) bias_l[i] = (g.bias && i < g.N) ? g.bias[(int64_t)grp * g.bias_gs + amtx_xp_gate_row(i, g.n_gate_shift)] : 0.f;
 
     const bf16_t* a_src[2];
     const bf16_t* w_src[2];
@@ -459,7 +460,7 @@
             int64_t mr = tm0 + row;                                                                           \
             if (mr >= g.M) mr = g.M - 1;                                                                      \
             a_src[n] = Abase + mr * g.lda + ((lane & 3) ^ rswz((row >> 2) & 3)) * 8;                          \
-            w_src[n] = Wbase + (int64_t)(tn0 + row) * g.k_pad + ((lane & 3) ^ rswz((row >> 4) & 3)) * 8;      \
+            w_src[n] = Wbase + (int64_t)amtx_xp_gate_row(tn0 + row, g.n_gate_shift) * g.k_pad + ((lane & 3) ^ rswz((row >> 4) & 3)) * 8; \
         }                                                                                                     \
     } while (0)
     const unsigned lds_base = __builtin_amdgcn_readfirstlane((unsigned)(uintptr_t)(lds_void_t*)smem) + wave * 2048;
@@ -577,16 +578,20 @@
             const int n0 = (lg % nbn) * RTB;
             const int64_t m0 = (int64_t)(lg / nbn) * RTB;
             const int nb = n0 + wn * 64 + 16 * (lane >> 4);
+            const bool tiled = C_TYPE == AMTX_T_BF16 && g.c_tiled != 0;
+            const int col_bytes = tiled ? AMTX_XP_CHUNK / 64 : ES, hstep = tiled ? amtx_xp_piece(1, 0, 0) : 16;
+            const int64_t lane_off = tiled ? (int64_t)amtx_xp_piece(0, lane >> 4, lane & 15) : ((lane & 15) * g.ldc + 16 * (lane >> 4)) * ES;
+            char* const ctile_base = Cbase + (int64_t)(n0 + wn * 64) * col_bytes + lane_off;
             f32x4_t bv[4];
 #pragma unroll
             for (int nt = 0; nt < 4; ++nt) bv[nt] = *reinterpret_cast<const f32x4_t*>(bias_l + nb + 4 * nt);
 #pragma unroll
             for (int mt = 0; mt < MT; ++mt) {
-                const int64_t m = m0 + wm * 128 + mt * 16 + (lane & 15);
+                const int64_t mrow = m0 + wm * 128 + mt * 16, m = mrow + (lane & 15);
 #ifdef AMTX_PP_NOSTORE
                 char* dst = reinterpret_cast<char*>(g_gemm_trash);
 #else
-                char* dst = m < g.M ? Cbase + (m * g.ldc + nb) * ES : reinterpret_cast<char*>(g_gemm_trash);
+                char* dst = m < g.M ? ctile_base + mrow * g.ldc * ES : reinterpret_cast<char*>(g_gemm_trash);
 #endif
                 float o[4][4];
 #pragma unroll
@@ -599,8 +604,8 @@
                 } else {
 #pragma unroll
                     for (int h = 0; h < 2; ++h)
-                        reinterpret_cast<uint4*>(dst)[h] = make_uint4(pack_bf16x2(o[2 * h][0], o[2 * h][1]), pack_bf16x2(o[2 * h][2], o[2 * h][3]),
-                                                                     pack_bf16x2(o[2 * h + 1][0], o[2 * h + 1][1]), pack_bf16x2(o[2 * h + 1][2], o[2 * h + 1][3]));
+                        *reinterpret_cast<uint4*>(dst + h * hstep) = make_uint4(pack_bf16x2(o[2 * h][0], o[2 * h][1]), pack_bf16x2(o[2 * h][2], o[2 * h][3]),
+                                                                               pack_bf16x2(o[2 * h + 1][0], o[2 * h + 1][1]), pack_bf16x2(o[2 * h + 1][2], o[2 * h + 1][3]));
                 }
 #pragma unroll
                 for (int nt = 0; nt < 4; ++nt) acc[nt][mt] = (f32x4_t){0.f, 0.f, 0.f, 0.f};
@@ -1250,6 +1255,8 @@
 
 static bool route_has_roll_epilogue(GemmRoute r, const GemmArgs& g) { return (r == ROUTE_SKINNY || r == ROUTE_GLDS128) && g.c_type == AMTX_T_F32; }
 bool amtx_gemm_has_roll_epilogue(const GemmArgs& g) { return route_has_roll_epilogue(gemm_route(g, gemm_switches()).route, g); }
+static bool route_writes_tiled_c(GemmRoute r, const GemmArgs& g) { return r == ROUTE_PP && g.c_type == AMTX_T_BF16 && g.N % 64 == 0; }
+bool amtx_gemm_writes_tiled_c(const GemmArgs& g) { return route_writes_tiled_c(gemm_route(g, gemm_switches()).route, g); }
 
 int amtx_launch_gemm(const GemmArgs& g, hipStream_t stream) {
     if (const int rc = gemm_validate(g); rc != AMTX_OK) return rc;
@@ -1262,6 +1269,10 @@
     AMTX_REQUIRE(g.C || g.pair_map || g.roll_out || g.copy16, "gemm: no output");
     AMTX_REQUIRE(!g.roll_out || roll_epilogue, "gemm: the piano-roll epilogue exists on the bf16 direct-to-LDS path with fp32 C only");
     AMTX_REQUIRE(!g.roll_out || (g.roll_T > 0 && g.M % g.roll_T == 0 && g.M < (1ll << 31)), "gemm: piano-roll epilogue: M must be clips x frames");
+    AMTX_REQUIRE(!g.c_tiled || (route_writes_tiled_c(r.route, g) && g.M % 16 == 0 && g.ldc == g.N && g.C),
+                 "gemm: tiled C exists on the two-group ring with 16-bit C, N a multiple of 64, M a multiple of 16 and ldc = N");
+    AMTX_REQUIRE(!g.n_gate_shift || (r.route == ROUTE_PP && g.n_gate_shift > 0 && g.n_gate_shift < 20 && g.N % (4 << g.n_gate_shift) == 0 && g.N == g.n_pad),
+                 "gemm: gate-interleaved columns exist on the two-group ring, N a multiple of 4 << shift without pad rows");
     const bool c16 = g.c_type == AMTX_T_BF16;
     switch (r.route) {
         case ROUTE_ERROR: amtx_set_error("%s", r.error); return AMTX_ERR_ARG;
diff --git a/amt_tools_amd/csrc/lstm.hip b/amt_tools_amd/csrc/lstm.hip
--- a/amt_tools_amd/csrc/lstm.hip
+++ b/amt_tools_amd/csrc/lstm.hip
@@ -223,9 +223,31 @@
     }
 }
 
-template <int NS, int X_TYPE, int OUT_TYPE, bool FAST, int NC>
-__device__ __forceinline__ void lstm4_step(char* smem, int cur, const uint4 (&wf)[4][4][NS], const typename XScalar<X_TYPE>::type (&xcur)[NC][4],
-                                           typename XScalar<X_TYPE>::type (&xnext)[NC][4], float (&c)[NC], const char* const (&xbase)[NC],
+template <int X_TYPE, int NC>
+struct XCellRows {
+    typedef typename XScalar<X_TYPE>::type raw_t[4];
+    const char* xbase[NC];
+    __device__ __forceinline__ void load(int j, int t, raw_t& dst) const { load_x4<X_TYPE>(xbase[j], (int64_t)t * 1024, dst); }
+    static __device__ __forceinline__ float gate(const raw_t& x, int q, int lane) { return unpack_xs(x[q], lane & 1); }
+};
+template <int NC>
+struct XCellTiles {
+    typedef uint2 raw_t;
+    const char* base;
+    int r0[NC];
+    __device__ __forceinline__ void load(int j, int t, raw_t& dst) const {
+        const int R = r0[j] + t;
+        dst = *reinterpret_cast<const uint2*>(base + (int64_t)(R >> 4) * (16 * AMTX_XP_CHUNK) + (R & 15) * amtx_xp_piece(0, 0, 1));
+    }
+    static __device__ __forceinline__ float gate(const raw_t& x, int q, int) {
+        const unsigned w = q < 2 ? x.x : x.y;
+        return (q & 1) ? unpack16_hi(w) : unpack16_lo(w);
+    }
+};
+
+template <int NS, int OUT_TYPE, bool FAST, int NC, class XL>
+__device__ __forceinline__ void lstm4_step(char* smem, int cur, const uint4 (&wf)[4][4][NS], const typename XL::raw_t (&xcur)[NC],
+                                           typename XL::raw_t (&xnext)[NC], float (&c)[NC], const XL& xl,
                                            char* const (&obase)[NC], int t, int tnext, int lane, const int (&hwoff)[NC], const bool (&clip_ok)[NC],
                                            float* save) {
     constexpr int RSTEP = 4 / NC;
@@ -238,14 +260,14 @@
             hf[ks][p] = *reinterpret_cast<const uint4*>(hb + p * HBUF_BYTES + ((lane & 15) * HP + 32 * ks + 8 * (lane >> 4)) * 2);
 
 #pragma unroll
-    for (int j = 0; j < NC; ++j) load_x4<X_TYPE>(xbase[j], (int64_t)tnext * 1024, xnext[j]);
+    for (int j = 0; j < NC; ++j) xl.load(j, tnext, xnext[j]);
 
     f32x4_t acc[4];
 #pragma unroll
     for (int q = 0; q < 4; ++q) {
         acc[q] = (f32x4_t){0.f, 0.f, 0.f, 0.f};
 #pragma unroll
-        for (int j = 0; j < NC; ++j) acc[q][RSTEP * j] = unpack_xs(xcur[j][q], lane & 1);
+        for (int j = 0; j < NC; ++j) acc[q][RSTEP * j] = XL::gate(xcur[j], q, lane);
     }
 #pragma unroll
     for (int ks = 0; ks < 4; ++ks) {
@@ -291,10 +313,35 @@
     lds_barrier();
 }
 
+template <int NS, int OUT_TYPE, bool FAST, int NC, class XL>
+__device__ __forceinline__ void bilstm4_walk(char* smem, const uint4 (&wf)[4][4][NS], float (&c)[NC], const XL xl, char* const (&obase)[NC], const int& T,
+                                             const int& dir, int lane, const int (&hwoff)[NC], const bool (&clip_ok)[NC], float* save) {
+    typename XL::raw_t x0[NC], x1[NC], x2[NC], x3[NC];
+    auto tidx = [&](int s) { return step_frame(s, T, dir); };
+#pragma unroll
+    for (int j = 0; j < NC; ++j) {
+        xl.load(j, tidx(0), x0[j]);
+        xl.load(j, tidx(1), x1[j]);
+        xl.load(j, tidx(2), x2[j]);
+    }
+    __syncthreads();
+
+    for (int s = 0; s < T; s += 4) {
+        bool ok1[NC], ok2[NC], ok3[NC];
+#pragma unroll
+        for (int j = 0; j < NC; ++j) { ok1[j] = clip_ok[j] && s + 1 < T; ok2[j] = clip_ok[j] && s + 2 < T; ok3[j] = clip_ok[j] && s + 3 < T; }
+        lstm4_step<NS, OUT_TYPE, FAST, NC>(smem, 0, wf, x0, x3, c, xl, obase, tidx(s), tidx(s + 3), lane, hwoff, clip_ok, save);
+        lstm4_step<NS, OUT_TYPE, FAST, NC>(smem, 1, wf, x1, x0, c, xl, obase, tidx(s + 1), tidx(s + 4), lane, hwoff, ok1, save);
+        lstm4_step<NS, OUT_TYPE, FAST, NC>(smem, 0, wf, x2, x1, c, xl, obase, tidx(s + 2), tidx(s + 5), lane, hwoff, ok2, save);
+        lstm4_step<NS, OUT_TYPE, FAST, NC>(smem, 1, wf, x3, x2, c, xl, obase, tidx(s + 3), tidx(s + 6), lane, hwoff, ok3, save);
+    }
+}
+
 template <int NS, int X_TYPE, int OUT_TYPE, int NC = 1>
 __global__ __launch_bounds__(LTHREADS) void bilstm4_kernel(LstmArgs a) {
     extern __shared__ __attribute__((aligned(16))) char smem[];
     constexpr bool FAST = true;
+    constexpr int XES = X_TYPE == AMTX_T_BF16 ? 2 : 4;
     const int tid = threadIdx.x, lane = tid & 63, wave = tid >> 6;
     const int unit = 16 * wave + (lane & 15), cg = lane >> 4;
     const int dir = blockIdx.y, grp = blockIdx.z;
@@ -314,7 +361,7 @@
 
     float c[NC];
     bool clip_ok[NC];
-    const char* xbase[NC];
+    int bclip[NC];
     char* obase[NC];
     int hwoff[NC];
     float* save = nullptr;
@@ -322,35 +369,28 @@
     for (int j = 0; j < NC; ++j) {
         const int b = (blockIdx.x * 4 + cg) * NC + j;
         clip_ok[j] = b < a.B;
+        bclip[j] = clip_ok[j] ? b : 0;
         c[j] = 0.f;
-        xbase[j] = reinterpret_cast<const char*>(a.xproj) +
-                   ((int64_t)grp * a.x_gs + (int64_t)(clip_ok[j] ? b : 0) * T * 1024 + dir * 512 + (X_TYPE == AMTX_T_BF16 ? (unit & ~1) : unit)) *
-                       (X_TYPE == AMTX_T_BF16 ? 2 : 4);
-        obase[j] = reinterpret_cast<char*>(a.out) +
-                   ((int64_t)grp * a.out_gs + (int64_t)(clip_ok[j] ? b : 0) * T * 256 + dir * 128 + unit) * (OUT_TYPE == AMTX_T_BF16 ? 2 : 4);
+        obase[j] = reinterpret_cast<char*>(a.out) + ((int64_t)grp * a.out_gs + (int64_t)bclip[j] * T * 256 + dir * 128 + unit) * (OUT_TYPE == AMTX_T_BF16 ? 2 : 4);
         hwoff[j] = ((4 * cg + (4 / NC) * j) * HP + unit) * 2;
-        if (NC == 1) save = a.save ? a.save + (((int64_t)grp * a.B + (clip_ok[j] ? b : 0)) * T * 2 + dir) * (5 * H) + unit : nullptr;
-    }
-
-    typename XScalar<X_TYPE>::type x0[NC][4], x1[NC][4], x2[NC][4], x3[NC][4];
-    auto tidx = [&](int s) { return (int64_t)step_frame(s, T, dir); };
-#pragma unroll
-    for (int j = 0; j < NC; ++j) {
-        load_x4<X_TYPE>(xbase[j], tidx(0) * 1024, x0[j]);
-        load_x4<X_TYPE>(xbase[j], tidx(1) * 1024, x1[j]);
-        load_x4<X_TYPE>(xbase[j], tidx(2) * 1024, x2[j]);
-    }
-    __syncthreads();
-
-    for (int s = 0; s < T; s += 4) {
-        bool ok1[NC], ok2[NC], ok3[NC];
-#pragma unroll
-        for (int j = 0; j < NC; ++j) { ok1[j] = clip_ok[j] && s + 1 < T; ok2[j] = clip_ok[j] && s + 2 < T; ok3[j] = clip_ok[j] && s + 3 < T; }
-        lstm4_step<NS, X_TYPE, OUT_TYPE, FAST, NC>(smem, 0, wf, x0, x3, c, xbase, obase, (int)tidx(s), (int)tidx(s + 3), lane, hwoff, clip_ok, save);
-        lstm4_step<NS, X_TYPE, OUT_TYPE, FAST, NC>(smem, 1, wf, x1, x0, c, xbase, obase, (int)tidx(s + 1), (int)tidx(s + 4), lane, hwoff, ok1, save);
-        lstm4_step<NS, X_TYPE, OUT_TYPE, FAST, NC>(smem, 0, wf, x2, x1, c, xbase, obase, (int)tidx(s + 2), (int)tidx(s + 5), lane, hwoff, ok2, save);
-        lstm4_step<NS, X_TYPE, OUT_TYPE, FAST, NC>(smem, 1, wf, x3, x2, c, xbase, obase, (int)tidx(s + 3), (int)tidx(s + 6), lane, hwoff, ok3, save);
-    }
+        if (NC == 1) save = a.save ? a.save + (((int64_t)grp * a.B + bclip[j]) * T * 2 + dir) * (5 * H) + unit : nullptr;
+    }
+    const char* xgrp = reinterpret_cast<const char*>(a.xproj) + (int64_t)grp * a.x_gs * XES;
+
+    if constexpr (NS == 1 && X_TYPE == AMTX_T_BF16) {
+        if (a.x_tiled) {
+            XCellTiles<NC> xl;
+            xl.base = xgrp + amtx_xp_tile_byte(0, dir * 512 + 4 * unit, 1024);
+#pragma unroll
+            for (int j = 0; j < NC; ++j) xl.r0[j] = bclip[j] * T;
+            bilstm4_walk<NS, OUT_TYPE, FAST, NC>(smem, wf, c, xl, obase, T, dir, lane, hwoff, clip_ok, save);
+            return;
+        }
+    }
+    XCellRows<X_TYPE, NC> xl;
+#pragma unroll
+    for (int j = 0; j < NC; ++j) xl.xbase[j] = xgrp + ((int64_t)bclip[j] * T * 1024 + dir * 512 + (X_TYPE == AMTX_T_BF16 ? (unit & ~1) : unit)) * XES;
+    bilstm4_walk<NS, OUT_TYPE, FAST, NC>(smem, wf, c, xl, obase, T, dir, lane, hwoff, clip_ok, save);
 }
 
 constexpr int GP = 4 * H + 8;
@@ -885,11 +925,18 @@
     for (int item = 0, n = amtx_layout_bilstm_items(hidden); item < n; ++item) amtx_layout_bilstm(item, whh_fwd, whh_bwd, hidden, put);
 }
 
+static bool route_reads_tiled_x(const LstmRouted& r, const LstmArgs& a) {
+    return (r.family == LSTM_CLIPS4 || r.family == LSTM_CLIPS8) && r.inst == LSTM_BF16 && !a.save;
+}
+bool amtx_lstm_reads_tiled_x(const LstmArgs& a) { return route_reads_tiled_x(lstm_route(a, lstm_switches()), a); }
+
 int amtx_launch_bilstm(const LstmArgs& a, hipStream_t stream) {
     AMTX_REQUIRE(a.xproj && a.whh && a.out, "bilstm: null pointer");
     AMTX_REQUIRE(a.B > 0 && a.T > 0 && a.groups > 0, "bilstm: bad sizes");
     AMTX_REQUIRE(a.planes == 1 || a.planes == 2, "bilstm: planes must be 1 or 2");
     const LstmRouted r = lstm_route(a, lstm_switches());
+    AMTX_REQUIRE(!a.x_tiled || (route_reads_tiled_x(r, a) && ((int64_t)a.B * a.T) % 16 == 0),
+                 "bilstm: tiled xproj exists for the four- and eight-clip launches with one plane, 16-bit xproj, no save and B T a multiple of 16");
     switch (r.inst) {
         case LSTM_BF16: return launch_routed<1, AMTX_T_BF16>(r, a, stream);
         case LSTM_BF16_F32IO: return launch_routed<1, AMTX_T_F32>(r, a, stream);
diff --git a/amt_tools_amd/csrc/ofmodel.hip b/amt_tools_amd/csrc/ofmodel.hip
--- a/amt_tools_amd/csrc/ofmodel.hip
+++ b/amt_tools_amd/csrc/ofmodel.hip
@@ -15,7 +15,7 @@
     X(ns, pack_linear_host) X(ns, bilstm_pack_host) X(ns, conv1_pack_host) X(ns, conv1g_pack_host) X(ns, conv3x3_pack_host)     \
     X(ns, conv3x3_gen_pack_host) X(ns, pack_conv1_dev) X(ns, pack_conv1g_dev) X(ns, pack_conv3x3_dev) X(ns, pack_conv_gen_dev)    \
     X(ns, pack_linear_dev) X(ns, launch_bilstm_pack_dev) X(ns, launch_conv1) X(ns, launch_conv3x3) X(ns, launch_conv3x3_gen)    \
-    X(ns, launch_conv_stack) X(ns, launch_gemm) X(ns, launch_bilstm)
+    X(ns, launch_conv_stack) X(ns, launch_gemm) X(ns, launch_bilstm) X(ns, gemm_writes_tiled_c) X(ns, lstm_reads_tiled_x)
 #define AMTX_KERNEL_FIELD(ns, name) decltype(&ns::amtx_##name) name;
 #define AMTX_KERNEL_ENTRY(ns, name) &ns::amtx_##name,
 struct KernelSet { AMTX_FMT_KERNELS(AMTX_KERNEL_FIELD, amtx_bf16) };
@@ -29,10 +29,11 @@
                   K_CONVG };
 struct ConvLayer { const char* name; int c_in, c_out; ConvFamily fam; size_t frag_per; };
 
-struct ConvSwitches { bool no_convg_mc2, no_conv_fuse, x3_no_split, no_convx12m, rowmajor_a3, no_roll_epilogue; };
+struct ConvSwitches { bool no_convg_mc2, no_conv_fuse, x3_no_split, no_convx12m, rowmajor_a3, no_roll_epilogue, rowmajor_xp; };
 ConvSwitches switches_from_env() {
     auto on = [](const char* name) { return getenv(name) != nullptr; };
-    return {on("AMTX_NO_CONVG_MC2"), on("AMTX_NO_CONV_FUSE"), on("AMTX_X3_NO_SPLIT"), on("AMTX_NO_CONVX12M"), on("AMTX_OF_ROWMAJOR_A3"), on("AMTX_OF_NO_ROLL_EPILOGUE")};
+    return {on("AMTX_NO_CONVG_MC2"), on("AMTX_NO_CONV_FUSE"), on("AMTX_X3_NO_SPLIT"), on("AMTX_NO_CONVX12M"), on("AMTX_OF_ROWMAJOR_A3"), on("AMTX_OF_NO_ROLL_EPILOGUE"),
+            on("AMTX_OF_ROWMAJOR_XP")};
 }
 
 struct ConvPlan {
@@ -42,6 +43,7 @@
     bool two_plane_acts;
     bool convx12; size_t c2x_per;
     bool rowmajor_a3, no_roll_epilogue;
+    bool rowmajor_xp;
     bool device_resync;
     int fuses_db_scale, takes_feats16;
 };
@@ -62,7 +64,7 @@
     p.two_plane_acts = pl == 2 && f3 == K_CONV && p.conv1_fused && !sw.x3_no_split && (f2 == K_CONV ? ic == 1 : ic > 1 && (9 * ic + 31) / 32 <= 2);
     p.convx12 = p.two_plane_acts && f2 == K_CONVG && ic >= 2 && ic <= 8 && amtx_conv1g_tapk(ic, 2) && !sw.no_convx12m;
     p.c2x_per = frag3x3(K_CONV, nf1, nf1);
-    p.rowmajor_a3 = sw.rowmajor_a3; p.no_roll_epilogue = sw.no_roll_epilogue;
+    p.rowmajor_a3 = sw.rowmajor_a3; p.no_roll_epilogue = sw.no_roll_epilogue; p.rowmajor_xp = sw.rowmajor_xp;
     p.device_resync = f2 == K_CONVG || ic == 1;
     p.fuses_db_scale = p.conv1_fused && f2 == K_CONV && ic == 1;
     p.takes_feats16 = !(p.conv1_fused && f2 == K_CONVG && precision != AMTX_PREC_F16) ? 0 : p.convx12 ? 2 : pl == 1 && nf1 == 32 && amtx_conv1g_tapk(ic, pl);
@@ -497,6 +499,49 @@
     return g;
 }
 
+static GemmArgs xproj_gemm_args(const amtx_of_model* m, int stage, const Workspace& w, int64_t BT) {
+    const int at = m->act_type, pl = m->planes;
+    const bool sp = m->plan.two_plane_acts;
+    GemmArgs g;
+    if (stage == 0) {
+        g = gemm_args(w.e, m->dim_am, sp ? AMTX_T_SPLIT : at, m->rec_ih, pl, w.xp, m->xw, at, BT, m->n_rec, BT * m->dim_am, BT * m->xw);
+        g.a_split = BT * m->dim_am * m->n_heads;
+        return g;
+    }
+    const int kp = (m->dim_aj + 63) / 64 * 64;
+    if (pl == 1) {
+        g = gemm_args(w.joint16, kp, AMTX_T_BF16, m->adj_ih, pl, w.xp2, m->xw, at, BT, 1, 0, 0);
+        g.K = kp;
+    } else if (sp) {
+        g = gemm_args(w.joint16, kp, AMTX_T_SPLIT, m->adj_ih, pl, w.xp2, m->xw, at, BT, 1, 0, 0);
+        g.K = kp; g.a_split = BT * kp;
+    } else {
+        g = gemm_args(w.joint, m->dim_aj, AMTX_T_F32, m->adj_ih, pl, w.xp2, m->xw, at, BT, 1, 0, 0);
+    }
+    return g;
+}
+
+static LstmArgs bilstm_args(const amtx_of_model* m, int stage, const Workspace& w, int B, int T) {
+    const int64_t BT = (int64_t)B * T;
+    LstmArgs l;
+    l.xproj = stage == 0 ? w.xp : w.xp2; l.x_type = m->act_type; l.whh = (const bf16_t*)(stage == 0 ? m->rec_hh.p : m->adj_hh.p); l.planes = m->planes;
+    l.out = stage == 0 ? w.l1 : w.l2; l.out_type = m->act_type;
+    l.B = B; l.T = T; l.groups = stage == 0 ? m->n_rec : 1; l.x_gs = BT * m->xw; l.w_gs = (int64_t)m->hh_elems; l.out_gs = BT * m->dim_lm;
+    l.hidden = m->hid;
+    return l;
+}
+
+struct XpCall { bool tiled[2]; };
+static XpCall resolve_xp(const amtx_of_model* m, int B, int T) {
+    XpCall c{{false, false}};
+    if (m->plan.rowmajor_xp || ((int64_t)B * T) % 16 != 0 || m->hid != 128) return c;
+    const Workspace none{};
+    for (int stage = 0; stage < 2; ++stage)
+        c.tiled[stage] = m->k->gemm_writes_tiled_c(xproj_gemm_args(m, stage, none, (int64_t)B * T)) && m->k->lstm_reads_tiled_x(bilstm_args(m, stage, none, B, T));
+    return c;
+}
+constexpr int XP_GATE_SHIFT = 7;
+
 struct FeatsIn { const float* feats; const void* feats16; int64_t stride_b, stride_c, stride_t, stride_f; const float *clip_max, *ref; };
 
 template <class Mark>
@@ -589,14 +634,13 @@
     if ((rc = k->launch_gemm(g, s)) != AMTX_OK) return rc;
     mark();
 
-    g = gemm_args(w.e, m->dim_am, at_d, m->rec_ih, pl, w.xp, m->xw, at, BT, m->n_rec, BT * m->dim_am, BT * m->xw);
-    g.a_split = e_split;
+    const XpCall xpc = resolve_xp(m, B, T);
+    g = xproj_gemm_args(m, 0, w, BT);
+    if (xpc.tiled[0]) { g.c_tiled = 1; g.n_gate_shift = XP_GATE_SHIFT; }
     if ((rc = k->launch_gemm(g, s)) != AMTX_OK) return rc;
     mark();
-    LstmArgs l;
-    l.xproj = w.xp; l.x_type = at; l.whh = (const bf16_t*)m->rec_hh.p; l.planes = pl; l.out = w.l1; l.out_type = at;
-    l.B = B; l.T = T; l.groups = m->n_rec; l.x_gs = BT * m->xw; l.w_gs = (int64_t)m->hh_elems; l.out_gs = BT * m->dim_lm;
-    l.hidden = m->hid;
+    LstmArgs l = bilstm_args(m, 0, w, B, T);
+    l.x_tiled = xpc.tiled[0];
     if ((rc = k->launch_bilstm(l, s)) != AMTX_OK) return rc;
     mark();
     g = gemm_args(w.l1, m->dim_lm, at, m->rec_out, pl, w.joint, m->dim_aj, AMTX_T_F32, BT, m->n_rec, BT * m->dim_lm, m->n_out);
@@ -620,18 +664,15 @@
 
     if (pl == 1) {
         if (!copy_on && (rc = amtx_launch_cvt_pad_bf16((const float*)w.joint, m->dim_aj, m->dim_aj, (bf16_t*)w.joint16, kp, BT, s, m->f16)) != AMTX_OK) return rc;
-        g = gemm_args(w.joint16, kp, AMTX_T_BF16, m->adj_ih, pl, w.xp2, m->xw, at, BT, 1, 0, 0);
-        g.K = kp;
     } else if (sp) {
         if ((rc = amtx_launch_cvt_split((const float*)w.joint, m->dim_aj, m->dim_aj, (bf16_t*)w.joint16, kp, BT * kp, BT, s)) != AMTX_OK) return rc;
-        g = gemm_args(w.joint16, kp, AMTX_T_SPLIT, m->adj_ih, pl, w.xp2, m->xw, at, BT, 1, 0, 0);
-        g.K = kp; g.a_split = BT * kp;
-    } else {
-        g = gemm_args(w.joint, m->dim_aj, AMTX_T_F32, m->adj_ih, pl, w.xp2, m->xw, at, BT, 1, 0, 0);
-    }
+    }
+    g = xproj_gemm_args(m, 1, w, BT);
+    if (xpc.tiled[1]) { g.c_tiled = 1; g.n_gate_shift = XP_GATE_SHIFT; }
     if ((rc = k->launch_gemm(g, s)) != AMTX_OK) return rc;
     mark();
-    l.xproj = w.xp2; l.whh = (const bf16_t*)m->adj_hh.p; l.out = w.l2; l.groups = 1;
+    l = bilstm_args(m, 1, w, B, T);
+    l.x_tiled = xpc.tiled[1];
     if ((rc = k->launch_bilstm(l, s)) != AMTX_OK) return rc;
     mark();
     g = gemm_args(w.l2, m->dim_lm, at, m->adj_out, pl, w.mp, m->n_out, AMTX_T_F32, BT, 1, 0, 0);
@@ -660,6 +701,19 @@
 
 extern "C" int amtx_of_fuses_db_scale(const amtx_of_model* m) { return m && m->finalized && m->plan.fuses_db_scale; }
 extern "C" int amtx_of_conv_stack_fused(const amtx_of_model* m, int batch, int num_frames) { return m && resolve_conv(m, batch, num_frames, false).path == PATH_STACK; }
+extern "C" int amtx_of_xp_tiled(const amtx_of_model* m, int batch, int num_frames) {
+    if (!m || !m->finalized || batch <= 0 || num_frames <= 0) return 0;
+    const XpCall c = resolve_xp(m, batch, num_frames);
+    return (c.tiled[0] ? 1 : 0) | (c.tiled[1] ? 2 : 0);
+}
+extern "C" int64_t amtx_xp_tile_offset(int64_t row, int col, int n_cols) {
+    if (row < 0 || col < 0 || n_cols <= 0 || n_cols % 64 != 0 || col >= n_cols) return -1;
+    return amtx_xp_tile_byte(row, col, n_cols);
+}
+extern "C" int amtx_xp_gate_source_row(int col, int log2_hidden) {
+    if (col < 0 || log2_hidden < 0 || log2_hidden > 20) return -1;
+    return amtx_xp_gate_row(col, log2_hidden);
+}
 
 extern "C" int amtx_of_forward(const amtx_of_model* m, const float* feats, int64_t stride_b, int64_t stride_c, int64_t stride_t,
                                int64_t stride_f, int batch, int num_frames, void* workspace, size_t workspace_bytes,
diff --git a/amt_tools_amd/models.py b/amt_tools_amd/models.py
--- a/amt_tools_amd/models.py
+++ b/amt_tools_amd/models.py
@@ -391,6 +391,9 @@
 
     def conv_stack_fused(self, batch, num_frames):
         return bool(_lib.call('amtx_of_conv_stack_fused', self.handle, int(batch), int(num_frames)))
+
+    def xp_tiled(self, batch, num_frames):
+        return _lib.call('amtx_of_xp_tiled', self.handle, int(batch), int(num_frames))
 
     def forward(self, feats, want_logits=True):
         pending = feats if isinstance(feats, PendingFeatures) else None
diff --git a/include/amtx_xp.h b/include/amtx_xp.h
--- /dev/null
+++ b/include/amtx_xp.h
@@ -0,0 +1,18 @@
+#ifndef AMTX_XP_H
+#define AMTX_XP_H
+
+#include "amtx.h"
+
+#ifdef __cplusplus
+extern "C" {
+#endif
+
+int amtx_of_xp_tiled(const amtx_of_model* model, int batch, int num_frames);
+int64_t amtx_xp_tile_offset(int64_t row, int col, int n_cols);
+int amtx_xp_gate_source_row(int col, int log2_hidden);
+
+#ifdef __cplusplus
+}
+#endif
+
+#endif
```

Result: no change. 40.79 million, median of 6 (+0.5%).
